# google/libultrahdr

Hardware: AMD Instinct MI355X
Metric: Mpixels/s encode+decode (API-1 P010+YUV420, 4K), device-resident round trip (higher is better)
Workload: dtype f32; 1 GPU; API-1 3840x2160 round trip per step: encode (P010 HLG + YCbCr420 -> two-pass 3-ch gain map at scale 1, FDCT q95, Huffman: two JPEG scans) + decode (Huffman, IDCT, applyGainMap -> RGBA_F16 linear); frames resident in HBM

## Files before the change

### libultrahdr_amd/csrc/api_context.cpp

```cpp
#include "api_internal.h"

#include <sys/mman.h>
#include <mutex>
#include <algorithm>

namespace uhdr_api {
uhdr_error_info_t ensure(DeviceBuf& b, size_t bytes) {
  if (b.cap >= bytes) return ok_status();
  if (b.p) (void)hipFree(b.p);
  b.p = nullptr;
  b.cap = 0;
  size_t want = bytes + (bytes >> 3) + 256;
  HIP_TRY(hipMalloc(&b.p, want));
  b.cap = want;
  return ok_status();
}


size_t bytes_per_sample(int fmt) {
  switch (fmt) {
    case UHDR_IMG_FMT_24bppYCbCrP010:
    case UHDR_IMG_FMT_30bppYCbCr444: return 2;
    case UHDR_IMG_FMT_24bppRGB888: return 3;
    case UHDR_IMG_FMT_32bppRGBA8888:
// ... 389 lines not shown
  c->gain_tabs.push_back(g);
  *out = g.meta;
  return ok_status();
}

uhdr_error_info_t select_hdr_lut(uhdr_hip_ctx* c, uhdr_color_transfer_t ct, const float** lut, int* n) {
  *lut = nullptr;
  *n = 0;
  if (ct == UHDR_CT_HLG) {
    UHDR_TRY(upload_lut(&c->d_hlg_inv_ootf, host::hlg_inv_oetf_ootf_lut(), c->stream));
    *lut = c->d_hlg_inv_ootf; *n = kInvOetfN;
  } else if (ct == UHDR_CT_PQ) {
    UHDR_TRY(upload_lut(&c->d_pq_inv, host::pq_inv_oetf_lut(), c->stream));
    *lut = c->d_pq_inv; *n = kInvOetfN;
  } else if (ct == UHDR_CT_SRGB) {
    *lut = c->d_srgb; *n = kSrgbN;
  }
  return ok_status();
}

uhdr_error_info_t validate_metadata(const uhdr_gainmap_metadata_t* m) {
  if (!m) return err_status(UHDR_CODEC_INVALID_PARAM, "received nullptr for gainmap metadata descriptor");
  uhdr_error_info_t st = ok_status();
  for (int i = 0; i < 3; i++) {
    if (!std::isfinite(m->min_content_boost[i]) || !std::isfinite(m->max_content_boost[i]) ||
        !std::isfinite(m->offset_sdr[i]) || !std::isfinite(m->offset_hdr[i]) ||
        !std::isfinite(m->hdr_capacity_min) || !std::isfinite(m->hdr_capacity_max) || !std::isfinite(m->gamma[i])) {
      st = err_status(UHDR_CODEC_INVALID_PARAM, "Field(s) of gainmap metadata descriptor are either NaN or infinite");
    } else if (m->max_content_boost[i] < m->min_content_boost[i]) {
      st = err_status(UHDR_CODEC_INVALID_PARAM, "received bad value for content boost max %f, expects to be >= content boost min %f",
                      m->max_content_boost[i], m->min_content_boost[i]);
    } else if (m->min_content_boost[i] <= 0.0f) {
      return err_status(UHDR_CODEC_INVALID_PARAM, "received bad value for min boost %f, expects > 0.0f", m->min_content_boost[i]);
    } else if (m->gamma[i] <= 0.0f) {
      st = err_status(UHDR_CODEC_INVALID_PARAM, "received bad value for gamma %f, expects > 0.0f", m->gamma[i]);
    } else if (m->offset_sdr[i] < 0.0f) {
      st = err_status(UHDR_CODEC_INVALID_PARAM, "received bad value for offset sdr %f, expects to be >= 0.0f", m->offset_sdr[i]);
    } else if (m->offset_hdr[i] < 0.0f) {
      st = err_status(UHDR_CODEC_INVALID_PARAM, "received bad value for offset hdr %f, expects to be >= 0.0f", m->offset_hdr[i]);
    } else if (m->hdr_capacity_max <= m->hdr_capacity_min) {
      st = err_status(UHDR_CODEC_INVALID_PARAM, "received bad value for hdr capacity max %f, expects to be > hdr capacity min %f",
                      m->hdr_capacity_max, m->hdr_capacity_min);
    } else if (m->hdr_capacity_min < 1.0f) {
      st = err_status(UHDR_CODEC_INVALID_PARAM, "received bad value for hdr capacity min %f, expects to be >= 1.0f", m->hdr_capacity_min);
    }
  }
  return st;
}

bool is_rgb_fmt_host(int fmt) {
  return fmt == UHDR_IMG_FMT_64bppRGBAHalfFloat || fmt == UHDR_IMG_FMT_32bppRGBA8888 ||
         fmt == UHDR_IMG_FMT_32bppRGBA1010102;
}

uhdr_error_info_t validate_apply(const uhdr_raw_image_t* sdr, const uhdr_raw_image_t* gm,
                                 const uhdr_gainmap_metadata_t* md, uhdr_color_transfer_t out_ct,
                                 const uhdr_raw_image_t* dest) {
  if (dest == nullptr || dest->planes[UHDR_PLANE_PACKED] == nullptr)
    return err_status(UHDR_CODEC_INVALID_PARAM, "apply gainmap method received nullptr for destination image or plane pointer");
  if (dest->stride[UHDR_PLANE_PACKED] < dest->w)
    return err_status(UHDR_CODEC_INVALID_PARAM, "destination stride (%u) cannot be less than image width (%u)",
                      dest->stride[UHDR_PLANE_PACKED], dest->w);
  if (out_ct != UHDR_CT_LINEAR && out_ct != UHDR_CT_HLG && out_ct != UHDR_CT_PQ)
    return err_status(UHDR_CODEC_INVALID_PARAM,
                      "apply gainmap method expects output color transfer to be one of {UHDR_CT_LINEAR, UHDR_CT_HLG, UHDR_CT_PQ}. Received %d", out_ct);
  if ((out_ct == UHDR_CT_LINEAR && dest->fmt != UHDR_IMG_FMT_64bppRGBAHalfFloat) ||
      ((out_ct == UHDR_CT_HLG || out_ct == UHDR_CT_PQ) && dest->fmt != UHDR_IMG_FMT_32bppRGBA1010102))
    return err_status(UHDR_CODEC_INVALID_PARAM, "unsupported destination pixel format %d for output color transfer %d", dest->fmt, out_ct);
  UHDR_TRY(validate_metadata(md));
  if (!sdr || !gm) return err_status(UHDR_CODEC_INVALID_PARAM, "received nullptr for base image or gainmap image");
  if (sdr->fmt != UHDR_IMG_FMT_24bppYCbCr444 && sdr->fmt != UHDR_IMG_FMT_16bppYCbCr422 &&
      sdr->fmt != UHDR_IMG_FMT_12bppYCbCr420 && sdr->fmt != UHDR_IMG_FMT_24bppRGB888 &&
      sdr->fmt != UHDR_IMG_FMT_32bppRGBA8888)
    return err_status(UHDR_CODEC_UNSUPPORTED_FEATURE, "apply gainmap method expects base image color format to be one of "
                      "{UHDR_IMG_FMT_24bppYCbCr444, UHDR_IMG_FMT_16bppYCbCr422, UHDR_IMG_FMT_12bppYCbCr420, "
                      "UHDR_IMG_FMT_24bppRGB888, UHDR_IMG_FMT_32bppRGBA8888}. Received %d", sdr->fmt);
  if (gm->fmt != UHDR_IMG_FMT_8bppYCbCr400 && gm->fmt != UHDR_IMG_FMT_24bppRGB888 && gm->fmt != UHDR_IMG_FMT_32bppRGBA8888)
    return err_status(UHDR_CODEC_UNSUPPORTED_FEATURE, "apply gainmap method expects gainmap image color format to be one of "
                      "{UHDR_IMG_FMT_8bppYCbCr400, UHDR_IMG_FMT_24bppRGB888, UHDR_IMG_FMT_32bppRGBA8888}. Received %d", gm->fmt);
  return ok_status();
}

uhdr_error_info_t get_apply_tables(uhdr_hip_ctx* c, const uhdr_gainmap_metadata_t& md, float weight,
                                   int idw_scale, const float** d_out) {
  std::string key((const char*)&md, sizeof md);
  key.append((const char*)&weight, sizeof weight);
  key.append((const char*)&idw_scale, sizeof idw_scale);
  for (int i = 0; i < kTableSlots; i++)
    if (c->tab_cap[i] && c->tab_key[i] == key) { *d_out = c->d_tab[i]; return ok_status(); }
  const int slot = c->tab_next;
  c->tab_next = (c->tab_next + 1) % kTableSlots;
  std::vector<float> t;
  host::build_apply_tables(md, weight, idw_scale, &t);
  const size_t bytes = t.size() * sizeof(float);
  if (c->tab_cap[slot]) HIP_TRY(hipEventSynchronize(c->tab_ev[slot]));
  if (c->tab_cap[slot] < bytes) {
    HIP_TRY(hipStreamSynchronize(c->stream));
    if (c->h_tab[slot]) (void)hipHostFree(c->h_tab[slot]);
    if (c->d_tab[slot]) (void)hipFree(c->d_tab[slot]);
    c->h_tab[slot] = nullptr; c->d_tab[slot] = nullptr; c->tab_cap[slot] = 0;
    HIP_TRY(hipHostMalloc((void**)&c->h_tab[slot], bytes, hipHostMallocDefault));
    HIP_TRY(hipMalloc((void**)&c->d_tab[slot], bytes));
    if (!c->tab_ev[slot]) HIP_TRY(hipEventCreateWithFlags(&c->tab_ev[slot], hipEventDisableTiming));
    c->tab_cap[slot] = bytes;
  }
  memcpy(c->h_tab[slot], t.data(), bytes);
  HIP_TRY(hipMemcpyAsync(c->d_tab[slot], c->h_tab[slot], bytes, hipMemcpyHostToDevice, c->stream));
  HIP_TRY(hipEventRecord(c->tab_ev[slot], c->stream));
  c->tab_key[slot] = key;
  *d_out = c->d_tab[slot];
  return ok_status();
}
}


const char* uhdr_hip_version(void) { return "libuhdr_hip 0.3 (gfx950; reference libultrahdr 2.0.2 hot path)"; }

int uhdr_hip_device_count(void) {
  int n = 0;
  if (hipGetDeviceCount(&n) != hipSuccess) return 0;
  return n;
}

int uhdr_hip_current_device(void) {
  int d = -1;
  if (hipGetDevice(&d) != hipSuccess) return -1;
  return d;
}

uhdr_hip_ctx_t* uhdr_hip_create(int device, uhdr_error_info_t* err) {
  auto fail = [&](const char* what, hipError_t e) -> uhdr_hip_ctx_t* {
    if (err) *err = err_status(UHDR_CODEC_ERROR, "uhdr_hip_create: %s failed: %s (no CPU fallback exists behind this library)",
                               what, hipGetErrorString(e));
    return nullptr;
  };
  if (err) *err = ok_status();
  int n = 0;
  hipError_t e = hipGetDeviceCount(&n);
  if (e != hipSuccess || n == 0) return fail("hipGetDeviceCount", e == hipSuccess ? hipErrorNoDevice : e);
  if (device < 0) {
    e = hipGetDevice(&device);
    if (e != hipSuccess) return fail("hipGetDevice", e);
  }
  if (device >= n) return fail("device index", hipErrorInvalidDevice);
  e = hipSetDevice(device);
  if (e != hipSuccess) return fail("hipSetDevice", e);
  uhdr_hip_ctx* c = new uhdr_hip_ctx();
  c->device = device;
  {
    const char* e = getenv("UHDR_HIP_HUFF_TWO_PASS");
    c->huff_two_pass = e && atoi(e) != 0;
    e = getenv("UHDR_HIP_HUFF_ROUTE_LOG");
    c->huff_route_log = e && atoi(e) != 0;
  }
  e = hipStreamCreateWithFlags(&c->own_stream, hipStreamNonBlocking);
  if (e != hipSuccess) { delete c; return fail("hipStreamCreate", e); }
  c->stream = c->own_stream;
  uhdr_error_info_t st = upload_lut(&c->d_srgb, host::srgb_inv_oetf_lut(), c->stream);
  if (st.error_code != UHDR_CODEC_OK) {
    if (err) *err = st;
    (void)hipStreamDestroy(c->own_stream);
    delete c;
    return nullptr;
  }
  return c;
}

void uhdr_hip_destroy(uhdr_hip_ctx_t* c) {
  if (!c) return;
  (void)hipSetDevice(c->device);
  (void)hipStreamSynchronize(c->stream);
  for (auto& e : c->prof_entries) { (void)hipEventDestroy(e.a); (void)hipEventDestroy(e.b); }
  float* luts[] = {c->d_srgb, c->d_hlg_inv, c->d_pq_inv, c->d_hlg_oetf, c->d_pq_oetf, c->d_hlg_inv_ootf, (float*)c->d_math,
                   c->d_hlg_buckets, c->d_pq_buckets, c->d_hlg_buckets_pre, c->d_pq_buckets_pre};
  for (float* p : luts) if (p) (void)hipFree(p);
  for (int i = 0; i < kTableSlots; i++) {
    if (c->h_tab[i]) (void)hipHostFree(c->h_tab[i]);
    if (c->d_tab[i]) (void)hipFree(c->d_tab[i]);
    if (c->tab_ev[i]) (void)hipEventDestroy(c->tab_ev[i]);
  }
  for (auto& b : c->scratch) if (b.p) (void)hipFree(b.p);
  for (auto& b : c->jpg) if (b.p) (void)hipFree(b.p);
  for (auto& b : c->enc) if (b.p) (void)hipFree(b.p);
  if (c->huff_slots.p) (void)hipFree(c->huff_slots.p);
  for (auto& r : c->resident) if (r.buf.p) (void)hipFree(r.buf.p);
  if (c->pending.buf.p) (void)hipFree(c->pending.buf.p);
  if (c->pending.tmp.p) (void)hipFree(c->pending.tmp.p);
  if (c->minmax.p) (void)hipFree(c->minmax.p);
  if (c->d_coef_src) (void)hipFree(c->d_coef_src);
  if (c->d_huff) (void)hipFree(c->d_huff);
  if (c->d_srgb8) (void)hipFree(c->d_srgb8);
  for (float* q : c->d_lin10) if (q) (void)hipFree(q);
  for (auto& g : c->gain_tabs) if (g.d) (void)hipFree(g.d);
  uhdr_hip_comm_destroy(c);
  aux_worker_destroy(c);
  if (c->aux) uhdr_hip_destroy(c->aux);
  if (c->exchange.p) (void)hipFree(c->exchange.p);
  if (c->affine.p) (void)hipFree(c->affine.p);
  if (c->d_srgb_of_byte) (void)hipFree(c->d_srgb_of_byte);
  if (c->h_mm) (void)hipHostFree(c->h_mm);
  if (c->aux_ev) (void)hipEventDestroy(c->aux_ev);
  if (c->aux_ev2) (void)hipEventDestroy(c->aux_ev2);
  if (c->md_ev) (void)hipEventDestroy(c->md_ev);
  if (c->md_stream) (void)hipStreamDestroy(c->md_stream);
  if (c->h_flags) (void)hipHostFree(c->h_flags);
  if (c->pin.p) (void)hipHostFree(c->pin.p);
  if (c->pin.ev) (void)hipEventDestroy(c->pin.ev);
  if (c->huff_tabs.dev.p) (void)hipFree(c->huff_tabs.dev.p);
  if (c->own_stream) (void)hipStreamDestroy(c->own_stream);
  delete c;
}

int uhdr_hip_recycle(uhdr_hip_ctx_t* c, size_t keep_bytes) {
  if (!c) return -1;
  (void)hipSetDevice(c->device);
  (void)hipStreamSynchronize(c->stream);
  uhdr_hip_resident_forget(c);
  uhdr_hip_resident_begin(c);
  uhdr_hip_resident_end(c);
  c->sticky = ok_status();
  for (auto& h : c->huff_hint) h = uhdr_hip_ctx::HuffHint();
  c->stats = uhdr_hip_stats_t();
  c->deferred_md.valid = false;
  c->huff_slots_refused = 0;
  std::vector<DeviceBuf*> bufs;
  for (auto& b : c->scratch) bufs.push_back(&b);
  for (auto& b : c->jpg) bufs.push_back(&b);
  for (auto& b : c->enc) bufs.push_back(&b);
  bufs.push_back(&c->huff_slots);
  for (auto& r : c->resident) bufs.push_back(&r.buf);
  bufs.push_back(&c->pending.buf);
  bufs.push_back(&c->pending.tmp);
  size_t total = c->pin.cap;
  for (DeviceBuf* b : bufs) total += b->p ? b->cap : 0;
  std::sort(bufs.begin(), bufs.end(), [](const DeviceBuf* a, const DeviceBuf* b) { return (a->p ? a->cap : 0) > (b->p ? b->cap : 0); });
  for (DeviceBuf* b : bufs) {
    if (total <= keep_bytes) break;
    if (!b->p) continue;
    (void)hipFree(b->p);
    total -= b->cap;
    b->p = nullptr;
    b->cap = 0;
  }
  if (total > keep_bytes && c->pin.p) {
    if (c->pin.ev_pending && c->pin.ev) (void)hipEventSynchronize(c->pin.ev);
    (void)hipHostFree(c->pin.p);
    c->pin.p = nullptr;
    c->pin.cap = c->pin.off = 0;
    c->pin.ev_pending = false;
  }
  if (c->aux) (void)uhdr_hip_recycle(c->aux, keep_bytes);
  return c->device;
}

uhdr_error_info_t uhdr_hip_set_stream(uhdr_hip_ctx_t* c, void* hip_stream) {
  if (!c) return err_status(UHDR_CODEC_INVALID_PARAM, "received nullptr for uhdr_hip context");
  HIP_TRY(hipStreamSynchronize(c->stream));
  c->stream = hip_stream ? (hipStream_t)hip_stream : c->own_stream;
  return ok_status();
}

void* uhdr_hip_get_stream(uhdr_hip_ctx_t* c) { return c ? (void*)c->stream : nullptr; }

uhdr_error_info_t uhdr_hip_synchronize(uhdr_hip_ctx_t* c) {
  if (!c) return err_status(UHDR_CODEC_INVALID_PARAM, "received nullptr for uhdr_hip context");
  HIP_TRY(hipStreamSynchronize(c->stream));
  return ok_status();
}

void uhdr_hip_get_stats(uhdr_hip_ctx_t* c, uhdr_hip_stats_t* out) {
  if (!out) return;
  if (!c) { memset(out, 0, sizeof *out); return; }
  *out = c->stats;
}

namespace {
std::mutex g_seam_mu;
std::vector<uhdr_hip_seam_stage_t> g_seam_rows;
unsigned long long g_seam_seq = 0;
void seam_dump_at_exit() {
  const char* path = getenv("UHDR_HIP_SEAM_STATS_FILE");
  FILE* f = path ? fopen(path, "w") : nullptr;
  if (!f) return;
  std::lock_guard<std::mutex> lk(g_seam_mu);
  fprintf(f, "{");
  for (size_t i = 0; i < g_seam_rows.size(); i++) {
    const auto& r = g_seam_rows[i];
    fprintf(f, "%s\"%s\": {\"device\": %llu, \"reference\": %llu, \"device_ms\": %.3f, \"first_seq\": %llu}", i ? ", " : "", r.name, r.device_calls,
            r.reference_calls, r.device_ms, r.first_seq);
  }
  fprintf(f, "}\n");
  fclose(f);
}
}

void uhdr_hip_seam_note(const char* stage, int on_device, double ms) {
  if (!stage) return;
  static const bool dump = [] { return getenv("UHDR_HIP_SEAM_STATS_FILE") ? (atexit(seam_dump_at_exit), true) : false; }();
  (void)dump;
  std::lock_guard<std::mutex> lk(g_seam_mu);
  uhdr_hip_seam_stage_t* row = nullptr;
  for (auto& r : g_seam_rows)
    if (!strncmp(r.name, stage, sizeof r.name - 1)) { row = &r; break; }
  if (!row) {
    if (g_seam_rows.size() >= 64) return;
    uhdr_hip_seam_stage_t r;
// ... 152 lines not shown
```

### libultrahdr_amd/csrc/api_entropy.cpp

```cpp
#include "api_internal.h"

#include <condition_variable>
#include <functional>
#include <mutex>

uhdr_error_info_t uhdr_api::check_scan(const uhdr_hip_jpeg_scan_t* sc, bool need_coef, int* mcus_per_row, int* mcu_rows, int* blocks_per_mcu) {
  if (!sc) return err_status(UHDR_CODEC_INVALID_PARAM, "received nullptr for the scan description");
  if (sc->num_components != 1 && sc->num_components != 3)
    return err_status(UHDR_CODEC_INVALID_PARAM, "a scan has 1 or 3 components, received %d", sc->num_components);
  if (sc->w == 0 || sc->h == 0 || sc->w > 65535 || sc->h > 65535)
    return err_status(UHDR_CODEC_INVALID_PARAM, "image dimensions %ux%u are outside JPEG's 1..65535", sc->w, sc->h);
  int hmax = 1, vmax = 1, bpm = 0;
  for (int i = 0; i < sc->num_components; i++) {
    const int hs = sc->num_components == 1 ? 1 : sc->h_samp[i], vs = sc->num_components == 1 ? 1 : sc->v_samp[i];
    if (hs < 1 || hs > 2 || vs < 1 || vs > 2) return err_status(UHDR_CODEC_INVALID_PARAM, "component %d: sampling factors %dx%d not in {1, 2}", i, hs, vs);
    if (hs > hmax) hmax = hs;
    if (vs > vmax) vmax = vs;
    bpm += hs * vs;
    if (need_coef && (!sc->coef[i] || ((uintptr_t)sc->coef[i] & 15)))
      return err_status(UHDR_CODEC_INVALID_PARAM, "coefficient buffer %d is null or not 16-byte aligned", i);
    if (sc->blocks_w[i] < 1 || sc->blocks_h[i] < 1) return err_status(UHDR_CODEC_INVALID_PARAM, "component %d: empty block grid", i);
  }
  if (sc->num_components == 1) {
    *mcus_per_row = sc->blocks_w[0];
// ... 171 lines not shown
static bool make_fast_table(const uint8_t bits[17], const uint8_t vals[256], HuffFastTable* t, int* nsub_out = nullptr) {
  memset(t, 0, sizeof *t);
  int code = 0, k = 0, nsub = 0;
  int sub_of[512];
  for (int i = 0; i < 512; i++) sub_of[i] = -1;
  for (int l = 1; l <= 16; l++) {
    for (int i = 0; i < bits[l]; i++, k++, code++) {
      if (code >= (1 << l) || k >= 256) return false;
      if (l <= 9) {
        const int lo = code << (9 - l);
        for (int x = 0; x < (1 << (9 - l)); x++) t->l1[lo + x] = (uint16_t)((l << 8) | vals[k]);
      } else {
        const int prefix = code >> (l - 9);
        if (sub_of[prefix] < 0) {
          if (nsub >= kHuffL2Max) return false;
          sub_of[prefix] = nsub++;
          t->l1[prefix] = (uint16_t)(0x8000u | (unsigned)sub_of[prefix]);
        }
        const int rest = (code << (16 - l)) & 127;
        for (int x = 0; x < (1 << (16 - l)); x++) t->l2[sub_of[prefix]][rest + x] = (uint16_t)((l << 8) | vals[k]);
      }
    }
    code <<= 1;
  }
  if (nsub_out) *nsub_out = nsub;
  return true;
}

static void make_track_table(const HuffFastTable& f, bool is_dc, HuffFastTable* t) {
  auto conv = [&](uint16_t e) -> uint16_t {
    if (e & 0x8000u) return e;
    unsigned adv, kinc;
    if (e == 0) {
      adv = 16;
      kinc = is_dc ? 1 : 64;
    } else {
      const unsigned len = (e >> 8) & 31u, rs = e & 255u;
      if (is_dc) {
        const unsigned sz = rs > 15u ? 0u : rs;
        adv = len + sz;
        kinc = 1;
      } else {
        const unsigned sz = rs & 15u, run = rs >> 4;
        adv = len + sz;
        kinc = sz ? run + 1 : (run == 15u ? 16u : 64u);
      }
    }
    return (uint16_t)(adv | (kinc << 5));
  };
  for (int i = 0; i < 512; i++) t->l1[i] = conv(f.l1[i]);
  for (int s = 0; s < kHuffL2Max; s++)
    for (int i = 0; i < 128; i++) t->l2[s][i] = conv(f.l2[s][i]);
}

static void make_value_table(const HuffFastTable& f, bool is_dc, uint32_t* out ) {
  auto conv = [&](uint16_t e, bool first_level) -> uint32_t {
    if (first_level && (e & 0x8000u)) return 0x80000000u | (e & 31u);
    unsigned adv, kinc, sz = 0, bad = 0;
    if (e == 0) {
      adv = 16;
      kinc = is_dc ? 1 : 64;
      bad = 1;
    } else {
      const unsigned len = (e >> 8) & 31u, rs = e & 255u;
      if (is_dc) {
        if (rs > 15u) bad = 1; else sz = rs;
        adv = len + sz;
        kinc = 1;
      } else {
        sz = rs & 15u;
        const unsigned run = rs >> 4;
        adv = len + sz;
        kinc = sz ? run + 1 : (run == 15u ? 16u : 64u);
      }
    }
    return adv | (kinc << 5) | (sz << 12) | (bad << 16);
  };
  for (int i = 0; i < 512; i++) out[i] = conv(f.l1[i], true);
  for (int s = 0; s < kHuffL2Max; s++)
    for (int i = 0; i < 128; i++) out[512 + s * 128 + i] = conv(f.l2[s][i], false);
}

static void make_pair_table(const HuffFastTable& f, const HuffFastTable& t, const HuffFastTable& f_ac, const HuffFastTable& t_ac, int l2_base, uint32_t* out ) {
  constexpr int B = kHuffPairBits;
  for (int idx = 0; idx < kHuffPairWords; idx++) {
    const int p9 = idx >> (B - 9);
    const uint16_t e = f.l1[p9];
    uint32_t first;
    bool defined;
    if (e & 0x8000u) {
      const int sub = e & 31, rest = (idx & ((1 << (B - 9)) - 1)) << (16 - B);
      const uint16_t e2 = f.l2[sub][rest];
      if (e2 == 0 || (int)((e2 >> 8) & 31u) > B) {
        out[idx] = 0x80000000u | (uint32_t)(l2_base + sub);
        continue;
      }
      first = t.l2[sub][rest];
      defined = true;
    } else {
      first = t.l1[p9];
      defined = e != 0;
    }
    uint32_t word = first & 0xfffu;
    const int adv1 = (int)(first & 31u), kinc1 = (int)((first >> 5) & 127u);
    if (defined && kinc1 < 64 && adv1 < B) {
      const int r = B - adv1;
      const int next9 = ((idx << adv1) & (kHuffPairWords - 1)) >> (B - 9);
      const uint16_t n = f_ac.l1[next9];
      if (n != 0 && !(n & 0x8000u) && (int)((n >> 8) & 31u) <= r) {
        const uint32_t second = t_ac.l1[next9];
        word |= (second & 31u) << 12 | ((second >> 5) & 127u) << 17;
      }
    }
    out[idx] = word;
  }
}

static void make_pair_value_table(const HuffFastTable& f, const uint32_t* v, const HuffFastTable& f_ac, const uint32_t* v_ac, int l2_base, uint32_t* out ) {
  constexpr int B = kHuffPairBits;
  for (int idx = 0; idx < kHuffPairWords; idx++) {
    const int p9 = idx >> (B - 9);
    const uint16_t e = f.l1[p9];
    uint32_t first;
    bool defined;
    if (e & 0x8000u) {
      const int sub = e & 31, rest = (idx & ((1 << (B - 9)) - 1)) << (16 - B);
      const uint16_t e2 = f.l2[sub][rest];
      if (e2 == 0 || (int)((e2 >> 8) & 31u) > B) {
        out[2 * idx] = 0x80000000u | (uint32_t)(l2_base + sub);
        out[2 * idx + 1] = 0;
        continue;
      }
      first = v[512 + sub * 128 + rest];
      defined = true;
    } else {
      first = v[p9];
      defined = e != 0;
    }
    uint32_t second = 0;
    const int adv1 = (int)(first & 31u), kinc1 = (int)((first >> 5) & 127u);
    if (defined && !((first >> 16) & 1u) && kinc1 < 64 && adv1 < B) {
      const int r = B - adv1;
      const int next9 = ((idx << adv1) & (kHuffPairWords - 1)) >> (B - 9);
      const uint16_t n = f_ac.l1[next9];
      if (n != 0 && !(n & 0x8000u) && (int)((n >> 8) & 31u) <= r) second = v_ac[next9];
    }
    out[2 * idx] = first;
    out[2 * idx + 1] = second;
  }
}

uhdr_error_info_t uhdr_hip_huffman_decode_dev(uhdr_hip_ctx_t* c, const uhdr_hip_jpeg_scan_t* sc, const uhdr_hip_huff_tables_t* tables,
                                              const uint8_t* data, size_t data_bytes) {
  if (!c) return err_status(UHDR_CODEC_INVALID_PARAM, "received nullptr for uhdr_hip context");
  if (!data || data_bytes == 0 || data_bytes > 0xFFFFFFF0ull) return err_status(UHDR_CODEC_INVALID_PARAM, "received no (or more than 4 GiB of) entropy-coded data");
  int mpr = 0, mrows = 0, bpm = 0;
  UHDR_TRY(check_scan(sc, true, &mpr, &mrows, &bpm));
  if (sc->restart_interval < 0 || sc->restart_interval > 65535) return err_status(UHDR_CODEC_INVALID_PARAM, "restart_interval %d out of range", sc->restart_interval);
  HIP_TRY(hipSetDevice(c->device));
  if (!c->d_huff) {
    std::vector<uint32_t> blob(host::jpeg_huff_code_tables());
    blob.resize((size_t)host::kHuffTabWords + 16);
    memcpy(blob.data() + host::kHuffTabWords, host::jpeg_zigzag_to_natural(), 64);
    HIP_TRY(hipMalloc((void**)&c->d_huff, blob.size() * sizeof(uint32_t)));
    HIP_TRY(hipMemcpyAsync(c->d_huff, blob.data(), blob.size() * sizeof(uint32_t), hipMemcpyHostToDevice, c->stream));
    HIP_TRY(hipStreamSynchronize(c->stream));
  }
  const DbgClock dbg;
  constexpr size_t kTabDec = 0, kTabFast = (sizeof(HuffDecTable) * 4 + 255) & ~(size_t)255,
                   kTabVal = (kTabFast + sizeof(HuffFastTable) * 8 + 255) & ~(size_t)255, kTabPair = kTabVal + (size_t)4 * kHuffValWords * 4,
                   kTabPairVal = kTabPair + (size_t)kHuffPairBlobWords * 4, kTabBytes = kTabPairVal + (size_t)kHuffPairValBlobWords * 4;
  {
    uint8_t key[4 * (17 + 256)];
    for (int t = 0; t < 4; t++) {
      uint8_t* bits = key + (size_t)t * (17 + 256);
      uint8_t* vals = bits + 17;
      if (tables) {
        memcpy(bits, tables->bits[t], 17);
        memcpy(vals, tables->vals[t], 256);
      } else {
        memset(bits, 0, 17 + 256);
        host::jpeg_std_huff_table(t & 1, t >> 1, bits, vals);
      }
    }
    uhdr_hip_ctx::HuffTabCache& hc = c->huff_tabs;
    if (!hc.valid || memcmp(hc.key, key, sizeof key) != 0) {
      hc.valid = false;
      std::vector<HuffDecTable> tabs(4);
      std::vector<HuffFastTable> ftabs(8);
      std::vector<uint32_t> vtabs((size_t)4 * kHuffValWords), ptabs((size_t)kHuffPairBlobWords), pvtabs((size_t)kHuffPairValBlobWords);
      bool fast_ok = true;
      int l2_count[4] = {0, 0, 0, 0};
      for (int t = 0; t < 4; t++) {
        const uint8_t* bits = key + (size_t)t * (17 + 256);
        if (!make_dec_table(bits, bits + 17, &tabs[(size_t)t])) return err_status(UHDR_CODEC_INVALID_PARAM, "Huffman table %d is not a valid DHT table", t);
        fast_ok = make_fast_table(bits, bits + 17, &ftabs[(size_t)t], &l2_count[t]) && fast_ok;
      }
      int l2_base[4] = {0, 0, 0, 0};
      for (int t = 1; t < 4; t++) l2_base[t] = l2_base[t - 1] + l2_count[t - 1];
      if (l2_base[3] + l2_count[3] > kHuffL2Total) fast_ok = false;
      if (fast_ok)
        for (int t = 0; t < 4; t++) {
          make_track_table(ftabs[(size_t)t], (t & 1) == 0, &ftabs[(size_t)t + 4]);
          make_value_table(ftabs[(size_t)t], (t & 1) == 0, vtabs.data() + (size_t)t * kHuffValWords);
        }
      if (fast_ok)
        for (int t = 0; t < 4; t++)
        {
          make_pair_table(ftabs[(size_t)t], ftabs[(size_t)t + 4], ftabs[(size_t)(t | 1)], ftabs[(size_t)(t | 1) + 4], l2_base[t], ptabs.data() + (size_t)t * kHuffPairWords);
          make_pair_value_table(ftabs[(size_t)t], vtabs.data() + (size_t)t * kHuffValWords, ftabs[(size_t)(t | 1)], vtabs.data() + (size_t)(t | 1) * kHuffValWords,
                                l2_base[t], pvtabs.data() + (size_t)t * 2 * kHuffPairWords);
          uint16_t* l2t = (uint16_t*)(ptabs.data() + (size_t)4 * kHuffPairWords) + (size_t)l2_base[t] * 128;
          uint16_t* l2v = (uint16_t*)(pvtabs.data() + (size_t)8 * kHuffPairWords) + (size_t)l2_base[t] * 128;
          for (int i = 0; i < l2_count[t] * 128; i++) {
            l2t[i] = ftabs[(size_t)t + 4].l2[i / 128][i % 128];
            const uint32_t v = vtabs[(size_t)t * kHuffValWords + 512 + (size_t)i];
            l2v[i] = (uint16_t)(((v >> 16) & 1u) ? 0u : (v & 0xffffu));
          }
        }
      UHDR_TRY(ensure(hc.dev, kTabBytes));
      HIP_TRY(hipStreamSynchronize(c->stream));
      HIP_TRY(hipMemcpy((uint8_t*)hc.dev.p + kTabDec, tabs.data(), sizeof(HuffDecTable) * 4, hipMemcpyHostToDevice));
      HIP_TRY(hipMemcpy((uint8_t*)hc.dev.p + kTabFast, ftabs.data(), sizeof(HuffFastTable) * 8, hipMemcpyHostToDevice));
      HIP_TRY(hipMemcpy((uint8_t*)hc.dev.p + kTabVal, vtabs.data(), vtabs.size() * 4, hipMemcpyHostToDevice));
      HIP_TRY(hipMemcpy((uint8_t*)hc.dev.p + kTabPair, ptabs.data(), ptabs.size() * 4, hipMemcpyHostToDevice));
      HIP_TRY(hipMemcpy((uint8_t*)hc.dev.p + kTabPairVal, pvtabs.data(), pvtabs.size() * 4, hipMemcpyHostToDevice));
      memcpy(hc.key, key, sizeof key);
      hc.fast_ok = fast_ok;
      hc.valid = true;
    }
  }
  const bool fast_ok = c->huff_tabs.fast_ok;
  const uint8_t* tabs_dev = (const uint8_t*)c->huff_tabs.dev.p;
  if (!c->h_flags) HIP_TRY(hipHostMalloc((void**)&c->h_flags, 64 * sizeof(uint32_t), hipHostMallocDefault));
  HuffDecArgs a;
  memset(&a, 0, sizeof a);
  a.ncomp = sc->num_components;
  size_t zero_bytes[3] = {0, 0, 0};
  for (int i = 0; i < a.ncomp; i++) {
    a.coef[i] = const_cast<int16_t*>(sc->coef[i]);
    a.bw[i] = sc->blocks_w[i]; a.bh[i] = sc->blocks_h[i];
    a.hs[i] = a.ncomp == 1 ? 1 : sc->h_samp[i]; a.vs[i] = a.ncomp == 1 ? 1 : sc->v_samp[i];
    zero_bytes[i] = (size_t)a.bw[i] * a.bh[i] * 64 * sizeof(int16_t);
  }
  a.mcus_per_row = mpr;
  a.total_mcus = mpr * mrows;
  a.ri = sc->restart_interval;
  a.nseg = a.ri > 0 ? (a.total_mcus + a.ri - 1) / a.ri : 1;
  a.data = data;
  a.nbytes = (uint32_t)data_bytes;
  a.zigzag = (const uint8_t*)(c->d_huff + host::kHuffTabWords);
  const int nchunks = huff_marker_chunks(data_bytes);
  const size_t need = 16 + ((size_t)nchunks + 2 * (size_t)a.nseg) * sizeof(uint32_t);
  UHDR_TRY(ensure(c->scratch[5], need));
  uint8_t* base = (uint8_t*)c->scratch[5].p;
  a.tabs = (const HuffDecTable*)(tabs_dev + kTabDec);
  a.status = (uint32_t*)base;
  uint32_t* counts = a.status + 4;
  uint32_t* starts = counts + nchunks;
  uint32_t* ends = starts + a.nseg;
  a.starts = starts;
  a.ends = ends;
  dbg.mark("huffman_decode_dev: tables ready");
  const bool rst_sync = a.nseg > 1 && data_bytes / (size_t)a.nseg >= 320 && !getenv("UHDR_HIP_HUFF_RST_INTERVALS");
  const bool try_sync = (a.nseg == 1 || rst_sync) && data_bytes >= 4096 && data_bytes < ((size_t)1 << 29) && fast_ok && !getenv("UHDR_HIP_HUFF_SERIAL") && bpm <= 16;
  const int write_form = [] { const char* e = getenv("UHDR_HIP_HUFF_WRITE"); return e ? atoi(e) : 2; }();
  const bool form2 = try_sync && !rst_sync && write_form != 1;
  bool coef_zeroed = !form2;
  if (!form2)
    for (int i = 0; i < a.ncomp; i++) HIP_TRY(hipMemsetAsync(a.coef[i], 0, zero_bytes[i], c->stream));
  bool sync_done = false;
  if (try_sync) {
    struct Attempt { uint32_t sub_bits; int levels; };
    std::vector<Attempt> attempts;
    bool sparse = false;
    {
      const char* eb = getenv("UHDR_HIP_HUFF_SUB_BITS");
      const char* el = getenv("UHDR_HIP_HUFF_LEVELS");
      const int vb = eb ? atoi(eb) : 0;
      const bool vb_ok = vb >= 256 && vb <= 4096 && (vb & (vb - 1)) == 0;
      if (vb_ok || el) {
        const uint32_t sbits = vb_ok ? (uint32_t)vb : 1024u;
        const int lv = el ? atoi(el) : (sbits <= 512 ? 7 : 4);
        if (lv >= 1 && lv <= 15 && bpm * (lv + 1) <= kHuffHypSlots) attempts.push_back({sbits, lv});
        attempts.push_back({sbits, 0});
      } else {
        const uint64_t bits_per_block = (uint64_t)data_bytes * 8u / (uint64_t)((uint64_t)a.total_mcus * (uint64_t)bpm);
        const int lv_fit = kHuffHypSlots / bpm - 1;
        const int lv = lv_fit >= 15 ? 15 : (lv_fit >= 11 ? 11 : (lv_fit >= 7 ? 7 : (lv_fit >= 4 ? 4 : 0)));
        sparse = bits_per_block < 64;
        uint32_t first = bits_per_block < 64 ? 1024u : (bits_per_block < 200 ? 512u : (bits_per_block < 400 ? 2048u : 4096u));
        const uhdr_hip_ctx::HuffHint& hint = c->huff_hint[bpm & 15];
        if (hint.sub_bits > first && bits_per_block * 4 >= hint.bits_per_block * 3 && bits_per_block * 4 <= hint.bits_per_block * 5) first = hint.sub_bits;
        if (lv > 0)
          for (uint32_t sbits = first; sbits <= 4096u; sbits <<= 1) attempts.push_back({sbits, lv});
        attempts.push_back({1024u, 0});
      }
    }
    uint32_t sub_bits = attempts[0].sub_bits;
    bool use_hyp = false;
    for (const Attempt& t : attempts) { if (t.sub_bits < sub_bits) sub_bits = t.sub_bits; use_hyp = use_hyp || t.levels > 0; }
    const int max_rounds = 40;
    const int nch = huff_sync_chunks(data_bytes);
    const uint32_t nsub = huff_sync_max_subsequences(data_bytes, sub_bits);
    const uint32_t total_blocks = (uint32_t)a.total_mcus * (uint32_t)bpm;
    size_t off = 0;
    auto take = [&](size_t bytes) { const size_t o = off; off += (bytes + 255) & ~(size_t)255; return o; };
    const size_t rst_words = data_bytes / 32 + 2;
    const size_t o_clean = take(data_bytes + 16), o_cnt = take((size_t)nch * 4);
    const size_t o_flags = take(128), o_nblk = take((size_t)nsub * 4 + 4), o_dcd = take((size_t)total_blocks * 4), o_rm = rst_sync ? take(rst_words * 4) : 0;
    const size_t zero_bytes_sync = off - o_flags;
    const size_t o_s0 = take((size_t)nsub * 8), o_hm = use_hyp ? take((size_t)nsub * kHuffHypSlots) : 0;
    const size_t ff_bytes = off - o_s0;
    const size_t o_s1 = take((size_t)nsub * 8), o_c0 = take(nsub), o_c1 = take(nsub), o_dcp = take((size_t)((total_blocks + 255) / 256) * 12 + 16),
                 o_ft = take(sizeof(HuffFastTable) * 8),
                 o_st = take(((size_t)nsub / 2048 + 2) * 4), o_vt = take((size_t)4 * kHuffValWords * 4);
    const size_t o_hs = use_hyp ? take((size_t)nsub * kHuffHypSlots * 8) : 0, o_hc = use_hyp ? take((size_t)nsub * kHuffHypSlots * 2) : 0;
    size_t chain_tiles_off = 0;
    const size_t o_ch = use_hyp ? take(huff_hyp_chain_bytes(data_bytes, sub_bits, &chain_tiles_off)) : 0;
    (void)chain_tiles_off;
    const size_t o_ds = rst_sync ? take((size_t)a.nseg * 12) : 0, o_rp = rst_sync ? take((size_t)nch * 12) : 0;
    const size_t o_sl = use_hyp ? take((size_t)nsub * (size_t)bpm * 8) : 0;
    const int max_pieces = [&] {
      const char* e = getenv("UHDR_HIP_HUFF_PIECES");
      const int v = e ? atoi(e) : 4;
      return (use_hyp && form2 && !rst_sync && v >= 1 && v <= 4) ? v : 1;
    }();
    const size_t o_ms = max_pieces > 1 ? take((size_t)nsub * kHuffHypSlots * (size_t)(max_pieces - 1) * 8) : 0;
    const size_t o_mc = max_pieces > 1 ? take((size_t)nsub * kHuffHypSlots * (size_t)(max_pieces - 1) * 2) : 0;
    const size_t o_pe = max_pieces > 1 ? take((size_t)nsub * (size_t)max_pieces * 8 + 64) : 0;
    const size_t o_pc = max_pieces > 1 ? take(((size_t)nsub * (size_t)max_pieces + 4) * 4) : 0;
    const size_t o_st2 = max_pieces > 1 ? take(((size_t)nsub * (size_t)max_pieces / 2048 + 4) * 4) : 0;
    const size_t scan_bytes = form2 ? (size_t)total_blocks * 64 * sizeof(int16_t) : 0;
    const size_t o_cs = form2 ? take(scan_bytes + 256) : 0;
    UHDR_TRY(ensure(c->scratch[6], off));
    uint8_t* sb = (uint8_t*)c->scratch[6].p;
    HuffSyncArgs y;
    memset(&y, 0, sizeof y);
    y.clean = sb + o_clean;
    y.nbytes = (uint32_t)data_bytes;
    y.flags = (uint32_t*)(sb + o_flags);
    y.nstuffed = y.flags + 8;
    y.sub_bits = sub_bits;
    y.state[0] = (uint64_t*)(sb + o_s0); y.state[1] = (uint64_t*)(sb + o_s1);
    y.changed[0] = sb + o_c0; y.changed[1] = sb + o_c1;
    y.nblk = (uint32_t*)(sb + o_nblk);
    y.scan_tmp = (uint32_t*)(sb + o_st);
    y.dcd = (int*)(sb + o_dcd);
    y.total_blocks = total_blocks;
    y.blocks_per_mcu = bpm; y.ncomp = a.ncomp; y.mcus_per_row = a.mcus_per_row;
    uint32_t* rst_map = nullptr;
    if (rst_sync) {
      rst_map = (uint32_t*)(sb + o_rm);
      y.rst_map = rst_map;
      y.rst_blocks = (uint32_t)a.ri * (uint32_t)bpm;
      y.dc_seg = (int*)(sb + o_ds);
      y.rst_partial = (uint32_t*)(sb + o_rp);
      y.rst_chunks = (uint32_t)nch;
    }
    int j = 0;
    for (int i = 0; i < a.ncomp; i++) {
      y.bw[i] = a.bw[i]; y.bh[i] = a.bh[i]; y.hs[i] = a.hs[i]; y.vs[i] = a.vs[i]; y.coef[i] = a.coef[i];
      y.first_blk[i] = j;
      for (int k = 0; k < a.hs[i] * a.vs[i] && j < 16; k++) y.comp_of[j++] = (uint8_t)i;
    }
    y.ftabs = (const HuffFastTable*)(tabs_dev + kTabFast);
    y.ttabs = y.ftabs + 4;
    y.vtabs = (const uint32_t*)(tabs_dev + kTabVal);
    y.ptabs = (const uint32_t*)(tabs_dev + kTabPair);
    y.pvtabs = (const uint32_t*)(tabs_dev + kTabPairVal);
    y.zigzag = a.zigzag;
    (void)o_ft; (void)o_vt;
    if (use_hyp) {
      y.strag_list = (uint32_t*)(sb + o_sl);
      y.strag_cap = nsub * (uint32_t)bpm;
    }
    if (form2) y.coef_scan = (int16_t*)(sb + o_cs);
    const int main_levels_env = [&] { const char* e = getenv("UHDR_HIP_HUFF_MAIN_LEVELS"); return e ? atoi(e) : (sparse ? 1 : 2); }();
    if (j == bpm && bpm <= 16) {
      const bool fills_in_unstuff = attempts[0].levels > 0 && zero_bytes_sync % 16 == 0 && ff_bytes % 16 == 0 && zero_bytes_sync / 16 < 0xFFFFFFFFull &&
                                    ff_bytes / 16 < 0xFFFFFFFFull && !getenv("UHDR_HIP_HUFF_FILL_LAUNCHES");
      HuffInitFill init_fill;
      memset(&init_fill, 0, sizeof init_fill);
      if (fills_in_unstuff) {
        init_fill.zero_ptr = (uint4*)y.flags;
        init_fill.zero_vec = (uint32_t)(zero_bytes_sync / 16);
        init_fill.ff_ptr = (uint4*)y.state[0];
        init_fill.ff_vec = (uint32_t)(ff_bytes / 16);
      } else {
        HIP_TRY(hipMemsetAsync(y.flags, 0, zero_bytes_sync, c->stream));
      }
      auto pass0_zeroes = [&](const Attempt& t) { return form2 && t.levels > 0 && scan_bytes % 16 == 0 && scan_bytes / 16 < 0xFFFFFFFFull; };
      if (form2 && !pass0_zeroes(attempts[0])) HIP_TRY(hipMemsetAsync(y.coef_scan, 0, scan_bytes, c->stream));
      dbg.mark("huffman_decode_dev: fills enqueued");
      int final_buf = 0;
      uint32_t* fl = c->h_flags;
      for (int q = 0; q < 24; q++) fl[q] = 0;
      bool hyp_done = false, unstuffed = false, rounds_ran = false;
      auto start_over = [&](const Attempt& next) -> uhdr_error_info_t {
        HIP_TRY(hipMemsetAsync(y.flags, 0, 32, c->stream));
        HIP_TRY(hipMemsetAsync(y.flags + kHuffFlagStragglers, 0, 4, c->stream));
        HIP_TRY(hipMemsetAsync(y.nblk, 0, (size_t)nsub * 4 + 4, c->stream));
        if (form2) {
          if (!pass0_zeroes(next)) HIP_TRY(hipMemsetAsync(y.coef_scan, 0, scan_bytes, c->stream));
        } else {
          HIP_TRY(hipMemsetAsync(y.dcd, 0, (size_t)total_blocks * 4, c->stream));
          for (int i = 0; i < a.ncomp; i++) HIP_TRY(hipMemsetAsync(a.coef[i], 0, zero_bytes[i], c->stream));
        }
        return ok_status();
      };
      for (size_t ti = 0; ti < attempts.size() && !hyp_done && !rounds_ran; ti++) {
        const Attempt& t = attempts[ti];
        if (ti > 0) UHDR_TRY(start_over(t));
        y.sub_bits = t.sub_bits;
        y.zero_ptr = pass0_zeroes(t) ? (uint4*)y.coef_scan : nullptr;
        y.zero_vec = pass0_zeroes(t) ? (uint32_t)(scan_bytes / 16) : 0u;
        const uint32_t nsub_t = huff_sync_max_subsequences(data_bytes, t.sub_bits);
        if (t.levels > 0) {
          y.hyp_h = bpm;
          y.hyp_levels = t.levels;
          y.hyp_main_levels = rst_sync ? 0 : main_levels_env;
          y.strag_levels = [&] { const char* e = getenv("UHDR_HIP_HUFF_STRAG_LEVELS"); return e ? atoi(e) : t.levels; }();
          y.hyp_state = (uint64_t*)(sb + o_hs);
          y.hyp_map = sb + o_hm;
          y.hyp_cnt = (uint16_t*)(sb + o_hc);
          y.hyp_hist = getenv("UHDR_HIP_HUFF_DEBUG") ? 1 : 0;
          {
            int q = t.sub_bits >= 1024u ? (int)(t.sub_bits / 256u) : 1;
            if (getenv("UHDR_HIP_HUFF_PIECES_ALL")) q = (int)(t.sub_bits / 256u);
            if (q > max_pieces) q = max_pieces;
            if (q < 1) q = 1;
            while (q > 1 && (t.sub_bits % (uint32_t)q || (t.sub_bits / (uint32_t)q) % 32u)) q--;
            if (q == 3) q = 2;
            if (getenv("UHDR_HIP_HUFF_QMERGE") && atoi(getenv("UHDR_HIP_HUFF_QMERGE")) == 0) q = 1;
            y.pieces = q;
            y.mid_state = q > 1 ? (uint64_t*)(sb + o_ms) : nullptr;
            y.mid_cnt = q > 1 ? (uint16_t*)(sb + o_mc) : nullptr;
            y.pend = q > 1 ? (uint64_t*)(sb + o_pe) : nullptr;
            y.pcnt = q > 1 ? (uint32_t*)(sb + o_pc) : nullptr;
            y.scan_tmp = q > 1 ? (uint32_t*)(sb + o_st2) : (uint32_t*)(sb + o_st);
          }
          if (!(fills_in_unstuff && ti == 0)) HIP_TRY(hipMemsetAsync(y.state[0], 0xff, ff_bytes, c->stream));
          size_t tiles_off = 0;
          (void)huff_hyp_chain_bytes(data_bytes, t.sub_bits, &tiles_off);
          {
            ProfScope ps(c, "huffman_decode");
            if (!unstuffed)
              HIP_TRY(launch_huffman_unstuff(data, (uint32_t)data_bytes, (uint32_t*)(sb + o_cnt), y.flags + 8, sb + o_clean, c->stream, rst_map, y.rst_partial,
                                             fills_in_unstuff && ti == 0 ? &init_fill : nullptr));
            unstuffed = true;
            HIP_TRY(launch_huffman_decode_hyp(y, (int*)(sb + o_dcp), sb + o_ch, sb + o_ch + tiles_off, c->stream));
          }
          dbg.mark("huffman_decode_dev: hypothesis attempt enqueued");
          HIP_TRY(hipMemcpyAsync(fl, y.flags, 24 * sizeof(uint32_t), hipMemcpyDeviceToHost, c->stream));
          HIP_TRY(wait_stream(c));
          dbg.mark("huffman_decode_dev: hypothesis attempt finished");
          hyp_done = fl[2] == 0;
          if (hyp_done && ti > 0) {
            uhdr_hip_ctx::HuffHint& hint = c->huff_hint[bpm & 15];
            hint.sub_bits = t.sub_bits;
            hint.bits_per_block = (uint32_t)((uint64_t)data_bytes * 8u / ((uint64_t)a.total_mcus * (uint64_t)bpm));
          }
          if (getenv("UHDR_HIP_HUFF_DEBUG")) {
            uint32_t hist[32] = {};
            (void)hipMemcpy(hist, y.flags, sizeof hist, hipMemcpyDeviceToHost);
            fprintf(stderr, "uhdr_hip: hypothesis decode of %zu bytes, %u subsequences of %u bits x %d: merges per level %u %u %u %u %u %u+, %u paths unmerged after %d levels (%d in lockstep, %u paths handed to the straggler waves), true path %s\n",
                    data_bytes, nsub_t, t.sub_bits, bpm, hist[10], hist[11], hist[12], hist[13], hist[14], hist[15], fl[3], t.levels, y.hyp_main_levels, fl[kHuffFlagStragglers], hyp_done ? "resolved" : "LOST (next attempt)");
            fprintf(stderr, "uhdr_hip: the stragglers' merges at level 2 .. 10, 11+: %u %u %u %u %u %u %u %u %u %u\n", hist[22], hist[23], hist[24], hist[25], hist[26], hist[27], hist[28], hist[29],
                    hist[30], hist[31]);
          }
        } else {
          y.pieces = 1;
          y.scan_tmp = (uint32_t*)(sb + o_st);
          {
            ProfScope ps(c, "huffman_decode");
            if (!unstuffed) HIP_TRY(launch_huffman_unstuff(data, (uint32_t)data_bytes, (uint32_t*)(sb + o_cnt), y.flags + 8, sb + o_clean, c->stream, rst_map, y.rst_partial));
            unstuffed = true;
            HIP_TRY(launch_huffman_decode_sync(y, max_rounds, (int*)(sb + o_dcp), &final_buf, c->stream));
          }
          HIP_TRY(hipMemcpyAsync(fl, y.flags, 24 * sizeof(uint32_t), hipMemcpyDeviceToHost, c->stream));
          HIP_TRY(wait_stream(c));
          rounds_ran = true;
        }
      }
      const bool settled = hyp_done || fl[4 + max_rounds % 3] == 0;
      if (rst_sync && getenv("UHDR_HIP_HUFF_DEBUG"))
        fprintf(stderr, "uhdr_hip: restart file through the parallel decoder: %s, status bits %#x, %u markers dropped (%d expected), sequence sums %s\n",
                settled ? "settled" : "NOT settled", fl[1], fl[9], a.nseg - 1, fl[0] == fl[16] && fl[7] == fl[17] ? "equal" : "DIFFERENT");
      if (settled && rst_sync && ((fl[1] & 14u) != 0 || fl[9] != (uint32_t)(a.nseg - 1) || fl[0] != fl[16] || fl[7] != fl[17])) {
        for (int i = 0; i < a.ncomp; i++) HIP_TRY(hipMemsetAsync(a.coef[i], 0, zero_bytes[i], c->stream));
        coef_zeroed = true;
      } else if (settled) {
        if (fl[1] & 8u) return err_status(UHDR_CODEC_INVALID_PARAM, "corrupt entropy-coded data (the scan ends before its last block)");
        if (fl[1] & 2u) return err_status(UHDR_CODEC_INVALID_PARAM, "corrupt entropy-coded data (undefined Huffman code or a run past the end of a block)");
        sync_done = true;
      } else {
        if (a.nseg == 1 && !c->huff_serial_ok && data_bytes > (256u << 10)) {
          c->stats.entropy_decode_declined++;
          return err_status(UHDR_CODEC_UNSUPPORTED_FEATURE, "the parallel entropy decode did not settle in %d rounds; %zu bytes on one lane would take longer than the CPU", max_rounds, data_bytes);
        }
        for (int i = 0; i < a.ncomp; i++) HIP_TRY(hipMemsetAsync(a.coef[i], 0, zero_bytes[i], c->stream));
        coef_zeroed = true;
      }
    }
  }
  if (sync_done) {
    c->stats.entropy_decode_parallel++;
    return ok_status();
  }
  if (a.nseg == 1 && !c->huff_serial_ok && data_bytes > (256u << 10)) {
    c->stats.entropy_decode_declined++;
    return err_status(UHDR_CODEC_UNSUPPORTED_FEATURE, "a %zu-byte scan without restart markers that the parallel decoder does not take (Huffman tables outside its two-level form)", data_bytes);
  }
  if (!coef_zeroed)
    for (int i = 0; i < a.ncomp; i++) HIP_TRY(hipMemsetAsync(a.coef[i], 0, zero_bytes[i], c->stream));
  HIP_TRY(hipMemsetAsync(a.status, 0, 16, c->stream));
  {
    ProfScope ps(c, "huffman_decode");
    HIP_TRY(launch_huffman_decode(a, counts, starts, ends, c->stream));
  }
  if (a.nseg == 1) c->stats.entropy_decode_single_lane++;
  else c->stats.entropy_decode_intervals++;
  uint32_t st[2] = {0, 0};
  HIP_TRY(hipMemcpyAsync(st, a.status, sizeof st, hipMemcpyDeviceToHost, c->stream));
  HIP_TRY(wait_stream(c));
  if (st[1] != (uint32_t)(a.nseg - 1))
    return err_status(UHDR_CODEC_INVALID_PARAM, "found %u restart markers, a restart interval of %d MCUs over %d MCUs needs %d", st[1], a.ri,
                      a.total_mcus, a.nseg - 1);
  if (st[0] & 4u) return err_status(UHDR_CODEC_INVALID_PARAM, "restart markers out of sequence");
  if (st[0] & 2u) return err_status(UHDR_CODEC_INVALID_PARAM, "corrupt entropy-coded data (undefined Huffman code or a run past the end of a block)");
  return ok_status();
}

uhdr_error_info_t uhdr_api::aux_context(uhdr_hip_ctx* c, uhdr_hip_ctx** out) {
  if (!c->aux) {
    uhdr_error_info_t e = ok_status();
    c->aux = uhdr_hip_create(c->device, &e);
    if (!c->aux) return e.error_code != UHDR_CODEC_OK ? e : err_status(UHDR_CODEC_ERROR, "could not create the auxiliary context");
  }
  c->aux->prof = c->prof;
  c->aux->huff_serial_ok = c->huff_serial_ok;
  c->aux->huff_route_log = c->huff_route_log;
  c->aux->huff_two_pass = c->huff_two_pass;
  *out = c->aux;
  return ok_status();
}
void uhdr_api::aux_merge(uhdr_hip_ctx* c) {
  if (!c->aux) return;
  uhdr_hip_ctx* x = c->aux;
  c->stats.entropy_decode_parallel += x->stats.entropy_decode_parallel;
  c->stats.entropy_decode_intervals += x->stats.entropy_decode_intervals;
  c->stats.entropy_decode_single_lane += x->stats.entropy_decode_single_lane;
  c->stats.entropy_decode_declined += x->stats.entropy_decode_declined;
  c->stats.entropy_encode_stream += x->stats.entropy_encode_stream;
  c->stats.entropy_encode_intervals += x->stats.entropy_encode_intervals;
  x->stats = uhdr_hip_stats_t();
  for (auto& e : x->prof_entries) c->prof_entries.push_back(e);
  x->prof_entries.clear();
}

struct AuxWorker {
  static constexpr int kSpinUs = 300;
  std::thread th;
  std::mutex mu;
  std::condition_variable cv;
  std::function<void()> job;
  std::atomic<int> state{0};
  std::atomic<bool> busy{false};
  static bool spin_until(const std::function<bool()>& pred, int us) {
    const auto t0 = std::chrono::steady_clock::now();
    while (!pred()) {
      if (std::chrono::steady_clock::now() - t0 > std::chrono::microseconds(us)) return pred();
#if defined(__x86_64__)
      __builtin_ia32_pause();
#endif
    }
    return true;
  }
  AuxWorker() {
    th = std::thread([this] {
      for (;;) {
        if (!spin_until([this] { return state.load(std::memory_order_acquire) != 0; }, kSpinUs)) {
          std::unique_lock<std::mutex> lk(mu);
          cv.wait(lk, [this] { return state.load(std::memory_order_acquire) != 0; });
        }
        if (state.load(std::memory_order_acquire) == 2) return;
        std::function<void()> j;
        {
          std::lock_guard<std::mutex> lk(mu);
          j = std::move(job);
          state.store(0, std::memory_order_release);
        }
        j();
        {
          std::lock_guard<std::mutex> lk(mu);
          busy.store(false, std::memory_order_release);
        }
        cv.notify_all();
      }
    });
  }
  void run(std::function<void()> j) {
    {
      std::lock_guard<std::mutex> lk(mu);
      job = std::move(j);
      busy.store(true, std::memory_order_release);
      state.store(1, std::memory_order_release);
    }
    cv.notify_all();
  }
  void wait() {
    if (spin_until([this] { return !busy.load(std::memory_order_acquire); }, kSpinUs)) return;
    std::unique_lock<std::mutex> lk(mu);
    cv.wait(lk, [this] { return !busy.load(std::memory_order_acquire); });
  }
  ~AuxWorker() {
    {
      std::lock_guard<std::mutex> lk(mu);
      state.store(2, std::memory_order_release);
    }
    cv.notify_all();
    if (th.joinable()) th.join();
  }
};
void aux_worker_destroy(uhdr_hip_ctx* c) {
  if (c && c->aux_worker) {
    delete c->aux_worker;
    c->aux_worker = nullptr;
  }
}
bool uhdr_api::aux_post(uhdr_hip_ctx* c, std::function<void()> job) {
  static const bool no_thread = getenv("UHDR_HIP_NO_AUX_THREAD") != nullptr;
  if (no_thread) return false;
  if (!c->aux_worker) {
    try {
      c->aux_worker = new AuxWorker();
    } catch (...) {
      c->aux_worker = nullptr;
    }
  }
  if (!c->aux_worker) return false;
  c->aux_worker->run(std::move(job));
  return true;
}
void uhdr_api::aux_wait(uhdr_hip_ctx* c) {
  if (c->aux_worker) c->aux_worker->wait();
}
namespace {
template <typename FA, typename FB>
void run_pair(uhdr_hip_ctx* c, FA&& job_a, FB&& job_b) {
  static const bool no_thread = getenv("UHDR_HIP_NO_AUX_THREAD") != nullptr;
  if (!c->aux_worker && !no_thread) {
    try {
      c->aux_worker = new AuxWorker();
    } catch (...) {
      c->aux_worker = nullptr;
    }
  }
  if (c->aux_worker) {
    c->aux_worker->run(job_b);
    job_a();
    c->aux_worker->wait();
  } else {
    job_a();
    job_b();
  }
}
}

uhdr_error_info_t uhdr_hip_huffman_encode2_dev(uhdr_hip_ctx_t* c, const uhdr_hip_jpeg_scan_t* scan_a, uint8_t* out_a, size_t cap_a, size_t* bytes_a,
                                               const uhdr_hip_jpeg_scan_t* scan_b, uint8_t* out_b, size_t cap_b, size_t* bytes_b) {
  if (!c) return err_status(UHDR_CODEC_INVALID_PARAM, "received nullptr for uhdr_hip context");
  HIP_TRY(hipSetDevice(c->device));
  uhdr_hip_ctx* x = nullptr;
  UHDR_TRY(aux_context(c, &x));
  if (!c->aux_ev) HIP_TRY(hipEventCreateWithFlags(&c->aux_ev, hipEventDisableTiming));
  HIP_TRY(hipEventRecord(c->aux_ev, c->stream));
  HIP_TRY(hipStreamWaitEvent(x->stream, c->aux_ev, 0));
  uhdr_error_info_t ra = ok_status(), rb = ok_status();
  const int dev = c->device;
  run_pair(c, [&] { ra = uhdr_hip_huffman_encode_dev(c, scan_a, out_a, cap_a, bytes_a); },
           [&, dev] { (void)hipSetDevice(dev); rb = uhdr_hip_huffman_encode_dev(x, scan_b, out_b, cap_b, bytes_b); });
  aux_merge(c);
  return ra.error_code != UHDR_CODEC_OK ? ra : rb;
}

uhdr_error_info_t uhdr_hip_huffman_decode2_dev(uhdr_hip_ctx_t* c, const uhdr_hip_jpeg_scan_t* scan_a, const uhdr_hip_huff_tables_t* tables_a, const uint8_t* data_a,
                                               size_t bytes_a, const uhdr_hip_jpeg_scan_t* scan_b, const uhdr_hip_huff_tables_t* tables_b,
                                               const uint8_t* data_b, size_t bytes_b) {
  if (!c) return err_status(UHDR_CODEC_INVALID_PARAM, "received nullptr for uhdr_hip context");
  HIP_TRY(hipSetDevice(c->device));
  uhdr_hip_ctx* x = nullptr;
  UHDR_TRY(aux_context(c, &x));
  if (!c->aux_ev) HIP_TRY(hipEventCreateWithFlags(&c->aux_ev, hipEventDisableTiming));
  HIP_TRY(hipEventRecord(c->aux_ev, c->stream));
  HIP_TRY(hipStreamWaitEvent(x->stream, c->aux_ev, 0));
  uhdr_error_info_t ra = ok_status(), rb = ok_status();
  const int dev = c->device;
  run_pair(c, [&] { ra = uhdr_hip_huffman_decode_dev(c, scan_a, tables_a, data_a, bytes_a); },
           [&, dev] { (void)hipSetDevice(dev); rb = uhdr_hip_huffman_decode_dev(x, scan_b, tables_b, data_b, bytes_b); });
  aux_merge(c);
  return ra.error_code != UHDR_CODEC_OK ? ra : rb;
}
```

### libultrahdr_amd/csrc/api_internal.h

```cpp
#ifndef UHDR_HIP_API_INTERNAL_H
#define UHDR_HIP_API_INTERNAL_H

#pragma GCC visibility push(default)
#include "uhdr_hip.h"
#pragma GCC visibility pop

#include <cfloat>
#include <chrono>
#include <cmath>
#include <cstdarg>
#include <cstdio>
#include <cstring>
#include <atomic>
#include <functional>
#include <map>
#include <memory>
#include <string>
#include <thread>
#include <vector>
#include "exact_math.h"
#include "host_tables.h"
#include "uhdr_types.h"
#include "rccl_bind.h"

using namespace uhdr;

inline uhdr_error_info_t ok_status() {
  uhdr_error_info_t s;
  s.error_code = UHDR_CODEC_OK;
  s.has_detail = 0;
  s.detail[0] = 0;
  return s;
}
inline uhdr_error_info_t err_status(uhdr_codec_err_t code, const char* fmt, ...) {
  uhdr_error_info_t s;
  s.error_code = code;
  s.has_detail = 1;
  va_list ap;
  va_start(ap, fmt);
  vsnprintf(s.detail, sizeof s.detail, fmt, ap);
  va_end(ap);
  return s;
}
#define HIP_TRY(expr)                                                                      \
  do {                                                                                     \
    hipError_t e_ = (expr);                                                                \
    if (e_ != hipSuccess)                                                                  \
      return err_status(e_ == hipErrorOutOfMemory ? UHDR_CODEC_MEM_ERROR : UHDR_CODEC_ERROR, \
                        "HIP error '%s' at %s:%d", hipGetErrorString(e_), __FILE__, __LINE__); \
  } while (0)
#define UHDR_TRY(expr)                                 \
  do {                                                 \
    uhdr_error_info_t s_ = (expr);                     \
    if (s_.error_code != UHDR_CODEC_OK) return s_;     \
  } while (0)

struct DbgClock {
  bool on;
  std::chrono::steady_clock::time_point t0;
  DbgClock() : on(getenv("UHDR_HIP_CLOCK_DEBUG") != nullptr), t0(std::chrono::steady_clock::now()) {}
  void mark(const char* what) const {
    if (on) fprintf(stderr, "uhdr_hip:   [%7.1f us] %s\n", std::chrono::duration<double, std::micro>(std::chrono::steady_clock::now() - t0).count(), what);
  }
};

struct ProfEntry {
  hipEvent_t a, b;
  std::string family;
};

constexpr int kTableSlots = 4;

struct DeviceBuf {
  void* p = nullptr;
  size_t cap = 0;
};

struct uhdr_hip_ctx {
  int device = 0;
  hipStream_t own_stream = nullptr;
  hipStream_t stream = nullptr;
  float* d_srgb = nullptr;
  float* d_hlg_inv = nullptr;
  float* d_pq_inv = nullptr;
  float* d_hlg_oetf = nullptr;
  float* d_pq_oetf = nullptr;
  float* d_hlg_buckets = nullptr;
  float* d_pq_buckets = nullptr;
  float* d_hlg_buckets_pre = nullptr;
  float* d_pq_buckets_pre = nullptr;
  float* d_hlg_inv_ootf = nullptr;
  double* d_math = nullptr;
  float* h_tab[kTableSlots] = {};
  float* d_tab[kTableSlots] = {};
  size_t tab_cap[kTableSlots] = {};
  hipEvent_t tab_ev[kTableSlots] = {};
  std::string tab_key[kTableSlots];
  int tab_next = 0;
  DeviceBuf scratch[8];
  uhdr_hip_stats_t stats = {};
  bool huff_serial_ok = true;
  DeviceBuf huff_slots;
  bool huff_two_pass = false;
  bool huff_route_log = false;
  size_t huff_slots_refused = 0;
  DeviceBuf enc[3];
  uhdr_hip_ctx* aux = nullptr;
  struct AuxWorker* aux_worker = nullptr;
  DeviceBuf jpg[6];
  struct Resident {
    DeviceBuf buf;
    bool valid = false;
    uhdr_img_fmt_t fmt = UHDR_IMG_FMT_UNSPECIFIED;
    unsigned int w = 0, h = 0;
    const void* host[3] = {};
    unsigned int host_stride[3] = {};
    size_t off[3] = {};
    unsigned int dev_stride[3] = {};
    unsigned int prows[3] = {}, pcols[3] = {};
    bool host_unwritten = false;
    bool adopted = false;
    void* adopt_dst = nullptr;
    unsigned int adopt_stride = 0, adopt_w = 0, adopt_h = 0;
    bool adopt_expand = false;
  } resident[2];
  struct HuffHint { uint32_t sub_bits = 0, bits_per_block = 0; } huff_hint[16];
  struct HuffTabCache {
    bool valid = false, fast_ok = false;
    uint8_t key[4 * (17 + 256)] = {};
    DeviceBuf dev;
  } huff_tabs;
  struct PinArena {
    void* p = nullptr;
    size_t cap = 0, off = 0;
    hipEvent_t ev = nullptr;
    bool ev_pending = false;
  } pin;
  uint32_t* h_flags = nullptr;
  bool resident_on = false;
  bool resident_lazy = false;
  uhdr_error_info_t sticky = {};
  unsigned int resident_next = 0;
  struct PendingCopy {
    DeviceBuf buf;
    bool on = false;
    size_t off = 0, pitch = 0, dst_pitch = 0;
    unsigned int w = 0, h = 0, bps = 0;
    bool expand = false;
    void* dst = nullptr;
    DeviceBuf tmp;
  } pending;
  struct MallEntry { const void* p; uint64_t stamp; };
  std::vector<MallEntry> mall;
  uint64_t mall_clock = 0;
  DeviceBuf minmax;
  uint32_t* d_huff = nullptr;
  CoefSrc* d_coef_src = nullptr;
  unsigned int coef_src_next = 0;
  CoefSrc* coef_src_last_slot = nullptr;
  std::vector<uint8_t> coef_src_last;
  float* d_srgb8 = nullptr;
  StepTab srgb8_meta = {};
  float* d_lin10[5] = {};
  struct GainTab { float mn, mx; float* d; StepTab meta; };
  std::vector<GainTab> gain_tabs;
  void* comm = nullptr;
  int comm_rank = 0, comm_size = 0;
  bool comm_custom = false;
  uhdr_hip_comm_ops_t comm_ops = {};
  DeviceBuf exchange;
  DeviceBuf affine;
  float* d_srgb_of_byte = nullptr;
  float* h_mm = nullptr;
  bool defer_md = false;
  hipStream_t md_stream = nullptr;
  hipEvent_t md_ev = nullptr;
  std::function<void()> on_side_launched;
  bool side_job_posted = false;
  struct DeferredMd { bool valid = false, run = false; uhdr_hip_encode_cfg_t cfg; uhdr_color_transfer_t hdr_ct; int use_base_cg = 1; } deferred_md;
  hipEvent_t aux_ev = nullptr;
  hipEvent_t aux_ev2 = nullptr;
  bool prof = false;
  std::vector<ProfEntry> prof_entries;
};

struct ProfScope {
  uhdr_hip_ctx* c;
  ProfEntry e;
  bool on;
  ProfScope(uhdr_hip_ctx* ctx, const char* family) : c(ctx), on(ctx->prof) {
    if (!on) return;
    e.family = family;
    if (hipEventCreate(&e.a) != hipSuccess || hipEventCreate(&e.b) != hipSuccess) { on = false; return; }
    (void)hipEventRecord(e.a, c->stream);
  }
  ~ProfScope() {
    if (!on) return;
    (void)hipEventRecord(e.b, c->stream);
    c->prof_entries.push_back(e);
  }
};

namespace uhdr_api {
uhdr_error_info_t ensure(DeviceBuf& b, size_t bytes);
size_t bytes_per_sample(int fmt);
bool plane_geom(const uhdr_raw_image_t* im, int pl, size_t* rows, size_t* width);
size_t plane_bytes(const uhdr_raw_image_t* im, int pl);
uhdr_error_info_t validate_image(const uhdr_raw_image_t* im, const char* what);
ImageView view_of(const uhdr_raw_image_t* im);
ImageViewMut view_mut_of(const uhdr_raw_image_t* im);
uhdr_error_info_t adopted_copy_out(uhdr_hip_ctx* c, const void* src, size_t src_pitch, unsigned int bps, bool expand, unsigned int w, unsigned int h,
                                   void* dst, size_t dst_pitch);
uhdr_error_info_t resident_write_back(uhdr_hip_ctx* c, uhdr_hip_ctx::Resident& r);
uhdr_error_info_t resident_write_back_all(uhdr_hip_ctx* c);
void resident_retire(uhdr_hip_ctx* c, uhdr_hip_ctx::Resident& r, bool host_is_rewritten);
void resident_drop(uhdr_hip_ctx* c, const void* host_plane);
uhdr_error_info_t fast_h2d(uhdr_hip_ctx* c, void* dst, const void* src, size_t bytes);
uhdr_error_info_t stage_in(uhdr_hip_ctx* c, int slot, const uhdr_raw_image_t* host, uhdr_raw_image_t* dev, bool upload);
bool resident_keeps(int fmt);
uhdr_error_info_t resident_keep(uhdr_hip_ctx* c, const uhdr_raw_image_t* dev, const uhdr_raw_image_t* host, bool host_unwritten = false);
uhdr_error_info_t stage_out(uhdr_hip_ctx* c, const uhdr_raw_image_t* dev, uhdr_raw_image_t* host);
uhdr_error_info_t upload_lut(float** dst, const std::vector<float>& src, hipStream_t s);
uhdr_error_info_t upload_math(uhdr_hip_ctx* c);
uhdr_error_info_t upload_step_table(const host::OetfBuckets& b, float** slot, StepTab* meta, hipStream_t s);
uhdr_error_info_t gain_step_table(uhdr_hip_ctx* c, const GenParams& p, StepTab* out);
uhdr_error_info_t select_hdr_lut(uhdr_hip_ctx* c, uhdr_color_transfer_t ct, const float** lut, int* n);
uhdr_error_info_t validate_metadata(const uhdr_gainmap_metadata_t* m);
bool is_rgb_fmt_host(int fmt);
uhdr_error_info_t validate_apply(const uhdr_raw_image_t* sdr, const uhdr_raw_image_t* gm, const uhdr_gainmap_metadata_t* md, uhdr_color_transfer_t out_ct,
                                 const uhdr_raw_image_t* dest);
uhdr_error_info_t get_apply_tables(uhdr_hip_ctx* c, const uhdr_gainmap_metadata_t& md, float weight, int idw_scale, const float** d_out);
uhdr_error_info_t fill_gen_params(uhdr_hip_ctx* c, const uhdr_raw_image_t* sdr, const uhdr_raw_image_t* hdr, const uhdr_hip_encode_cfg_t* cfg, GenParams* p,
                                  int* use_base_cg, float* hdr_white_nits_out, bool sdr_in_registers = false);
void fill_finalize(MinmaxTableParams* t, const uhdr_hip_encode_cfg_t* cfg);
void fill_gainmap_desc(const uhdr_raw_image_t* hdr, const GenParams& p, uhdr_raw_image_t* gm);
uhdr_error_info_t generate_gainmap_finalize_md(const uhdr_hip_encode_cfg_t* cfg, uhdr_color_transfer_t hdr_ct, int use_base_cg, const float mm[6], uhdr_gainmap_metadata_t* md);
void note_table_stats(uhdr_hip_ctx* c, const uhdr_hip_encode_cfg_t* cfg);
uhdr_error_info_t two_pass_tail(uhdr_hip_ctx* c, const GenParams& p, int n_partials, const uhdr_hip_encode_cfg_t* cfg, uhdr_raw_image_t* gm);
uhdr_error_info_t fill_tone_map_params(uhdr_hip_ctx* c, const uhdr_raw_image_t* hdr, ToneMapParams* pp);
uhdr_error_info_t comm_all_reduce_min(uhdr_hip_ctx* c, float* buf, size_t n);
uhdr_error_info_t check_scan(const uhdr_hip_jpeg_scan_t* sc, bool need_coef, int* mcus_per_row, int* mcu_rows, int* blocks_per_mcu);
uhdr_error_info_t aux_context(uhdr_hip_ctx* c, uhdr_hip_ctx** out);
void aux_merge(uhdr_hip_ctx* c);
bool aux_post(uhdr_hip_ctx* c, std::function<void()> job);
void aux_wait(uhdr_hip_ctx* c);
}
using namespace uhdr_api;

void aux_worker_destroy(uhdr_hip_ctx* c);

#endif
```

### libultrahdr_amd/csrc/api_jpeg.cpp

```cpp
#include "api_internal.h"

void uhdr_hip_jpeg_quant_table(int quality, int is_chroma, uint16_t qt[64]) { host::jpeg_quant_table(quality, is_chroma, qt); }

int uhdr_hip_oetf_code_thresholds(uhdr_color_transfer_t ct, float thresholds[1024]) {
  if ((ct != UHDR_CT_HLG && ct != UHDR_CT_PQ) || !thresholds) return -1;
  const std::vector<float>& t = host::oetf_code_thresholds(ct);
  for (int i = 0; i < 1024; i++) thresholds[i] = t[(size_t)i];
  return 0;
}

uhdr_error_info_t uhdr_hip_selftest(uhdr_hip_ctx_t* c, int which, unsigned int arg0, unsigned int arg1, unsigned int seed, const float mm[6],
                                    unsigned long long out[8]) {
  if (!c) return err_status(UHDR_CODEC_INVALID_PARAM, "received nullptr for uhdr_hip context");
  if (!out || which < 0 || which > 4 || (which == 4 && (!mm || arg0 > 2 || arg1 < 1 || arg1 > 3 || arg0 >= arg1)) || (which == 2 && (arg0 < 1 || arg1 > 254 || arg0 > arg1)))
    return err_status(UHDR_CODEC_INVALID_PARAM, "bad self-test arguments");
  HIP_TRY(hipSetDevice(c->device));
  UHDR_TRY(upload_math(c));
  UHDR_TRY(ensure(c->affine, kAffineDevBytes));
  UHDR_TRY(ensure(c->exchange, 256));
  unsigned long long* d_out = (unsigned long long*)c->exchange.p;
  HIP_TRY(hipMemsetAsync(d_out, 0, 64, c->stream));
  if (which == 4) {
    MinmaxTableParams t;
    memset(&t, 0, sizeof t);
// ... 1016 lines not shown
}

static uhdr_error_info_t idct_upsample_rgb_impl(uhdr_hip_ctx_t* c, const int16_t* const coef[3], const int bw[3], const int bh[3],
                                                const uint16_t* const qt[3], int variant, int vsamp, uhdr_raw_image_t* rgb) {
  if (bw[1] != bw[2] || bh[1] != bh[2]) return err_status(UHDR_CODEC_UNSUPPORTED_FEATURE, "Cb and Cr block grids differ");
  if (vsamp == 1 && ((unsigned)bw[1] * 8 < (rgb->w + 1) / 2 || (unsigned)bh[1] * 8 < rgb->h))
    return err_status(UHDR_CODEC_INVALID_PARAM, "a %dx%d chroma block grid does not cover a %ux%u 4:2:2 image", bw[1], bh[1], rgb->w, rgb->h);
  for (int k = 0; k < 3; k++)
    for (int i = 0; i < 64; i++)
      if (qt[k][i] == 0) return err_status(UHDR_CODEC_INVALID_PARAM, "quantization table %d entry %d is zero", k, i);
  uint8_t* scratch = nullptr;
  if (variant == 0) {
    UHDR_TRY(ensure(c->jpg[5], upsample_scratch_bytes(bw, bh)));
    scratch = (uint8_t*)c->jpg[5].p;
  }
  rgb->range = UHDR_CR_FULL_RANGE;
  ProfScope ps(c, vsamp == 2 ? "idct_upsample_rgb" : "idct_upsample_rgb422");
  HIP_TRY(launch_idct_upsample_rgb(coef, bw, bh, qt, variant, vsamp, view_mut_of(rgb), scratch, c->stream));
  return ok_status();
}

static uhdr_error_info_t idct_upsample_rgb_dev(const char* name, uhdr_hip_ctx_t* c, const int16_t* coef_y, const int16_t* coef_cb,
                                               const int16_t* coef_cr, unsigned int w, unsigned int h, int cbw, int cbh, const uint16_t qt_y[64],
                                               const uint16_t qt_cb[64], const uint16_t qt_cr[64], int variant, int vsamp, uhdr_raw_image_t* rgb) {
  if (!c) return err_status(UHDR_CODEC_INVALID_PARAM, "received nullptr for uhdr_hip context");
  if (!coef_y || !coef_cb || !coef_cr || !qt_y || !qt_cb || !qt_cr || !rgb || !rgb->planes[0])
    return err_status(UHDR_CODEC_INVALID_PARAM, "received bad argument for %s", name);
  if (rgb->fmt != UHDR_IMG_FMT_24bppRGB888 && rgb->fmt != UHDR_IMG_FMT_32bppRGBA8888)
    return err_status(UHDR_CODEC_UNSUPPORTED_FEATURE, "%s expects UHDR_IMG_FMT_24bppRGB888 or UHDR_IMG_FMT_32bppRGBA8888. Received %d", name, rgb->fmt);
  if (variant != 0 && variant != 1) return err_status(UHDR_CODEC_INVALID_PARAM, "unknown libjpeg variant %d", variant);
  if (w == 0 || h == 0 || w > 65535 || h > 65535) return err_status(UHDR_CODEC_INVALID_PARAM, "image dimensions %ux%u are outside JPEG's 1..65535", w, h);
  if (rgb->w != w || rgb->h != h) return err_status(UHDR_CODEC_INVALID_PARAM, "destination is %ux%u, the image %ux%u", rgb->w, rgb->h, w, h);
  if (rgb->stride[0] < w) return err_status(UHDR_CODEC_INVALID_PARAM, "stride (%u) cannot be less than width (%u)", rgb->stride[0], w);
  if (((uintptr_t)coef_y | (uintptr_t)coef_cb | (uintptr_t)coef_cr) & 15)
    return err_status(UHDR_CODEC_INVALID_PARAM, "coefficient buffers must be 16-byte aligned");
  HIP_TRY(hipSetDevice(c->device));
  const int16_t* coef[3] = {coef_y, coef_cb, coef_cr};
  const int bw[3] = {(int)((w + 7) / 8), cbw, cbw};
  const int bh[3] = {(int)((h + 7) / 8), cbh, cbh};
  const uint16_t* qt[3] = {qt_y, qt_cb, qt_cr};
  return idct_upsample_rgb_impl(c, coef, bw, bh, qt, variant, vsamp, rgb);
}

uhdr_error_info_t uhdr_hip_idct_upsample_rgb_dev(uhdr_hip_ctx_t* c, const int16_t* coef_y, const int16_t* coef_cb, const int16_t* coef_cr,
                                                 unsigned int w, unsigned int h, const uint16_t qt_y[64], const uint16_t qt_cb[64],
                                                 const uint16_t qt_cr[64], int variant, uhdr_raw_image_t* rgb) {
  return idct_upsample_rgb_dev("idct_upsample_rgb", c, coef_y, coef_cb, coef_cr, w, h, (int)((w + 15) / 16), (int)((h + 15) / 16), qt_y, qt_cb, qt_cr,
                               variant, 2, rgb);
}

uhdr_error_info_t uhdr_hip_idct_upsample_rgb422_dev(uhdr_hip_ctx_t* c, const int16_t* coef_y, const int16_t* coef_cb, const int16_t* coef_cr,
                                                    unsigned int w, unsigned int h, const uint16_t qt_y[64], const uint16_t qt_cb[64],
                                                    const uint16_t qt_cr[64], int variant, uhdr_raw_image_t* rgb) {
  return idct_upsample_rgb_dev("idct_upsample_rgb422", c, coef_y, coef_cb, coef_cr, w, h, (int)(((w + 1) / 2 + 7) / 8), (int)((h + 7) / 8), qt_y, qt_cb,
                               qt_cr, variant, 1, rgb);
}

static uhdr_error_info_t jpeg_decode_rgb_impl(uhdr_hip_ctx_t* c, const uhdr_hip_jpeg_header_t* hdr, const uint8_t* scan_data, size_t scan_bytes,
                                              int out_channels, int variant, uint8_t* rgb, unsigned int stride_px, bool allow_422) {
  const char* name = allow_422 ? "jpeg_decode_rgb_any" : "jpeg_decode_rgb";
  if (!c) return err_status(UHDR_CODEC_INVALID_PARAM, "received nullptr for uhdr_hip context");
  if (!hdr || !scan_data || !rgb) return err_status(UHDR_CODEC_INVALID_PARAM, "received nullptr argument for %s", name);
  if (out_channels != 3 && out_channels != 4) return err_status(UHDR_CODEC_INVALID_PARAM, "out_channels is 3 (RGB888) or 4 (RGBA8888), received %d", out_channels);
  if (variant != 0 && variant != 1) return err_status(UHDR_CODEC_INVALID_PARAM, "unknown libjpeg variant %d", variant);
  uhdr_hip_jpeg_scan_t sc = hdr->scan;
  int mpr = 0, mrows = 0, bpm = 0;
  UHDR_TRY(check_scan(&sc, false, &mpr, &mrows, &bpm));
  if (stride_px < sc.w) return err_status(UHDR_CODEC_INVALID_PARAM, "stride (%u) cannot be less than width (%u)", stride_px, sc.w);
  const bool s444 = sc.num_components == 3 && sc.h_samp[0] == 1 && sc.v_samp[0] == 1 && sc.h_samp[1] == 1 && sc.v_samp[1] == 1 &&
                    sc.h_samp[2] == 1 && sc.v_samp[2] == 1;
  if (s444) {
    uint8_t* planes[3] = {rgb, nullptr, nullptr};
    const unsigned int hs[3] = {stride_px, 0, 0}, vs[3] = {sc.h, 0, 0};
    return jpeg_decode_scan_impl(c, hdr, scan_data, scan_bytes, out_channels, variant, planes, hs, vs);
  }
  const int vsamp = subsampled_vsamp(sc);
  if (vsamp == 0 || (vsamp == 1 && !allow_422))
    return err_status(UHDR_CODEC_UNSUPPORTED_FEATURE, "RGB output on the device takes 4:2:0 or 4:4:4 files; received %d components at %dx%d / %dx%d / %dx%d",
                      sc.num_components, sc.h_samp[0], sc.v_samp[0], sc.h_samp[1], sc.v_samp[1], sc.h_samp[2], sc.v_samp[2]);
  if (sc.blocks_w[1] != sc.blocks_w[2] || sc.blocks_h[1] != sc.blocks_h[2]) return err_status(UHDR_CODEC_UNSUPPORTED_FEATURE, "Cb and Cr block grids differ");
  const DbgClock dbg;
  UHDR_TRY(jpeg_scan_to_coefficients(c, hdr, scan_data, scan_bytes, dbg, sc));
  resident_drop(c, rgb);
  uhdr_raw_image_t img;
  memset(&img, 0, sizeof img);
  img.fmt = out_channels == 3 ? UHDR_IMG_FMT_24bppRGB888 : UHDR_IMG_FMT_32bppRGBA8888;
  img.w = sc.w;
  img.h = sc.h;
  const size_t pitch_px = ((size_t)sc.w + 63) & ~(size_t)63;
  UHDR_TRY(ensure(c->jpg[4], pitch_px * (size_t)out_channels * sc.h));
  img.planes[0] = c->jpg[4].p;
  img.stride[0] = (unsigned int)pitch_px;
  const uint16_t* qt[3] = {hdr->qtable[0], hdr->qtable[1], hdr->qtable[2]};
  UHDR_TRY(idct_upsample_rgb_impl(c, sc.coef, sc.blocks_w, sc.blocks_h, qt, variant, vsamp, &img));
  HIP_TRY(hipMemcpy2DAsync(rgb, (size_t)stride_px * out_channels, c->jpg[4].p, pitch_px * out_channels, (size_t)sc.w * out_channels, sc.h,
                           hipMemcpyDeviceToHost, c->stream));
  HIP_TRY(hipStreamSynchronize(c->stream));
  dbg.mark(vsamp == 1 ? "jpeg_decode_rgb_any: done" : "jpeg_decode_rgb: done");
  return ok_status();
}

static uhdr_error_info_t jpeg_decode_rgb_timed(uhdr_hip_ctx_t* c, const uhdr_hip_jpeg_header_t* hdr, const uint8_t* scan_data, size_t scan_bytes,
                                               int out_channels, int variant, uint8_t* rgb, unsigned int stride_px, bool allow_422) {
  const auto t0 = std::chrono::steady_clock::now();
  const uhdr_error_info_t r = jpeg_decode_rgb_impl(c, hdr, scan_data, scan_bytes, out_channels, variant, rgb, stride_px, allow_422);
  if (c) c->stats.last_jpeg_decode_rgb_ns = (unsigned long long)std::chrono::duration_cast<std::chrono::nanoseconds>(std::chrono::steady_clock::now() - t0).count();
  return r;
}

uhdr_error_info_t uhdr_hip_jpeg_decode_rgb(uhdr_hip_ctx_t* c, const uhdr_hip_jpeg_header_t* hdr, const uint8_t* scan_data, size_t scan_bytes,
                                           int out_channels, int variant, uint8_t* rgb, unsigned int stride_px) {
  return jpeg_decode_rgb_timed(c, hdr, scan_data, scan_bytes, out_channels, variant, rgb, stride_px, false);
}

uhdr_error_info_t uhdr_hip_jpeg_decode_rgb_any(uhdr_hip_ctx_t* c, const uhdr_hip_jpeg_header_t* hdr, const uint8_t* scan_data, size_t scan_bytes,
                                               int out_channels, int variant, uint8_t* rgb, unsigned int stride_px) {
  return jpeg_decode_rgb_timed(c, hdr, scan_data, scan_bytes, out_channels, variant, rgb, stride_px, true);
}

uhdr_error_info_t uhdr_hip_decode_api1_scans_dev(uhdr_hip_ctx_t* c, const uhdr_hip_jpeg_header_t* base, const uint8_t* base_data, size_t base_bytes,
                                                 uhdr_color_gamut_t base_cg, const uhdr_hip_jpeg_header_t* map, const uint8_t* map_data, size_t map_bytes,
                                                 uhdr_color_gamut_t map_cg, int libjpeg_variant, const uhdr_gainmap_metadata_t* md,
                                                 uhdr_color_transfer_t output_ct, uhdr_img_fmt_t output_format, float max_display_boost,
                                                 uhdr_raw_image_t* dest) {
  if (!c) return err_status(UHDR_CODEC_INVALID_PARAM, "received nullptr for uhdr_hip context");
  if (!base || !base_data || !map || !map_data || !md || !dest) return err_status(UHDR_CODEC_INVALID_PARAM, "received nullptr argument for decode_api1_scans");
  if (libjpeg_variant != 0 && libjpeg_variant != 1) return err_status(UHDR_CODEC_INVALID_PARAM, "unknown libjpeg variant %d", libjpeg_variant);
  uhdr_hip_jpeg_scan_t sb = base->scan, sm = map->scan;
  int mpr = 0, mrows = 0, bpm = 0;
  UHDR_TRY(check_scan(&sb, false, &mpr, &mrows, &bpm));
  if (sb.num_components != 3 || sb.h_samp[0] != 2 || sb.v_samp[0] != 2 || sb.h_samp[1] != 1 || sb.v_samp[1] != 1 || sb.h_samp[2] != 1 || sb.v_samp[2] != 1)
    return err_status(UHDR_CODEC_UNSUPPORTED_FEATURE, "decode_api1_scans takes a 4:2:0 base image (the form JpegR writes); decode the scans with uhdr_hip_jpeg_decode_scan");
  UHDR_TRY(check_scan(&sm, false, &mpr, &mrows, &bpm));
  const int nm = sm.num_components;
  if (nm == 3 && (bpm != 3 || memcmp(map->qtable[1], map->qtable[2], sizeof map->qtable[1])))
    return err_status(UHDR_CODEC_UNSUPPORTED_FEATURE, "a three-channel gain map is a 4:4:4 scan with one chroma quantization table here");
  if (base_bytes == 0 || map_bytes == 0 || base_bytes > 0xFFFFFFF0ull || map_bytes > 0xFFFFFFF0ull) return err_status(UHDR_CODEC_INVALID_PARAM, "received no (or too much) entropy-coded data");
  HIP_TRY(hipSetDevice(c->device));
  for (int i = 0; i < 3; i++) {
    UHDR_TRY(ensure(c->jpg[1 + i], (size_t)sb.blocks_w[i] * sb.blocks_h[i] * 128));
    sb.coef[i] = (const int16_t*)c->jpg[1 + i].p;
  }
  size_t off = 0, o_map[3] = {0, 0, 0};
  for (int i = 0; i < nm; i++) { o_map[i] = off; off += ((size_t)sm.blocks_w[i] * sm.blocks_h[i] * 128 + 255) & ~(size_t)255; }
  UHDR_TRY(ensure(c->enc[0], off));
  for (int i = 0; i < nm; i++) sm.coef[i] = (const int16_t*)((const uint8_t*)c->enc[0].p + o_map[i]);
  c->huff_serial_ok = false;
  auto tables_of = [](const uhdr_hip_jpeg_header_t* h) -> const uhdr_hip_huff_tables_t* {
    for (int t = 0; t < 4; t++)
      for (int l = 0; l < 17; l++)
        if (h->tables.bits[t][l]) return &h->tables;
    return nullptr;
  };
  const uhdr_error_info_t hs = uhdr_hip_huffman_decode2_dev(c, &sb, tables_of(base), base_data, base_bytes, &sm, tables_of(map), map_data, map_bytes);
  c->huff_serial_ok = true;
  if (hs.error_code != UHDR_CODEC_OK) return hs;
  uhdr_raw_image_t gm;
  memset(&gm, 0, sizeof gm);
  gm.cg = map_cg;
  gm.ct = UHDR_CT_UNSPECIFIED;
  gm.range = UHDR_CR_FULL_RANGE;
  gm.w = sm.w;
  gm.h = sm.h;
  const size_t pitch_px = ((size_t)sm.w + 63) & ~(size_t)63;
  if (nm == 3) {
    gm.fmt = UHDR_IMG_FMT_32bppRGBA8888;
    UHDR_TRY(ensure(c->jpg[4], pitch_px * 4 * sm.h));
    gm.planes[0] = c->jpg[4].p;
    gm.stride[0] = (unsigned int)pitch_px;
    UHDR_TRY(uhdr_hip_idct_dequant_rgb_dev(c, sm.coef[0], sm.coef[1], sm.coef[2], sm.blocks_w[0], sm.blocks_h[0], map->qtable[0], map->qtable[1], libjpeg_variant, &gm));
  } else {
    gm.fmt = UHDR_IMG_FMT_8bppYCbCr400;
    const size_t pitch = ((size_t)sm.blocks_w[0] * 8 + 63) & ~(size_t)63;
    UHDR_TRY(ensure(c->jpg[4], pitch * (size_t)sm.blocks_h[0] * 8));
    gm.planes[0] = c->jpg[4].p;
    gm.stride[0] = (unsigned int)pitch;
    UHDR_TRY(uhdr_hip_idct_dequant_dev(c, sm.coef[0], sm.blocks_w[0], sm.blocks_h[0], map->qtable[0], (uint8_t*)c->jpg[4].p, pitch));
  }
  uhdr_hip_jpeg_coefficients_t bc;
  memset(&bc, 0, sizeof bc);
  for (int i = 0; i < 3; i++) {
    bc.coef[i] = sb.coef[i];
    bc.blocks_w[i] = sb.blocks_w[i];
    bc.blocks_h[i] = sb.blocks_h[i];
    memcpy(bc.qtable[i], base->qtable[i], sizeof bc.qtable[i]);
  }
  uhdr_error_info_t ap = uhdr_hip_apply_gainmap_coef_dev(c, &bc, sb.w, sb.h, base_cg, &gm, md, output_ct, output_format, max_display_boost, dest);
  if (ap.error_code != UHDR_CODEC_UNSUPPORTED_FEATURE) return ap;
  size_t ppitch[3], poff[3], total = 0;
  for (int i = 0; i < 3; i++) {
    ppitch[i] = ((size_t)sb.blocks_w[i] * 8 + 63) & ~(size_t)63;
    poff[i] = total;
    total += ppitch[i] * (size_t)sb.blocks_h[i] * 8;
  }
  UHDR_TRY(ensure(c->jpg[0], total));
  uhdr_raw_image_t bi;
  memset(&bi, 0, sizeof bi);
  bi.fmt = UHDR_IMG_FMT_12bppYCbCr420;
  bi.cg = base_cg;
  bi.ct = UHDR_CT_SRGB;
  bi.range = UHDR_CR_FULL_RANGE;
  bi.w = sb.w;
  bi.h = sb.h;
  for (int i = 0; i < 3; i++) {
    uint8_t* d = (uint8_t*)c->jpg[0].p + poff[i];
    UHDR_TRY(uhdr_hip_idct_dequant_dev(c, sb.coef[i], sb.blocks_w[i], sb.blocks_h[i], base->qtable[i], d, ppitch[i]));
    bi.planes[i] = d;
    bi.stride[i] = (unsigned int)ppitch[i];
  }
  return uhdr_hip_apply_gainmap_dev(c, &bi, &gm, md, output_ct, output_format, max_display_boost, dest, 0, 0);
}

size_t uhdr_hip_jpeg_assemble(const uhdr_hip_jpeg_scan_t* sc, const uint16_t qt_luma[64], const uint16_t qt_chroma[64], const uint8_t* scan_data,
                              size_t scan_bytes, uint8_t* out, size_t cap) {
  int mpr = 0, mrows = 0, bpm = 0;
  if (check_scan(sc, false, &mpr, &mrows, &bpm).error_code != UHDR_CODEC_OK || !qt_luma || !scan_data || !out) return 0;
  if (sc->num_components > 1 && !qt_chroma) return 0;
  const int nc = sc->num_components, ntab = nc > 1 ? 2 : 1;
  const uint8_t* zz = host::jpeg_zigzag_to_natural();
  std::vector<uint8_t> v;
  v.reserve(scan_bytes + 1024);
  auto put = [&](unsigned b) { v.push_back((uint8_t)b); };
  auto put16 = [&](unsigned x) { put(x >> 8); put(x & 0xff); };
  put(0xff); put(0xd8);
  put(0xff); put(0xe0); put16(16); for (char ch : {'J', 'F', 'I', 'F'}) put((unsigned char)ch); put(0); put(1); put(1); put(0); put16(1); put16(1); put(0); put(0);
  for (int t = 0; t < ntab; t++) {
    const uint16_t* q = t ? qt_chroma : qt_luma;
    put(0xff); put(0xdb); put16(67); put(t);
    for (int i = 0; i < 64; i++) {
      if (q[zz[i]] == 0 || q[zz[i]] > 255) return 0;
      put(q[zz[i]]);
    }
  }
  put(0xff); put(0xc0); put16(8 + 3 * nc); put(8); put16(sc->h); put16(sc->w); put(nc);
  for (int i = 0; i < nc; i++) { put(i + 1); put(((nc == 1 ? 1 : sc->h_samp[i]) << 4) | (nc == 1 ? 1 : sc->v_samp[i])); put(i ? 1 : 0); }
  for (int t = 0; t < ntab; t++) {
    for (int ac = 0; ac < 2; ac++) {
      uint8_t bits[17], vals[256];
      const int nv = host::jpeg_std_huff_table(ac, t, bits, vals);
      put(0xff); put(0xc4); put16(2 + 1 + 16 + nv); put((ac << 4) | t);
      for (int i = 1; i <= 16; i++) put(bits[i]);
      for (int i = 0; i < nv; i++) put(vals[i]);
    }
  }
  if (sc->restart_interval > 0) { put(0xff); put(0xdd); put16(4); put16((unsigned)sc->restart_interval); }
  put(0xff); put(0xda); put16(6 + 2 * nc); put(nc);
  for (int i = 0; i < nc; i++) { put(i + 1); put(i ? 0x11 : 0x00); }
  put(0); put(63); put(0);
  v.insert(v.end(), scan_data, scan_data + scan_bytes);
  put(0xff); put(0xd9);
  if (v.size() > cap) return 0;
  memcpy(out, v.data(), v.size());
  return v.size();
}
```

### libultrahdr_amd/csrc/huffman_decode_sync.hip

```cpp
#include <cstdio>
#include <cstdlib>
#include <cstring>

#include "lds_copy.h"
#include "wg_scan.h"
#include "uhdr_types.h"

namespace uhdr {
namespace {

constexpr int kChunk = 4096;
constexpr int kSyncBlock = 64;

__device__ __forceinline__ uint32_t rst_weight1(uint32_t at) { return (at * 2654435761u + 0x9e3779b9u) | 1u; }
__device__ __forceinline__ uint32_t rst_weight2(uint32_t at) { return ((at ^ (at >> 15)) * 0x85ebca6bu + 0xc2b2ae35u) | 1u; }
__device__ __forceinline__ bool is_stuffed(const uint8_t* __restrict__ d, uint32_t i) { return i > 0 && d[i] == 0 && d[i - 1] == 0xffu; }
__device__ __forceinline__ bool is_rst_first(const uint8_t* __restrict__ d, uint32_t i, uint32_t n) {
  return d[i] == 0xffu && i + 1 < n && (d[i + 1] & 0xf8u) == 0xd0u;
}
template <bool RST>
__device__ __forceinline__ bool is_dropped(const uint8_t* __restrict__ d, uint32_t i, uint32_t n) {
  if (is_stuffed(d, i)) return true;
  if (!RST) return false;
  return is_rst_first(d, i, n) || (i > 0 && (d[i] & 0xf8u) == 0xd0u && d[i - 1] == 0xffu);
}

template <bool RST>
__device__ __forceinline__ uint32_t dropmask16(const uint8_t* __restrict__ data, uint32_t base, uint32_t n) {
  uint32_t m = 0;
  if (base + 17u <= n && base > 0 && ((uintptr_t)(data + base) & 15u) == 0) {
    const uint4 v = *(const uint4*)(data + base);
    const uint32_t w[4] = {v.x, v.y, v.z, v.w};
    uint32_t prev = data[base - 1];
    const uint32_t next = data[base + 16u];
#pragma unroll
    for (uint32_t k = 0; k < 16; k++) {
      const uint32_t cur = (w[k >> 2] >> (8u * (k & 3u))) & 0xffu;
      const uint32_t nx = k < 15 ? (w[(k + 1u) >> 2] >> (8u * ((k + 1u) & 3u))) & 0xffu : next;
      bool drop = cur == 0u && prev == 0xffu;
      if (RST) drop = drop || (cur == 0xffu && (nx & 0xf8u) == 0xd0u) || ((cur & 0xf8u) == 0xd0u && prev == 0xffu);
      m |= drop ? (1u << k) : 0u;
      prev = cur;
    }
  } else {
    for (uint32_t k = 0; k < 16 && base + k < n; k++) m |= is_dropped<RST>(data, base + k, n) ? (1u << k) : 0u;
  }
  return m;
}
template <bool RST>
__global__ __launch_bounds__(256) void unstuff_count_kernel(const uint8_t* __restrict__ data, uint32_t n, uint32_t* __restrict__ counts, const HuffInitFill fill) {
  __shared__ uint32_t s_cnt;
  if (threadIdx.x == 0) s_cnt = 0;
  {
    const uint32_t t = blockIdx.x * 256u + threadIdx.x, nt = gridDim.x * 256u;
    const uint4 z = make_uint4(0, 0, 0, 0), f = make_uint4(0xffffffffu, 0xffffffffu, 0xffffffffu, 0xffffffffu);
    for (uint32_t v = t; v < fill.zero_vec; v += nt) fill.zero_ptr[v] = z;
    for (uint32_t v = t; v < fill.ff_vec; v += nt) fill.ff_ptr[v] = f;
  }
  __syncthreads();
  const uint32_t base = blockIdx.x * kChunk + threadIdx.x * 16;
  const uint32_t c = base < n ? (uint32_t)__builtin_popcount(dropmask16<RST>(data, base, n)) : 0u;
  if (c) atomicAdd(&s_cnt, c);
  __syncthreads();
  if (threadIdx.x == 0) counts[blockIdx.x] = s_cnt;
}
__global__ __launch_bounds__(1024) void sync_scan_kernel(uint32_t* __restrict__ counts, int n, uint32_t* __restrict__ total) {
  __shared__ uint32_t s_w[16];
  const int tid = (int)threadIdx.x;
  const int per = (n + 1023) / 1024, lo = min(tid * per, n), hi = min(lo + per, n);
  uint32_t sum = 0;
  for (int i0 = lo; i0 < hi; i0 += 8) {
    uint32_t v[8];
#pragma unroll
    for (int j = 0; j < 8; j++) v[j] = counts[min(i0 + j, hi - 1)];
#pragma unroll
    for (int j = 0; j < 8; j++) sum += (i0 + j < hi) ? v[j] : 0u;
  }
  uint32_t sc[1] = {sum}, all[1];
  wg_incl_scan<1024, 1>(sc, s_w, all);
  uint32_t run = sc[0] - sum;
  for (int i0 = lo; i0 < hi; i0 += 8) {
    uint32_t v[8];
#pragma unroll
    for (int j = 0; j < 8; j++) v[j] = counts[min(i0 + j, hi - 1)];
#pragma unroll
    for (int j = 0; j < 8; j++) {
      if (i0 + j < hi) counts[i0 + j] = run;
      run += v[j];
    }
  }
  if (tid == 1023 && total) *total = all[0];
}
constexpr int kScanThreads = 256, kScanPer = 8, kScanTile = kScanThreads * kScanPer;
__global__ __launch_bounds__(kScanThreads) void scan_tiles_kernel(uint32_t* __restrict__ v, int n, uint32_t* __restrict__ tile_sum) {
  __shared__ uint32_t s_val[kScanTile];
  __shared__ uint32_t s_w[kScanThreads / 64];
  const int tid = (int)threadIdx.x, base = (int)blockIdx.x * kScanTile;
  uint32_t ld[kScanPer];
#pragma unroll
  for (int j = 0; j < kScanPer; j++) ld[j] = v[min(base + j * kScanThreads + tid, n - 1)];
#pragma unroll
  for (int j = 0; j < kScanPer; j++) s_val[j * kScanThreads + tid] = base + j * kScanThreads + tid < n ? ld[j] : 0u;
  __syncthreads();
  uint32_t x[kScanPer], sum = 0;
#pragma unroll
  for (int j = 0; j < kScanPer; j++) { x[j] = s_val[tid * kScanPer + j]; sum += x[j]; }
  uint32_t sc[1] = {sum}, all[1];
  wg_incl_scan<kScanThreads, 1>(sc, s_w, all);
  uint32_t run = sc[0] - sum;
#pragma unroll
  for (int j = 0; j < kScanPer; j++) { s_val[tid * kScanPer + j] = run; run += x[j]; }
  __syncthreads();
#pragma unroll
  for (int j = 0; j < kScanPer; j++) {
    const int i = base + j * kScanThreads + tid;
    if (i < n) v[i] = s_val[j * kScanThreads + tid];
  }
  if (tid == kScanThreads - 1) tile_sum[blockIdx.x] = all[0];
}
__device__ __forceinline__ uint32_t tile_offset(const HuffSyncArgs& a) {
  const uint32_t tile = (uint32_t)__builtin_amdgcn_readfirstlane((int)((blockIdx.x * blockDim.x) / (uint32_t)kScanTile));
  uint32_t off = 0;
  for (uint32_t t = 0; t < tile; t++) off += a.scan_tmp[t];
  return off;
}
constexpr int kUnstuffSelfPrefix = 4096;
template <bool RST>
__global__ __launch_bounds__(256) void unstuff_compact_kernel(const uint8_t* __restrict__ data, uint32_t n, const uint32_t* __restrict__ chunk_base,
                                                              uint8_t* __restrict__ clean, uint32_t* __restrict__ rst_map, uint32_t* __restrict__ rst_partial,
                                                              uint32_t* __restrict__ total) {
  __shared__ uint32_t s_w[4];
  __shared__ uint32_t s_rst[3];
  const uint32_t tid = threadIdx.x, base = blockIdx.x * kChunk + tid * 16;
  if (RST && tid < 3) s_rst[tid] = 0;
  const uint32_t mask = base < n ? dropmask16<RST>(data, base, n) : 0u;
  const uint32_t c = (uint32_t)__builtin_popcount(mask);
  uint32_t before = 0;
  if (total) {
    uint32_t part[1] = {0}, all[1];
    for (uint32_t i = tid; i < blockIdx.x; i += 256u) part[0] += chunk_base[i];
    wg_incl_scan<256, 1>(part, s_w, all);
    before = all[0];
  } else {
    before = chunk_base[blockIdx.x];
  }
  uint32_t sc[1] = {c}, mine[1];
  wg_incl_scan<256, 1>(sc, s_w, mine);
  if (total && blockIdx.x == gridDim.x - 1 && tid == 0) *total = before + mine[0];
  uint32_t dropped = before + sc[0] - c;
  if (mask == 0 && base + 16u <= n && ((uintptr_t)(data + base) & 15u) == 0) {
    const uint4 v = *(const uint4*)(data + base);
    uint8_t* d = clean + (base - dropped);
    __builtin_memcpy(d, &v.x, 4);
    __builtin_memcpy(d + 4, &v.y, 4);
    __builtin_memcpy(d + 8, &v.z, 4);
    __builtin_memcpy(d + 12, &v.w, 4);
  } else {
// ... 1055 lines not shown
__device__ __forceinline__ void chain_stage_rows(uint8_t (*s_rows)[kMapPitch], int tid, const uint8_t* __restrict__ rows, int first, int n) {
  const int row = tid / 3, part = tid - row * 3;
  uint4 v;
  if (first + row < n) {
    v = *(const uint4*)(rows + (size_t)(first + row) * kHuffHypSlots + part * 16);
  } else {
    const uint32_t b0 = (uint32_t)(16 * part) * 0x01010101u + 0x03020100u;
    v = make_uint4(b0, b0 + 0x04040404u, b0 + 0x08080808u, b0 + 0x0c0c0c0cu);
  }
  uint32_t* d = (uint32_t*)(s_rows[row] + part * 16);
  d[0] = v.x; d[1] = v.y; d[2] = v.z; d[3] = v.w;
}
__device__ __forceinline__ uint32_t chain_step(const uint8_t* row, uint32_t cur) { return cur == 0xffu ? 0xffu : (uint32_t)row[cur]; }

__device__ __forceinline__ void chain_entry_walk(const HuffSyncArgs& a, const uint8_t* __restrict__ tile_map, uint8_t* __restrict__ tile_entry,
                                                 uint8_t (*s_tiles)[kMapPitch], uint8_t (*s_gmap)[kMapPitch], uint32_t* s_gentry ) {
  const int tid = (int)threadIdx.x;
  const uint32_t nclean = a.nbytes - *a.nstuffed, nbits = nclean * 8u;
  const int nlinks = (int)((nbits + a.sub_bits - 1) / a.sub_bits) - 1;
  const int ntiles = (nlinks + kChainTile - 1) / kChainTile;
  const int grp = tid / kHuffHypSlots, s = tid - grp * kHuffHypSlots;
  uint32_t carry = 0;
  for (int c0 = 0; c0 < ntiles; c0 += kChainTile) {
    chain_stage_rows(s_tiles, tid, tile_map, c0, ntiles);
    __syncthreads();
    {
      uint32_t cur = (uint32_t)s;
#pragma unroll
      for (int k = 0; k < kChainGroup; k++) cur = chain_step(s_tiles[grp * kChainGroup + k], cur);
      s_gmap[grp][s] = (uint8_t)cur;
    }
    __syncthreads();
    if (tid == 0) {
      uint32_t c = carry;
      for (int g = 0; g < kChainGroups; g++) {
        s_gentry[g] = c;
        c = chain_step(s_gmap[g], c);
      }
      s_gentry[kChainGroups] = c;
    }
    __syncthreads();
    if (tid < kChainGroups) {
      uint32_t cur = s_gentry[tid];
      for (int k = 0; k < kChainGroup; k++) {
        const int tl = c0 + tid * kChainGroup + k;
        if (tl < ntiles) tile_entry[tl] = (uint8_t)cur;
        cur = chain_step(s_tiles[tid * kChainGroup + k], cur);
      }
    }
    carry = s_gentry[kChainGroups];
    __syncthreads();
  }
}
__global__ __launch_bounds__(kChainWg) void hyp_chain_tiles_kernel(const HuffSyncArgs a, uint8_t* __restrict__ prefix ,
                                                                   uint8_t* __restrict__ tile_map ) {
  __shared__ __attribute__((aligned(16))) uint8_t s_links[kChainTile][kMapPitch];
  __shared__ __attribute__((aligned(16))) uint8_t s_gmap[kChainGroups][kMapPitch];
  __shared__ __attribute__((aligned(16))) uint8_t s_gpre[kChainGroups][kMapPitch];
  const int tid = (int)threadIdx.x;
  const uint32_t nclean = a.nbytes - *a.nstuffed, nbits = nclean * 8u;
  const int nsub = (int)((nbits + a.sub_bits - 1) / a.sub_bits);
  const int nlinks = nsub - 1;
  const int base = (int)blockIdx.x * kChainTile;
  if (base < nlinks) {
    chain_stage_rows(s_links, tid, a.hyp_map, base, nlinks);
    __syncthreads();
    const int grp = tid / kHuffHypSlots, s = tid - grp * kHuffHypSlots;
    {
      uint32_t cur = (uint32_t)s;
#pragma unroll
      for (int k = 0; k < kChainGroup; k++) cur = chain_step(s_links[grp * kChainGroup + k], cur);
      s_gmap[grp][s] = (uint8_t)cur;
    }
    __syncthreads();
    if (tid < kHuffHypSlots) {
      uint32_t c = (uint32_t)tid;
#pragma unroll
      for (int g = 0; g < kChainGroups; g++) {
        s_gpre[g][tid] = (uint8_t)c;
        c = chain_step(s_gmap[g], c);
      }
      tile_map[(size_t)blockIdx.x * kHuffHypSlots + tid] = (uint8_t)c;
    }
    __syncthreads();
    uint32_t cur = s_gpre[grp][s];
#pragma unroll
    for (int k = 0; k < kChainGroup; k++) {
      const int link = grp * kChainGroup + k, i = base + link;
      if (i < nlinks) prefix[(size_t)i * kHuffHypSlots + s] = (uint8_t)cur;
      cur = chain_step(s_links[link], cur);
    }
  }
}
__global__ __launch_bounds__(kChainWg) void hyp_chain_entry_kernel(const HuffSyncArgs a, const uint8_t* __restrict__ tile_map, uint8_t* __restrict__ tile_entry) {
  __shared__ __attribute__((aligned(16))) uint8_t s_tiles[kChainTile][kMapPitch];
  __shared__ __attribute__((aligned(16))) uint8_t s_gmap[kChainGroups][kMapPitch];
  __shared__ uint32_t s_gentry[kChainGroups + 1];
  chain_entry_walk(a, tile_map, tile_entry, s_tiles, s_gmap, s_gentry);
}
__global__ __launch_bounds__(kChainThreads) void hyp_chain_walk_kernel(const HuffSyncArgs a, const uint8_t* __restrict__ prefix,
                                                                       const uint8_t* __restrict__ tile_entry) {
  const int tid = (int)threadIdx.x;
  const uint32_t nclean = a.nbytes - *a.nstuffed, nbits = nclean * 8u;
  const int nsub = (int)((nbits + a.sub_bits - 1) / a.sub_bits);
  const int nlinks = nsub - 1;
  const int i = (int)blockIdx.x * kChainTile + tid;
  bool lost = false;
  if (i < nlinks) {
    uint32_t g = tile_entry[blockIdx.x];
    if (g != 0xffu) g = prefix[(size_t)i * kHuffHypSlots + g];
    if (g == 0xffu) {
      lost = true;
    } else {
      const size_t at = (size_t)i * kHuffHypSlots + g;
      const uint64_t end_i = a.hyp_state[at];
      const uint32_t cnt_next = a.hyp_cnt[at];
      a.state[0][i] = end_i;
      a.nblk[i + 1] = cnt_next;
      if (a.pieces > 1) {
        const uint32_t Q = (uint32_t)a.pieces;
        a.pend[(size_t)i * Q + (Q - 1u)] = end_i;
        const size_t mo = at * (size_t)(Q - 1u);
        uint32_t sum = 0;
        for (uint32_t q = 0; q + 1u < Q; q++) {
          const uint32_t cq = a.mid_cnt[mo + q];
          a.pend[(size_t)(i + 1) * Q + q] = a.mid_state[mo + q];
          a.pcnt[(size_t)(i + 1) * Q + q] = cq;
          sum += cq;
        }
        a.pcnt[(size_t)(i + 1) * Q + (Q - 1u)] = cnt_next - sum;
      }
      if (i == nlinks - 1 && a.hyp_map[at] == 0xffu) lost = true;
    }
  }
  const uint64_t m = __builtin_amdgcn_ballot_w64(lost);
  if (m != 0 && (uint32_t)(tid & 63) == (uint32_t)__builtin_ctzll(m)) atomicOr(a.flags + 2, 1u);
}

__device__ __forceinline__ void dc_block_scan(int v[3], int* s_sum , int) {
  int x[3] = {v[0], v[1], v[2]}, all[3];
  wg_incl_scan<1024, 3>(x, s_sum, all);
  v[0] = x[0]; v[1] = x[1]; v[2] = x[2];
}
__global__ __launch_bounds__(1024) void dc_partial_kernel(const HuffSyncArgs a, int* __restrict__ partial) {
  __shared__ int s_sum[3 * 16];
  const int tid = (int)threadIdx.x;
  const uint32_t t = blockIdx.x * 1024u + (uint32_t)tid;
  int v[3] = {0, 0, 0};
  if (t < a.total_blocks) v[a.comp_of[t % (uint32_t)a.blocks_per_mcu]] = a.dcd[t];
  dc_block_scan(v, s_sum, tid);
  if (tid == 1023) { partial[blockIdx.x * 3] = v[0]; partial[blockIdx.x * 3 + 1] = v[1]; partial[blockIdx.x * 3 + 2] = v[2]; }
}
constexpr int kPlaceChunk = 256;
__device__ __forceinline__ void dc_chunk_scan(int v[3], int* s_sum , int) {
  int x[3] = {v[0], v[1], v[2]}, all[3];
  wg_incl_scan<kPlaceChunk, 3>(x, s_sum, all);
  v[0] = x[0]; v[1] = x[1]; v[2] = x[2];
}
__global__ __launch_bounds__(kPlaceChunk) void dc_partial2_kernel(const HuffSyncArgs a, int* __restrict__ partial) {
  __shared__ int s_sum[3 * (kPlaceChunk / 64)];
  const int tid = (int)threadIdx.x;
  const uint32_t t = blockIdx.x * (uint32_t)kPlaceChunk + (uint32_t)tid;
  int v[3] = {0, 0, 0};
  if (t < a.total_blocks) v[a.comp_of[t % (uint32_t)a.blocks_per_mcu]] = a.coef_scan[(size_t)t * 64];
  dc_chunk_scan(v, s_sum, tid);
  if (tid == kPlaceChunk - 1) { partial[blockIdx.x * 3] = v[0]; partial[blockIdx.x * 3 + 1] = v[1]; partial[blockIdx.x * 3 + 2] = v[2]; }
}
constexpr int kPlaceSelfPrefix = 4096;
__global__ __launch_bounds__(kPlaceChunk) void coef_place_kernel(const HuffSyncArgs a, const int* __restrict__ partial, int self_prefix) {
  __shared__ int s_sum[3 * (kPlaceChunk / 64)];
  __shared__ int16_t s_dc[kPlaceChunk];
  __shared__ uint32_t s_dst[kPlaceChunk];
  __shared__ uint8_t s_inv[64];
  const int tid = (int)threadIdx.x;
  const uint32_t t0 = blockIdx.x * (uint32_t)kPlaceChunk, t = t0 + (uint32_t)tid;
  const uint32_t bpm = (uint32_t)a.blocks_per_mcu;
  if (tid < 64) s_inv[a.zigzag[tid]] = (uint8_t)tid;
  int v[3] = {0, 0, 0};
  int c = 0;
  uint32_t where = 0xffffffffu;
  if (t < a.total_blocks) {
    const uint32_t m = t / bpm, j = t - m * bpm;
    c = a.comp_of[j];
    v[c] = a.coef_scan[(size_t)t * 64];
    const int my = (int)(m / (uint32_t)a.mcus_per_row), mx = (int)(m - (uint32_t)my * (uint32_t)a.mcus_per_row);
    const int jj = (int)j - a.first_blk[c];
    const int by = my * a.vs[c] + jj / a.hs[c], bx = mx * a.hs[c] + jj % a.hs[c];
    if (by < a.bh[c] && bx < a.bw[c]) where = ((uint32_t)c << 30) | ((uint32_t)by * (uint32_t)a.bw[c] + (uint32_t)bx);
  }
  s_dst[tid] = where;
  int carry[3];
  if (self_prefix) {
    int part[3] = {0, 0, 0};
    for (uint32_t i = (uint32_t)tid; i < blockIdx.x; i += (uint32_t)kPlaceChunk) {
      part[0] += partial[i * 3];
      part[1] += partial[i * 3 + 1];
      part[2] += partial[i * 3 + 2];
    }
    wg_incl_scan<kPlaceChunk, 3>(part, s_sum, carry);
  } else {
    carry[0] = partial[blockIdx.x * 3];
    carry[1] = partial[blockIdx.x * 3 + 1];
    carry[2] = partial[blockIdx.x * 3 + 2];
  }
  dc_chunk_scan(v, s_sum, tid);
  s_dc[tid] = (int16_t)((c == 0 ? carry[0] : (c == 1 ? carry[1] : carry[2])) + v[c]);
  __syncthreads();
  const uint32_t lane = (uint32_t)tid & 63u, wv = (uint32_t)tid >> 6;
  const uint32_t half = lane >> 5, n0 = (lane & 31u) * 2u;
  const uint32_t z0 = s_inv[n0], z1 = s_inv[n0 + 1u];
  int16_t* const c0 = a.coef[0];
  int16_t* const c1 = a.coef[1];
  int16_t* const c2 = a.coef[2];
#pragma unroll 4
  for (uint32_t s = 0; s < 32u; s++) {
    const uint32_t loc = wv * 64u + s * 2u + half;
    const uint32_t ent = s_dst[loc];
    if (ent == 0xffffffffu) continue;
    const int16_t* src = a.coef_scan + (size_t)(t0 + loc) * 64;
    uint32_t lo = (uint16_t)src[z0];
    const uint32_t hi = (uint16_t)src[z1];
    if (n0 == 0) lo = (uint16_t)s_dc[loc];
    const uint32_t cc = ent >> 30;
    int16_t* base = cc == 0 ? c0 : (cc == 1 ? c1 : c2);
    uint32_t* dst = (uint32_t*)(base + (size_t)(ent & 0x3fffffffu) * 64);
    dst[lane & 31u] = lo | (hi << 16);
  }
}
__global__ __launch_bounds__(1024) void dc_scan_partials_kernel(int* __restrict__ partial, int nchunks) {
  __shared__ int s_sum[3 * 16];
  const int tid = (int)threadIdx.x;
  const int per = (nchunks + 1023) / 1024, lo = min(tid * per, nchunks), hi = min(lo + per, nchunks);
  int v[3] = {0, 0, 0};
  for (int i = lo; i < hi; i++)
    for (int c = 0; c < 3; c++) v[c] += partial[i * 3 + c];
  int own[3] = {v[0], v[1], v[2]};
  dc_block_scan(v, s_sum, tid);
  int run[3] = {v[0] - own[0], v[1] - own[1], v[2] - own[2]};
  for (int i = lo; i < hi; i++)
    for (int c = 0; c < 3; c++) {
      const int x = partial[i * 3 + c];
      partial[i * 3 + c] = run[c];
      run[c] += x;
    }
}
__global__ __launch_bounds__(1024) void dc_apply_kernel(const HuffSyncArgs a, const int* __restrict__ partial) {
  __shared__ int s_sum[3 * 16];
  const int tid = (int)threadIdx.x;
  const uint32_t t = blockIdx.x * 1024u + (uint32_t)tid;
  const uint32_t bpm = (uint32_t)a.blocks_per_mcu;
  int v[3] = {0, 0, 0};
  int c = 0;
  uint32_t m = 0, j = 0;
  if (t < a.total_blocks) {
    m = t / bpm;
    j = t - m * bpm;
    c = a.comp_of[j];
    v[c] = a.dcd[t];
  }
  dc_block_scan(v, s_sum, tid);
  if (t >= a.total_blocks) return;
  const int dc = partial[blockIdx.x * 3 + c] + v[c];
  if (a.rst_map) {
    a.dcd[t] = dc;
    if ((t + 1u) % a.rst_blocks == 0 && t + 1u < a.total_blocks) {
      int* g = a.dc_seg + (size_t)((t + 1u) / a.rst_blocks) * 3;
      for (int cc = 0; cc < 3; cc++) g[cc] = partial[blockIdx.x * 3 + cc] + v[cc];
    }
    return;
  }
  const int my = (int)(m / (uint32_t)a.mcus_per_row), mx = (int)(m - (uint32_t)my * (uint32_t)a.mcus_per_row);
  const int jj = (int)j - a.first_blk[c];
  const int by = my * a.vs[c] + jj / a.hs[c], bx = mx * a.hs[c] + jj % a.hs[c];
  if (by < a.bh[c] && bx < a.bw[c]) a.coef[c][((size_t)by * a.bw[c] + bx) * 64] = (int16_t)dc;
}
__global__ __launch_bounds__(256) void dc_restart_kernel(const HuffSyncArgs a) {
  if (blockIdx.x == 0) {
    __shared__ uint32_t s_acc[3];
    if (threadIdx.x < 3) s_acc[threadIdx.x] = 0;
    __syncthreads();
    uint32_t v[3] = {0, 0, 0};
    for (uint32_t i = threadIdx.x; i < a.rst_chunks; i += 256u)
      for (int k = 0; k < 3; k++) v[k] += a.rst_partial[i * 3 + k];
    for (int k = 0; k < 3; k++)
      if (v[k]) atomicAdd(&s_acc[k], v[k]);
    __syncthreads();
    if (threadIdx.x == 0) { a.flags[9] = s_acc[0]; a.flags[16] = s_acc[1]; a.flags[17] = s_acc[2]; }
  }
  const uint32_t t = blockIdx.x * 256u + threadIdx.x;
  if (t >= a.total_blocks) return;
  const uint32_t bpm = (uint32_t)a.blocks_per_mcu;
  const uint32_t m = t / bpm, j = t - m * bpm, seg = t / a.rst_blocks;
  const int c = a.comp_of[j];
  const int dc = a.dcd[t] - (seg ? a.dc_seg[(size_t)seg * 3 + c] : 0);
  const int my = (int)(m / (uint32_t)a.mcus_per_row), mx = (int)(m - (uint32_t)my * (uint32_t)a.mcus_per_row);
  const int jj = (int)j - a.first_blk[c];
  const int by = my * a.vs[c] + jj / a.hs[c], bx = mx * a.hs[c] + jj % a.hs[c];
  if (by < a.bh[c] && bx < a.bw[c]) a.coef[c][((size_t)by * a.bw[c] + bx) * 64] = (int16_t)dc;
}

}

static void launch_write(const HuffSyncArgs& a, uint32_t nsub, int final_buf, hipStream_t s) {
  const size_t per_wave = (size_t)64 * ((a.sub_bits >> 3) + 4) + 64;
  const int waves = per_wave * 4 <= (20u << 10) ? 4 : (per_wave * 2 <= (20u << 10) ? 2 : 1);
  const size_t lds = per_wave * waves;
  const int threads = 64 * waves;
  const int grid = (int)((nsub + threads - 1) / threads);
  if (lds > (20u << 10)) (void)hipFuncSetAttribute((const void*)sync_write_kernel, hipFuncAttributeMaxDynamicSharedMemorySize, (int)lds);
  hipLaunchKernelGGL(sync_write_kernel, dim3(grid), dim3(threads), lds, s, a, final_buf);
}

int huff_sync_chunks(uint64_t nbytes) { return (int)((nbytes + kChunk - 1) / kChunk); }

namespace {
__global__ __launch_bounds__(256) void stray_marker_kernel(const uint8_t* __restrict__ data, uint32_t n, uint32_t* __restrict__ flag) {
  const uint32_t base = (blockIdx.x * 256u + threadIdx.x) * 16u;
  if (base >= n) return;
  bool found = false;
  if (base + 17u <= n && ((uintptr_t)(data + base) & 15u) == 0) {
    const uint4 v = *(const uint4*)(data + base);
    const uint32_t w[5] = {v.x, v.y, v.z, v.w, (uint32_t)data[base + 16u]};
#pragma unroll
    for (uint32_t i = 0; i < 16; i++) {
      const uint32_t c0 = (w[i >> 2] >> (8u * (i & 3u))) & 0xffu, c1 = (w[(i + 1u) >> 2] >> (8u * ((i + 1u) & 3u))) & 0xffu;
      found = found || (c0 == 0xffu && c1 != 0u && c1 != 0xffu && (c1 & 0xf8u) != 0xd0u);
    }
  } else {
    for (uint32_t i = base; i < base + 16u && i + 1u < n; i++) {
      const uint32_t c0 = data[i], c1 = data[i + 1u];
      found = found || (c0 == 0xffu && c1 != 0u && c1 != 0xffu && (c1 & 0xf8u) != 0xd0u);
    }
  }
  if (found) *(volatile uint32_t*)flag = 1u;
}
}
hipError_t launch_stray_marker_check(const uint8_t* data, uint32_t nbytes, uint32_t* flag, hipStream_t s) {
  const int grid = (int)((nbytes + 4095u) / 4096u);
  hipLaunchKernelGGL(stray_marker_kernel, dim3(grid), dim3(256), 0, s, data, nbytes, flag);
  return hipGetLastError();
}

hipError_t launch_huffman_unstuff(const uint8_t* data, uint32_t nbytes, uint32_t* chunk_counts, uint32_t* nstuffed_dev, uint8_t* clean, hipStream_t s,
                                  uint32_t* rst_map, uint32_t* rst_partial, const HuffInitFill* fill) {
  const int nchunks = huff_sync_chunks(nbytes);
  HuffInitFill f;
  memset(&f, 0, sizeof f);
  if (fill) f = *fill;
  if (rst_map) hipLaunchKernelGGL(unstuff_count_kernel<true>, dim3(nchunks), dim3(256), 0, s, data, nbytes, chunk_counts, f);
  else hipLaunchKernelGGL(unstuff_count_kernel<false>, dim3(nchunks), dim3(256), 0, s, data, nbytes, chunk_counts, f);
  uint32_t* total = nstuffed_dev;
  if (nchunks > kUnstuffSelfPrefix) {
    hipLaunchKernelGGL(sync_scan_kernel, dim3(1), dim3(1024), 0, s, chunk_counts, nchunks, nstuffed_dev);
    total = nullptr;
  }
  if (rst_map) hipLaunchKernelGGL(unstuff_compact_kernel<true>, dim3(nchunks), dim3(256), 0, s, data, nbytes, (const uint32_t*)chunk_counts, clean, rst_map, rst_partial, total);
  else hipLaunchKernelGGL(unstuff_compact_kernel<false>, dim3(nchunks), dim3(256), 0, s, data, nbytes, (const uint32_t*)chunk_counts, clean, rst_map, rst_partial, total);
  return hipGetLastError();
}
static void launch_write2(const HuffSyncArgs& a, uint32_t nsub, int final_buf, hipStream_t s) {
  const size_t per_wave = (size_t)64 * ((a.sub_bits >> 3) + 4) + 64;
  const int waves = per_wave * 4 <= (20u << 10) ? 4 : (per_wave * 2 <= (20u << 10) ? 2 : 1);
  const size_t lds = sizeof(Write2Lds) + per_wave * waves;
  const int threads = 64 * waves;
  const int grid = (int)((nsub + threads - 1) / threads);
  static size_t opted = 0;
  if (lds > opted) {
    (void)hipFuncSetAttribute((const void*)sync_write2_kernel, hipFuncAttributeMaxDynamicSharedMemorySize, (int)lds);
    opted = lds;
  }
  hipLaunchKernelGGL(sync_write2_kernel, dim3(grid), dim3(threads), lds, s, a, final_buf);
}
static void launch_place(const HuffSyncArgs& a, int* dc_partial, hipStream_t s) {
  const int nch = (int)((a.total_blocks + kPlaceChunk - 1) / kPlaceChunk);
  hipLaunchKernelGGL(dc_partial2_kernel, dim3(nch), dim3(kPlaceChunk), 0, s, a, dc_partial);
  const int self_prefix = nch <= kPlaceSelfPrefix ? 1 : 0;
  if (!self_prefix) hipLaunchKernelGGL(dc_scan_partials_kernel, dim3(1), dim3(1024), 0, s, dc_partial, nch);
  hipLaunchKernelGGL(coef_place_kernel, dim3(nch), dim3(kPlaceChunk), 0, s, a, (const int*)dc_partial, self_prefix);
}
int huff_place_chunk() { return kPlaceChunk; }
static void launch_dc(const HuffSyncArgs& a, int* dc_partial, hipStream_t s) {
  const int nch = (int)((a.total_blocks + 1023) / 1024);
  hipLaunchKernelGGL(dc_partial_kernel, dim3(nch), dim3(1024), 0, s, a, dc_partial);
  hipLaunchKernelGGL(dc_scan_partials_kernel, dim3(1), dim3(1024), 0, s, dc_partial, nch);
  hipLaunchKernelGGL(dc_apply_kernel, dim3(nch), dim3(1024), 0, s, a, (const int*)dc_partial);
  if (a.rst_map) hipLaunchKernelGGL(dc_restart_kernel, dim3((a.total_blocks + 255) / 256), dim3(256), 0, s, a);
}

uint32_t huff_sync_max_subsequences(uint64_t nbytes, uint32_t sub_bits) { return (uint32_t)((nbytes * 8 + sub_bits - 1) / sub_bits); }

hipError_t launch_huffman_decode_sync(const HuffSyncArgs& a, int max_rounds, int* dc_partial, int* final_buf, hipStream_t s) {
  const uint32_t nsub = huff_sync_max_subsequences(a.nbytes, a.sub_bits);
  const int grid = (int)((nsub + kSyncBlock - 1) / kSyncBlock);
  const size_t lds = (size_t)kSyncBlock * ((a.sub_bits >> 3) + 4) + 64;
  for (int r = 0; r <= max_rounds; r++) hipLaunchKernelGGL(sync_round_kernel, dim3(grid), dim3(kSyncBlock), lds, s, a, r);
  *final_buf = 0;
  {
    const int nt = (int)((nsub + kScanTile - 1) / kScanTile);
    hipLaunchKernelGGL(scan_tiles_kernel, dim3(nt), dim3(kScanThreads), 0, s, a.nblk, (int)nsub, a.scan_tmp);
  }
  if (a.coef_scan && !a.rst_map) {
    launch_write2(a, nsub, *final_buf, s);
    launch_place(a, dc_partial, s);
  } else {
    launch_write(a, nsub, *final_buf, s);
    launch_dc(a, dc_partial, s);
  }
  return hipGetLastError();
}

size_t huff_hyp_chain_bytes(uint64_t nbytes, uint32_t sub_bits, size_t* tiles_offset) {
  const size_t nsub = huff_sync_max_subsequences(nbytes, sub_bits), ntiles = (nsub + kChainTile - 1) / kChainTile;
  const size_t pre = ntiles * kChainThreads * kHuffHypSlots;
  if (tiles_offset) *tiles_offset = pre;
  return pre + ntiles * kHuffHypSlots + ((ntiles + 255) & ~(size_t)255);
}

hipError_t launch_huffman_decode_hyp(const HuffSyncArgs& a, int* dc_partial, uint8_t* chain_prefix, uint8_t* chain_tiles, hipStream_t s) {
  const uint32_t nsub = huff_sync_max_subsequences(a.nbytes, a.sub_bits);
  const int grid = (int)((nsub + 63) / 64);
  const int threads = 64 * a.hyp_h;
  const size_t lds0 = (size_t)64 * ((a.sub_bits >> 3) + 4) + 64;
  const size_t lds1_stage = ((((size_t)(64 + a.hyp_levels) * ((a.sub_bits >> 3) + 4) + 16 + 7) >> 2) + 1 & ~(size_t)1) * 4;
  const size_t lds1 = lds1_stage + (size_t)threads * 10 + 16;
  {
    static size_t opted = 0;
    if (lds1 + sizeof(PairLds) + 64 > (64u << 10) && lds1 > opted) {
      const hipError_t e1 = hipFuncSetAttribute((const void*)hyp_pass1q_kernel, hipFuncAttributeMaxDynamicSharedMemorySize, (int)lds1);
      if (e1 != hipSuccess) return e1;
      opted = lds1;
    }
  }
  const bool dbg = getenv("UHDR_HIP_HUFF_DEBUG") != nullptr;
  hipEvent_t ev[9];
  int nev = 0;
  auto mark = [&]() {
    if (dbg && nev < 9) {
      (void)hipEventCreate(&ev[nev]);
      (void)hipEventRecord(ev[nev], s);
      nev++;
    }
  };
  mark();
  static const bool qmerge = !(getenv("UHDR_HIP_HUFF_QMERGE") && atoi(getenv("UHDR_HIP_HUFF_QMERGE")) == 0);
  static const bool no_fused = getenv("UHDR_HIP_HUFF_NO_FUSED_PASSES") != nullptr;
  const size_t lds01 = (((((size_t)64 * ((a.sub_bits >> 3) + 4) + 16 + 7) >> 2) + 1) & ~(size_t)1) * 4 + (size_t)64 * a.hyp_h * 8 + (size_t)threads * 2 + 16;
  if (qmerge && !no_fused && a.hyp_main_levels == 1 && a.hyp_levels > 1 && !a.rst_map && lds01 + sizeof(PairLds) + 64 <= (64u << 10)) {
    hipLaunchKernelGGL(hyp_pass01_kernel, dim3((nsub + kFusedStride - 1) / kFusedStride), dim3(threads), lds01, s, a);
    mark();
  } else {
    hipLaunchKernelGGL(hyp_pass0_kernel, dim3(grid), dim3(threads), lds0, s, a);
    mark();
    if (qmerge) hipLaunchKernelGGL(hyp_pass1q_kernel, dim3(grid), dim3(threads), lds1, s, a);
    else hipLaunchKernelGGL(hyp_pass1_kernel, dim3(grid), dim3(threads), lds1, s, a);
  }
  {
    const hipError_t e1 = hipGetLastError();
    if (e1 != hipSuccess) return e1;
  }
  if (qmerge && a.hyp_main_levels > 0 && a.hyp_main_levels < a.hyp_levels) {
    static const int smul = [] { const char* e = getenv("UHDR_HIP_HUFF_STRAG_MUL"); const int v = e ? atoi(e) : 1; return v >= 1 && v <= 16 ? v : 1; }();
    int sgrid = (int)((nsub * (uint32_t)a.hyp_h / 16u + kStragWaves - 1) / kStragWaves) * smul;
    if (sgrid < 64) sgrid = 64;
    if (sgrid > 4096) sgrid = 4096;
    hipLaunchKernelGGL(hyp_straggler_kernel, dim3(sgrid), dim3(64 * kStragWaves), 0, s, a);
  }
  mark();
  const int ntiles = (int)((nsub + kChainTile - 1) / kChainTile);
  uint8_t* chain_entry = chain_tiles + (size_t)ntiles * kHuffHypSlots;
  hipLaunchKernelGGL(hyp_chain_tiles_kernel, dim3(ntiles), dim3(kChainWg), 0, s, a, chain_prefix, chain_tiles);
  hipLaunchKernelGGL(hyp_chain_entry_kernel, dim3(1), dim3(kChainWg), 0, s, a, (const uint8_t*)chain_tiles, chain_entry);
  hipLaunchKernelGGL(hyp_chain_walk_kernel, dim3(ntiles), dim3(kChainThreads), 0, s, a, (const uint8_t*)chain_prefix, (const uint8_t*)chain_entry);
  mark();
  HuffSyncArgs w = a;
  uint32_t nw = nsub;
  if (a.pieces > 1 && a.coef_scan && !a.rst_map) {
    w.sub_bits = a.sub_bits / (uint32_t)a.pieces;
    w.state[0] = a.pend;
    w.nblk = a.pcnt;
    nw = nsub * (uint32_t)a.pieces;
  }
  {
    const int nt = (int)((nw + kScanTile - 1) / kScanTile);
    hipLaunchKernelGGL(scan_tiles_kernel, dim3(nt), dim3(kScanThreads), 0, s, w.nblk, (int)nw, w.scan_tmp);
  }
  mark();
  if (a.coef_scan && !a.rst_map) {
    launch_write2(w, nw, 0, s);
    mark();
    launch_place(a, dc_partial, s);
  } else {
    launch_write(a, nsub, 0, s);
    mark();
    launch_dc(a, dc_partial, s);
  }
  mark();
  if (dbg) {
    (void)hipStreamSynchronize(s);
    static const char* names[] = {"pass0", "pass1 (+ stragglers)", "chain x3", "nblk scan", "write", "dc x3 / place", "-"};
    fprintf(stderr, "uhdr_hip: hypothesis decode kernels:");
    for (int i = 0; i + 1 < nev; i++) {
      float ms = 0;
      (void)hipEventElapsedTime(&ms, ev[i], ev[i + 1]);
      fprintf(stderr, " %s %.0f us,", names[i], ms * 1e3f);
    }
    fprintf(stderr, "\n");
    for (int i = 0; i < nev; i++) (void)hipEventDestroy(ev[i]);
  }
  return hipGetLastError();
}

}
```

### libultrahdr_amd/csrc/idct_core.h

```cpp
#pragma once
#include "uhdr_types.h"

namespace uhdr {
namespace idct {

#define FIX_0_298631336 2446
#define FIX_0_390180644 3196
#define FIX_0_541196100 4433
#define FIX_0_765366865 6270
#define FIX_0_899976223 7373
#define FIX_1_175875602 9633
#define FIX_1_501321110 12299
#define FIX_1_847759065 15137
#define FIX_1_961570560 16069
#define FIX_2_053119869 16819
#define FIX_2_562915447 20995
#define FIX_3_072711026 25172

template <bool M24>
__device__ __forceinline__ int mulc(int a, int c) {
  if constexpr (M24) return __mul24(a, c);
  else return (int)((uint32_t)a * (uint32_t)c);
}
template <int PASS, bool M24>
__device__ __forceinline__ void idct_1d(const int in[8], int out[8]) {
  constexpr int sh = PASS == 0 ? 13 - 2 : 13 + 2 + 3;
  constexpr uint32_t fudge = (1u << (sh - 1)) + (PASS == 1 ? (512u << 18) : 0u);
  int z2 = in[2], z3 = in[6];
  int z1 = mulc<M24>(z2 + z3, FIX_0_541196100);
  int tmp2 = z1 + mulc<M24>(z3, -FIX_1_847759065);
  int tmp3 = z1 + mulc<M24>(z2, FIX_0_765366865);
  z2 = in[0]; z3 = in[4];
  int tmp0 = (int)(((uint32_t)(z2 + z3) << 13) + fudge);
  int tmp1 = (int)(((uint32_t)(z2 - z3) << 13) + fudge);
  const int tmp10 = tmp0 + tmp3, tmp13 = tmp0 - tmp3, tmp11 = tmp1 + tmp2, tmp12 = tmp1 - tmp2;
  tmp0 = in[7]; tmp1 = in[5]; tmp2 = in[3]; tmp3 = in[1];
  z1 = tmp0 + tmp3; z2 = tmp1 + tmp2; z3 = tmp0 + tmp2;
  int z4 = tmp1 + tmp3;
  const int z5 = mulc<M24>(z3 + z4, FIX_1_175875602);
  tmp0 = mulc<M24>(tmp0, FIX_0_298631336);
  tmp1 = mulc<M24>(tmp1, FIX_2_053119869);
  tmp2 = mulc<M24>(tmp2, FIX_3_072711026);
  tmp3 = mulc<M24>(tmp3, FIX_1_501321110);
  z1 = mulc<M24>(z1, -FIX_0_899976223);
  z2 = mulc<M24>(z2, -FIX_2_562915447);
  z3 = mulc<M24>(z3, -FIX_1_961570560);
  z4 = mulc<M24>(z4, -FIX_0_390180644);
  z3 += z5; z4 += z5;
  tmp0 += z1 + z3; tmp1 += z2 + z4; tmp2 += z2 + z3; tmp3 += z1 + z4;
  const int sum[8] = {tmp10 + tmp3, tmp11 + tmp2, tmp12 + tmp1, tmp13 + tmp0, tmp13 - tmp0, tmp12 - tmp1, tmp11 - tmp2, tmp10 - tmp3};
#pragma unroll
  for (int k = 0; k < 8; k++) {
    if constexpr (PASS == 0) {
      out[k] = sum[k] >> sh;
    } else {
      const int t = (int)(((uint32_t)sum[k] >> 18) & 1023u) - 384;
      out[k] = min(max(t, 0), 255);
    }
  }
}

__device__ __forceinline__ void load_dequant_row(const int16_t* __restrict__ coef, int bw, int by, int bx, int rr,
                                                 const int q[8], int v[8], int& big, bool row_ok = true) {
  if (bx < bw && row_ok) {
    const uint4 raw = *(const uint4*)(coef + ((size_t)by * bw + bx) * 64 + rr * 8);
    const uint32_t w4[4] = {raw.x, raw.y, raw.z, raw.w};
#pragma unroll
    for (int c = 0; c < 4; c++) {
      v[2 * c] = __mul24((int)(int16_t)(w4[c] & 0xffff), q[2 * c]);
      v[2 * c + 1] = __mul24((int)(int16_t)(w4[c] >> 16), q[2 * c + 1]);
    }
    const int mx = max(max(max(v[0], v[1]), max(v[2], v[3])), max(max(v[4], v[5]), max(v[6], v[7])));
    const int mn = min(min(min(v[0], v[1]), min(v[2], v[3])), min(min(v[4], v[5]), min(v[6], v[7])));
    big |= (int)(mx > 8191) | (int)(mn < -8191);
  } else {
#pragma unroll
    for (int c = 0; c < 8; c++) v[c] = 0;
  }
}

__device__ __forceinline__ void idct_wave(int* ws, const int v[8], int big, int rr, int rb, uint32_t s[8]) {
  const int cb = rr, cc = rb;
  const bool fast = __builtin_amdgcn_ballot_w64(big != 0) == 0;
#pragma unroll
  for (int c = 0; c < 8; c++) ws[rb * 72 + rr * 9 + c] = v[c];
  __builtin_amdgcn_wave_barrier();
  __builtin_amdgcn_s_waitcnt(0xc07f);
  int in[8], out[8];
#pragma unroll
  for (int r = 0; r < 8; r++) in[r] = ws[cb * 72 + r * 9 + cc];
  if (fast) idct_1d<0, true>(in, out); else idct_1d<0, false>(in, out);
  __builtin_amdgcn_wave_barrier();
#pragma unroll
  for (int r = 0; r < 8; r++) ws[cb * 72 + r * 9 + cc] = out[r];
  __builtin_amdgcn_wave_barrier();
  __builtin_amdgcn_s_waitcnt(0xc07f);
#pragma unroll
  for (int c = 0; c < 8; c++) in[c] = ws[rb * 72 + rr * 9 + c];
  if (fast) idct_1d<1, true>(in, out); else idct_1d<1, false>(in, out);
#pragma unroll
  for (int c = 0; c < 8; c++) s[c] = (uint32_t)out[c];
  __builtin_amdgcn_wave_barrier();
}

}
}
```

### libultrahdr_amd/csrc/uhdr_types.h

```cpp
#pragma once
#include <hip/hip_runtime.h>
#include <stdint.h>

#include "device_math.h"
#include "uhdr_hip.h"

namespace uhdr {

struct ImageView {
  const void* p[3];
  uint32_t stride[3];
  uint32_t w, h;
  int fmt;
  int range;
};
struct ImageViewMut {
  void* p[3];
  uint32_t stride[3];
  uint32_t w, h;
  int fmt;
  int range;
};

constexpr int kSrgbN = 1024;
// ... 168 lines not shown
struct YuvXformParams {
  ImageViewMut img;
  Mat3 c;
};
struct RgbToYcbcrParams {
  ImageView src;
  ImageViewMut dst;
  Rgb2Yuv k;
};

hipError_t launch_apply_gainmap(const ApplyParams& p, hipStream_t s);
hipError_t launch_apply_gainmap_coef(const ApplyParams& p, hipStream_t s);
int apply_quad_mode(const ApplyParams& p);
hipError_t launch_generate_gainmap(const GenParams& p, bool two_pass, hipStream_t s);
hipError_t launch_affine_map(const AffineParams& p, hipStream_t s);
hipError_t launch_minmax_table(const MinmaxTableParams& p, hipStream_t s);
hipError_t launch_map_blocks(const float* ratio, const AffineDev* dev, const double* math_tab, int nch, int bw, int bh, const uint16_t* qt_luma,
                             const uint16_t* qt_chroma, int16_t* const coef[3], uint8_t* map_out, uint32_t out_stride, hipStream_t s);
hipError_t launch_base_blocks(const ImageView& yuv420, const Mat3* c, const uint16_t* qt_luma, const uint16_t* qt_chroma, int16_t* const coef[3],
                              hipStream_t s);
hipError_t launch_selftest(int which, unsigned long long* out, uint32_t arg0, uint32_t arg1, uint32_t seed, const double* math_tab, const AffineDev* dev,
                           hipStream_t s);
int gen_partials_count(const GenParams& p);
hipError_t launch_encode_api0_fused(const FusedParams& p, bool two_pass, int* grid_out, hipStream_t s);
hipError_t launch_tone_map(const ToneMapParams& p, hipStream_t s);
hipError_t launch_transform_yuv(const YuvXformParams& p, hipStream_t s);
hipError_t launch_rgb_to_ycbcr(const RgbToYcbcrParams& p, hipStream_t s);
struct FdctEdge {
  int on, w, h, col_mode, fill, mcu_rows;
};
hipError_t launch_fdct_quant(const uint8_t* plane, size_t stride, int bw, int bh,
                             const uint16_t* qt_host, int16_t* coef, hipStream_t s, const FdctEdge* edge = nullptr);

hipError_t launch_fdct_quant_rgb(const uint8_t* rgb, size_t pitch, int bpp, int bw, int bh, const uint16_t* qt_luma_host,
                                 const uint16_t* qt_chroma_host, int16_t* coef_y, int16_t* coef_cb, int16_t* coef_cr, hipStream_t s, int vw = 0,
                                 int vh = 0);
hipError_t launch_repack(int mode, const void* src, size_t src_pitch, void* dst, size_t dst_pitch, uint32_t w, uint32_t h,
                         hipStream_t s);
struct EffectPlane {
  const void* src;
  void* dst;
  uint32_t elem;
  uint32_t src_w, src_h, src_stride;
  uint32_t dst_w, dst_h, dst_stride;
  uint32_t mode;
  uint32_t a0, a1;
};
hipError_t launch_effect_plane(const EffectPlane& p, hipStream_t s);

struct HuffArgs {
  const int16_t* coef[3];
  int bw[3], bh[3];
  int hs[3], vs[3];
  int ncomp;
  int mcus_per_row, total_mcus;
  int ri;
  int blocks_per_mcu;
  int nseg;
  const uint32_t* tables;
  const uint8_t* zigzag;
  uint8_t* slots;
  uint32_t slot_stride;
  uint32_t* seg_bytes;
};
uint32_t huff_slot_stride();
struct HuffStream {
  uint32_t* seg_bits;
  uint64_t* seg_start;
  uint32_t* raw;
  uint64_t raw_words;
  uint32_t* meta;
  uint32_t* slots;
};
int huff_stream_segment_mcus(int blocks_per_mcu);
size_t huff_stream_slot_bytes(int nseg);
int huff_stuff_chunks(uint64_t raw_bytes);
hipError_t launch_huffman_encode_stream(const HuffArgs& a, const HuffStream& t, uint32_t* chunk_counts, uint64_t* out_bytes, uint8_t* out, uint64_t cap,
                                        hipStream_t s);
hipError_t launch_huffman_encode(const HuffArgs& a, uint64_t* offsets, uint32_t* status, uint8_t* out, uint64_t cap, hipStream_t s);

struct HuffDecTable {
  uint16_t lut[512];
  int maxcode[18];
  int valoff[17];
  uint8_t vals[256];
};
struct HuffDecArgs {
  const uint8_t* data;
  uint32_t nbytes;
  const uint32_t* starts;
  const uint32_t* ends;
  int nseg, ri, total_mcus, mcus_per_row, ncomp;
  int bw[3], bh[3], hs[3], vs[3];
  int16_t* coef[3];
  const HuffDecTable* tabs;
  const uint8_t* zigzag;
  uint32_t* status;
};
constexpr int kHuffL2Max = 16;
struct HuffFastTable {
  uint16_t l1[512];
  uint16_t l2[kHuffL2Max][128];
};
constexpr int kHuffValWords = 512 + kHuffL2Max * 128;
constexpr int kHuffPairBits = 10, kHuffPairWords = 1 << kHuffPairBits;
constexpr int kHuffL2Total = 32;
constexpr int kHuffPairBlobWords = 4 * kHuffPairWords + kHuffL2Total * 128 / 2;
constexpr int kHuffPairValBlobWords = 8 * kHuffPairWords + kHuffL2Total * 128 / 2;
struct HuffSyncArgs {
  const uint8_t* clean;
  uint32_t nbytes;
  const uint32_t* nstuffed;
  uint32_t sub_bits;
  uint64_t* state[2];
  uint8_t* changed[2];
  uint32_t* nblk;
  uint32_t* scan_tmp;
  uint32_t* flags;
  int* dcd;
  uint32_t total_blocks;
  int blocks_per_mcu, ncomp, mcus_per_row;
  int bw[3], bh[3], hs[3], vs[3], first_blk[3];
  uint8_t comp_of[16];
  int16_t* coef[3];
  const HuffFastTable* ftabs;
  const HuffFastTable* ttabs;
  const uint32_t* vtabs;
  const uint32_t* ptabs;
  const uint32_t* pvtabs;
  const uint8_t* zigzag;
  int hyp_h, hyp_levels;
  uint64_t* hyp_state;
  uint8_t* hyp_map;
  uint16_t* hyp_cnt;
  int hyp_hist;
  int hyp_main_levels;
  int strag_levels;
  uint32_t* strag_list;
  uint32_t strag_cap;
  int16_t* coef_scan;
  uint4* zero_ptr;
  uint32_t zero_vec;
  int pieces;
  uint64_t* mid_state;
  uint16_t* mid_cnt;
  uint64_t* pend;
  uint32_t* pcnt;
  const uint32_t* rst_map;
  uint32_t rst_blocks;
  int* dc_seg;
  uint32_t* rst_partial;
  uint32_t rst_chunks;
};
constexpr int kHuffHypSlots = 48;
constexpr int kHuffFlagStragglers = 20;
constexpr int kHuffFlagStray = 21;
size_t huff_hyp_chain_bytes(uint64_t nbytes, uint32_t sub_bits, size_t* tiles_offset);
hipError_t launch_huffman_decode_hyp(const HuffSyncArgs& a, int* dc_partial, uint8_t* chain_prefix, uint8_t* chain_tiles, hipStream_t s);
int huff_sync_chunks(uint64_t nbytes);
uint32_t huff_sync_max_subsequences(uint64_t nbytes, uint32_t sub_bits);
struct HuffInitFill {
  uint4* zero_ptr;
  uint32_t zero_vec;
  uint4* ff_ptr;
  uint32_t ff_vec;
};
hipError_t launch_huffman_unstuff(const uint8_t* data, uint32_t nbytes, uint32_t* chunk_counts, uint32_t* nstuffed_dev, uint8_t* clean, hipStream_t s,
                                  uint32_t* rst_map, uint32_t* rst_partial, const HuffInitFill* fill = nullptr);
hipError_t launch_huffman_decode_sync(const HuffSyncArgs& a, int max_rounds, int* dc_partial, int* final_buf, hipStream_t s);
void launch_profile_mark(hipStream_t s);
int huff_marker_chunks(uint64_t nbytes);
int huff_place_chunk();
hipError_t launch_stray_marker_check(const uint8_t* data, uint32_t nbytes, uint32_t* flag, hipStream_t s);
hipError_t launch_huffman_decode(const HuffDecArgs& a, uint32_t* counts, uint32_t* starts, uint32_t* ends, hipStream_t s);

hipError_t launch_idct_dequant(const int16_t* coef, int bw, int bh, const uint16_t* qt_host, uint8_t* plane,
                               size_t stride, hipStream_t s);
hipError_t launch_idct_dequant_rgb(const int16_t* coef_y, const int16_t* coef_cb, const int16_t* coef_cr, int bw, int bh,
                                   const uint16_t* qt_luma_host, const uint16_t* qt_chroma_host, int variant,
                                   const ImageViewMut& rgb, hipStream_t s);
size_t upsample_scratch_bytes(const int bw[3], const int bh[3]);
hipError_t launch_idct_upsample_rgb(const int16_t* const coef[3], const int bw[3], const int bh[3], const uint16_t* const qt_host[3],
                                    int variant, int vsamp, const ImageViewMut& rgb, uint8_t* chroma_scratch, hipStream_t s);
hipError_t launch_jpeg_rgb_to_ycc(const ImageView& rgb, const ImageViewMut& ycc, hipStream_t s);
hipError_t launch_jpeg_ycc_to_rgb(const ImageView& ycc, const ImageViewMut& rgb, int variant, hipStream_t s);

}
```

Baseline: 12020 Mpixels/s.

## Fuse IDCT and color conversion into Huffman coefficient placement via sample sinks

Adds a sample-sink path so the final coefficient-placement kernel after Huffman decoding writes IDCT'd samples directly. Base planes get planar Y/Cb/Cr, and the 3-channel gain map gets packed RGB/RGBA. This skips writing the natural-order coefficient buffers and the separate IDCT/dequant launches, cutting a full coefficient round trip through HBM. In exchange, the base image no longer takes the fused coefficient-domain applyGainMap path and instead goes through the sample-based fallback. Chunk size drops to 240 for RGB placement, and an env var can disable either sink.

```diff
diff --git a/libultrahdr_amd/csrc/api_context.cpp b/libultrahdr_amd/csrc/api_context.cpp
--- a/libultrahdr_amd/csrc/api_context.cpp
+++ b/libultrahdr_amd/csrc/api_context.cpp
@@ -565,6 +565,10 @@
     c->huff_two_pass = e && atoi(e) != 0;
     e = getenv("UHDR_HIP_HUFF_ROUTE_LOG");
     c->huff_route_log = e && atoi(e) != 0;
+    e = getenv("UHDR_HIP_DECODE_COEF_TAIL");
+    const int tail = e ? atoi(e) : 0;
+    c->coef_tail_base = tail != 0 && tail != 3;
+    c->coef_tail_map = tail != 0 && tail != 2;
   }
   e = hipStreamCreateWithFlags(&c->own_stream, hipStreamNonBlocking);
   if (e != hipSuccess) { delete c; return fail("hipStreamCreate", e); }
diff --git a/libultrahdr_amd/csrc/api_entropy.cpp b/libultrahdr_amd/csrc/api_entropy.cpp
--- a/libultrahdr_amd/csrc/api_entropy.cpp
+++ b/libultrahdr_amd/csrc/api_entropy.cpp
@@ -347,6 +347,12 @@
 
 uhdr_error_info_t uhdr_hip_huffman_decode_dev(uhdr_hip_ctx_t* c, const uhdr_hip_jpeg_scan_t* sc, const uhdr_hip_huff_tables_t* tables,
                                               const uint8_t* data, size_t data_bytes) {
+  return huffman_decode_sink_dev(c, sc, tables, data, data_bytes, nullptr, nullptr);
+}
+
+uhdr_error_info_t uhdr_api::huffman_decode_sink_dev(uhdr_hip_ctx* c, const uhdr_hip_jpeg_scan_t* sc, const uhdr_hip_huff_tables_t* tables, const uint8_t* data,
+                                                    size_t data_bytes, const HuffSampleSink* sink, bool* wrote_samples) {
+  if (wrote_samples) *wrote_samples = false;
   if (!c) return err_status(UHDR_CODEC_INVALID_PARAM, "received nullptr for uhdr_hip context");
   if (!data || data_bytes == 0 || data_bytes > 0xFFFFFFF0ull) return err_status(UHDR_CODEC_INVALID_PARAM, "received no (or more than 4 GiB of) entropy-coded data");
   int mpr = 0, mrows = 0, bpm = 0;
@@ -507,7 +513,7 @@
     const size_t zero_bytes_sync = off - o_flags;
     const size_t o_s0 = take((size_t)nsub * 8), o_hm = use_hyp ? take((size_t)nsub * kHuffHypSlots) : 0;
     const size_t ff_bytes = off - o_s0;
-    const size_t o_s1 = take((size_t)nsub * 8), o_c0 = take(nsub), o_c1 = take(nsub), o_dcp = take((size_t)((total_blocks + 255) / 256) * 12 + 16),
+    const size_t o_s1 = take((size_t)nsub * 8), o_c0 = take(nsub), o_c1 = take(nsub), o_dcp = take((size_t)((total_blocks + (uint32_t)huff_place_chunk() - 1) / (uint32_t)huff_place_chunk()) * 12 + 16),
                  o_ft = take(sizeof(HuffFastTable) * 8),
                  o_st = take(((size_t)nsub / 2048 + 2) * 4), o_vt = take((size_t)4 * kHuffValWords * 4);
     const size_t o_hs = use_hyp ? take((size_t)nsub * kHuffHypSlots * 8) : 0, o_hc = use_hyp ? take((size_t)nsub * kHuffHypSlots * 2) : 0;
@@ -571,6 +577,7 @@
       y.strag_cap = nsub * (uint32_t)bpm;
     }
     if (form2) y.coef_scan = (int16_t*)(sb + o_cs);
+    const HuffSampleSink* const use_sink = form2 && sink && sink->kind != 0 ? sink : nullptr;
     const int main_levels_env = [&] { const char* e = getenv("UHDR_HIP_HUFF_MAIN_LEVELS"); return e ? atoi(e) : (sparse ? 1 : 2); }();
     if (j == bpm && bpm <= 16) {
       const bool fills_in_unstuff = attempts[0].levels > 0 && zero_bytes_sync % 16 == 0 && ff_bytes % 16 == 0 && zero_bytes_sync / 16 < 0xFFFFFFFFull &&
@@ -644,7 +651,7 @@
               HIP_TRY(launch_huffman_unstuff(data, (uint32_t)data_bytes, (uint32_t*)(sb + o_cnt), y.flags + 8, sb + o_clean, c->stream, rst_map, y.rst_partial,
                                              fills_in_unstuff && ti == 0 ? &init_fill : nullptr));
             unstuffed = true;
-            HIP_TRY(launch_huffman_decode_hyp(y, (int*)(sb + o_dcp), sb + o_ch, sb + o_ch + tiles_off, c->stream));
+            HIP_TRY(launch_huffman_decode_hyp(y, (int*)(sb + o_dcp), sb + o_ch, sb + o_ch + tiles_off, c->stream, use_sink));
           }
           dbg.mark("huffman_decode_dev: hypothesis attempt enqueued");
           HIP_TRY(hipMemcpyAsync(fl, y.flags, 24 * sizeof(uint32_t), hipMemcpyDeviceToHost, c->stream));
@@ -671,7 +678,7 @@
             ProfScope ps(c, "huffman_decode");
             if (!unstuffed) HIP_TRY(launch_huffman_unstuff(data, (uint32_t)data_bytes, (uint32_t*)(sb + o_cnt), y.flags + 8, sb + o_clean, c->stream, rst_map, y.rst_partial));
             unstuffed = true;
-            HIP_TRY(launch_huffman_decode_sync(y, max_rounds, (int*)(sb + o_dcp), &final_buf, c->stream));
+            HIP_TRY(launch_huffman_decode_sync(y, max_rounds, (int*)(sb + o_dcp), &final_buf, c->stream, use_sink));
           }
           HIP_TRY(hipMemcpyAsync(fl, y.flags, 24 * sizeof(uint32_t), hipMemcpyDeviceToHost, c->stream));
           HIP_TRY(wait_stream(c));
@@ -689,6 +696,7 @@
         if (fl[1] & 8u) return err_status(UHDR_CODEC_INVALID_PARAM, "corrupt entropy-coded data (the scan ends before its last block)");
         if (fl[1] & 2u) return err_status(UHDR_CODEC_INVALID_PARAM, "corrupt entropy-coded data (undefined Huffman code or a run past the end of a block)");
         sync_done = true;
+        if (wrote_samples) *wrote_samples = use_sink != nullptr;
       } else {
         if (a.nseg == 1 && !c->huff_serial_ok && data_bytes > (256u << 10)) {
           c->stats.entropy_decode_declined++;
@@ -883,6 +891,15 @@
 uhdr_error_info_t uhdr_hip_huffman_decode2_dev(uhdr_hip_ctx_t* c, const uhdr_hip_jpeg_scan_t* scan_a, const uhdr_hip_huff_tables_t* tables_a, const uint8_t* data_a,
                                                size_t bytes_a, const uhdr_hip_jpeg_scan_t* scan_b, const uhdr_hip_huff_tables_t* tables_b,
                                                const uint8_t* data_b, size_t bytes_b) {
+  return huffman_decode2_sink_dev(c, scan_a, tables_a, data_a, bytes_a, nullptr, nullptr, scan_b, tables_b, data_b, bytes_b, nullptr, nullptr);
+}
+
+uhdr_error_info_t uhdr_api::huffman_decode2_sink_dev(uhdr_hip_ctx* c, const uhdr_hip_jpeg_scan_t* scan_a, const uhdr_hip_huff_tables_t* tables_a, const uint8_t* data_a,
+                                                     size_t bytes_a, const HuffSampleSink* sink_a, bool* samples_a, const uhdr_hip_jpeg_scan_t* scan_b,
+                                                     const uhdr_hip_huff_tables_t* tables_b, const uint8_t* data_b, size_t bytes_b, const HuffSampleSink* sink_b,
+                                                     bool* samples_b) {
+  if (samples_a) *samples_a = false;
+  if (samples_b) *samples_b = false;
   if (!c) return err_status(UHDR_CODEC_INVALID_PARAM, "received nullptr for uhdr_hip context");
   HIP_TRY(hipSetDevice(c->device));
   uhdr_hip_ctx* x = nullptr;
@@ -892,8 +909,8 @@
   HIP_TRY(hipStreamWaitEvent(x->stream, c->aux_ev, 0));
   uhdr_error_info_t ra = ok_status(), rb = ok_status();
   const int dev = c->device;
-  run_pair(c, [&] { ra = uhdr_hip_huffman_decode_dev(c, scan_a, tables_a, data_a, bytes_a); },
-           [&, dev] { (void)hipSetDevice(dev); rb = uhdr_hip_huffman_decode_dev(x, scan_b, tables_b, data_b, bytes_b); });
+  run_pair(c, [&] { ra = huffman_decode_sink_dev(c, scan_a, tables_a, data_a, bytes_a, sink_a, samples_a); },
+           [&, dev] { (void)hipSetDevice(dev); rb = huffman_decode_sink_dev(x, scan_b, tables_b, data_b, bytes_b, sink_b, samples_b); });
   aux_merge(c);
   return ra.error_code != UHDR_CODEC_OK ? ra : rb;
 }
diff --git a/libultrahdr_amd/csrc/api_internal.h b/libultrahdr_amd/csrc/api_internal.h
--- a/libultrahdr_amd/csrc/api_internal.h
+++ b/libultrahdr_amd/csrc/api_internal.h
@@ -102,6 +102,7 @@
   bool huff_serial_ok = true;
   DeviceBuf huff_slots;
   bool huff_two_pass = false;
+  bool coef_tail_base = false, coef_tail_map = false;
   bool huff_route_log = false;
   size_t huff_slots_refused = 0;
   DeviceBuf enc[3];
@@ -244,6 +245,12 @@
 void aux_merge(uhdr_hip_ctx* c);
 bool aux_post(uhdr_hip_ctx* c, std::function<void()> job);
 void aux_wait(uhdr_hip_ctx* c);
+uhdr_error_info_t huffman_decode_sink_dev(uhdr_hip_ctx* c, const uhdr_hip_jpeg_scan_t* sc, const uhdr_hip_huff_tables_t* tables, const uint8_t* data,
+                                          size_t data_bytes, const HuffSampleSink* sink, bool* wrote_samples);
+uhdr_error_info_t huffman_decode2_sink_dev(uhdr_hip_ctx* c, const uhdr_hip_jpeg_scan_t* scan_a, const uhdr_hip_huff_tables_t* tables_a, const uint8_t* data_a,
+                                           size_t bytes_a, const HuffSampleSink* sink_a, bool* samples_a, const uhdr_hip_jpeg_scan_t* scan_b,
+                                           const uhdr_hip_huff_tables_t* tables_b, const uint8_t* data_b, size_t bytes_b, const HuffSampleSink* sink_b,
+                                           bool* samples_b);
 }
 using namespace uhdr_api;
 
diff --git a/libultrahdr_amd/csrc/api_jpeg.cpp b/libultrahdr_amd/csrc/api_jpeg.cpp
--- a/libultrahdr_amd/csrc/api_jpeg.cpp
+++ b/libultrahdr_amd/csrc/api_jpeg.cpp
@@ -1192,9 +1192,14 @@
         if (h->tables.bits[t][l]) return &h->tables;
     return nullptr;
   };
-  const uhdr_error_info_t hs = uhdr_hip_huffman_decode2_dev(c, &sb, tables_of(base), base_data, base_bytes, &sm, tables_of(map), map_data, map_bytes);
-  c->huff_serial_ok = true;
-  if (hs.error_code != UHDR_CODEC_OK) return hs;
+  size_t ppitch[3], poff[3], total = 0;
+  for (int i = 0; i < 3; i++) {
+    ppitch[i] = ((size_t)sb.blocks_w[i] * 8 + 63) & ~(size_t)63;
+    poff[i] = total;
+    total += ppitch[i] * (size_t)sb.blocks_h[i] * 8;
+  }
+  const bool base_sink = !c->coef_tail_base && ppitch[0] <= 0xFFFFFFFFull;
+  if (base_sink) UHDR_TRY(ensure(c->jpg[0], total));
   uhdr_raw_image_t gm;
   memset(&gm, 0, sizeof gm);
   gm.cg = map_cg;
@@ -1203,37 +1208,61 @@
   gm.w = sm.w;
   gm.h = sm.h;
   const size_t pitch_px = ((size_t)sm.w + 63) & ~(size_t)63;
+  const size_t pitch_y = ((size_t)sm.blocks_w[0] * 8 + 63) & ~(size_t)63;
   if (nm == 3) {
     gm.fmt = UHDR_IMG_FMT_32bppRGBA8888;
     UHDR_TRY(ensure(c->jpg[4], pitch_px * 4 * sm.h));
-    gm.planes[0] = c->jpg[4].p;
     gm.stride[0] = (unsigned int)pitch_px;
-    UHDR_TRY(uhdr_hip_idct_dequant_rgb_dev(c, sm.coef[0], sm.coef[1], sm.coef[2], sm.blocks_w[0], sm.blocks_h[0], map->qtable[0], map->qtable[1], libjpeg_variant, &gm));
   } else {
     gm.fmt = UHDR_IMG_FMT_8bppYCbCr400;
-    const size_t pitch = ((size_t)sm.blocks_w[0] * 8 + 63) & ~(size_t)63;
-    UHDR_TRY(ensure(c->jpg[4], pitch * (size_t)sm.blocks_h[0] * 8));
-    gm.planes[0] = c->jpg[4].p;
-    gm.stride[0] = (unsigned int)pitch;
-    UHDR_TRY(uhdr_hip_idct_dequant_dev(c, sm.coef[0], sm.blocks_w[0], sm.blocks_h[0], map->qtable[0], (uint8_t*)c->jpg[4].p, pitch));
-  }
-  uhdr_hip_jpeg_coefficients_t bc;
-  memset(&bc, 0, sizeof bc);
-  for (int i = 0; i < 3; i++) {
-    bc.coef[i] = sb.coef[i];
-    bc.blocks_w[i] = sb.blocks_w[i];
-    bc.blocks_h[i] = sb.blocks_h[i];
-    memcpy(bc.qtable[i], base->qtable[i], sizeof bc.qtable[i]);
-  }
-  uhdr_error_info_t ap = uhdr_hip_apply_gainmap_coef_dev(c, &bc, sb.w, sb.h, base_cg, &gm, md, output_ct, output_format, max_display_boost, dest);
-  if (ap.error_code != UHDR_CODEC_UNSUPPORTED_FEATURE) return ap;
-  size_t ppitch[3], poff[3], total = 0;
-  for (int i = 0; i < 3; i++) {
-    ppitch[i] = ((size_t)sb.blocks_w[i] * 8 + 63) & ~(size_t)63;
-    poff[i] = total;
-    total += ppitch[i] * (size_t)sb.blocks_h[i] * 8;
-  }
-  UHDR_TRY(ensure(c->jpg[0], total));
+    UHDR_TRY(ensure(c->jpg[4], pitch_y * (size_t)sm.blocks_h[0] * 8));
+    gm.stride[0] = (unsigned int)pitch_y;
+  }
+  gm.planes[0] = c->jpg[4].p;
+  HuffSampleSink kb, km;
+  memset(&kb, 0, sizeof kb);
+  memset(&km, 0, sizeof km);
+  if (base_sink) {
+    kb.kind = 1;
+    for (int i = 0; i < 3; i++) {
+      kb.plane[i] = (uint8_t*)c->jpg[0].p + poff[i];
+      kb.pitch[i] = (uint32_t)ppitch[i];
+      for (int k = 0; k < 64; k++) kb.q[i][k] = base->qtable[i][k];
+    }
+  }
+  if (!c->coef_tail_map && pitch_px * 4 <= 0xFFFFFFFFull) {
+    km.kind = nm == 3 ? 2 : 1;
+    km.bpp = 4;
+    km.plane[0] = (uint8_t*)c->jpg[4].p;
+    km.pitch[0] = (uint32_t)(nm == 3 ? pitch_px * 4 : pitch_y);
+    km.w = sm.w;
+    km.h = sm.h;
+    huff_sink_set_variant(&km, libjpeg_variant);
+    for (int i = 0; i < nm; i++)
+      for (int k = 0; k < 64; k++) km.q[i][k] = map->qtable[i][k];
+  }
+  bool base_samples = false, map_samples = false;
+  const uhdr_error_info_t hs = huffman_decode2_sink_dev(c, &sb, tables_of(base), base_data, base_bytes, kb.kind ? &kb : nullptr, &base_samples, &sm, tables_of(map),
+                                                        map_data, map_bytes, km.kind ? &km : nullptr, &map_samples);
+  c->huff_serial_ok = true;
+  if (hs.error_code != UHDR_CODEC_OK) return hs;
+  if (!map_samples) {
+    if (nm == 3) UHDR_TRY(uhdr_hip_idct_dequant_rgb_dev(c, sm.coef[0], sm.coef[1], sm.coef[2], sm.blocks_w[0], sm.blocks_h[0], map->qtable[0], map->qtable[1], libjpeg_variant, &gm));
+    else UHDR_TRY(uhdr_hip_idct_dequant_dev(c, sm.coef[0], sm.blocks_w[0], sm.blocks_h[0], map->qtable[0], (uint8_t*)c->jpg[4].p, pitch_y));
+  }
+  if (!base_samples) {
+    uhdr_hip_jpeg_coefficients_t bc;
+    memset(&bc, 0, sizeof bc);
+    for (int i = 0; i < 3; i++) {
+      bc.coef[i] = sb.coef[i];
+      bc.blocks_w[i] = sb.blocks_w[i];
+      bc.blocks_h[i] = sb.blocks_h[i];
+      memcpy(bc.qtable[i], base->qtable[i], sizeof bc.qtable[i]);
+    }
+    uhdr_error_info_t ap = uhdr_hip_apply_gainmap_coef_dev(c, &bc, sb.w, sb.h, base_cg, &gm, md, output_ct, output_format, max_display_boost, dest);
+    if (ap.error_code != UHDR_CODEC_UNSUPPORTED_FEATURE) return ap;
+    UHDR_TRY(ensure(c->jpg[0], total));
+  }
   uhdr_raw_image_t bi;
   memset(&bi, 0, sizeof bi);
   bi.fmt = UHDR_IMG_FMT_12bppYCbCr420;
@@ -1244,7 +1273,7 @@
   bi.h = sb.h;
   for (int i = 0; i < 3; i++) {
     uint8_t* d = (uint8_t*)c->jpg[0].p + poff[i];
-    UHDR_TRY(uhdr_hip_idct_dequant_dev(c, sb.coef[i], sb.blocks_w[i], sb.blocks_h[i], base->qtable[i], d, ppitch[i]));
+    if (!base_samples) UHDR_TRY(uhdr_hip_idct_dequant_dev(c, sb.coef[i], sb.blocks_w[i], sb.blocks_h[i], base->qtable[i], d, ppitch[i]));
     bi.planes[i] = d;
     bi.stride[i] = (unsigned int)ppitch[i];
   }
diff --git a/libultrahdr_amd/csrc/huffman_decode_sync.hip b/libultrahdr_amd/csrc/huffman_decode_sync.hip
--- a/libultrahdr_amd/csrc/huffman_decode_sync.hip
+++ b/libultrahdr_amd/csrc/huffman_decode_sync.hip
@@ -2,7 +2,9 @@
 #include <cstdlib>
 #include <cstring>
 
+#include "idct_core.h"
 #include "lds_copy.h"
+#include "upsample_core.h"
 #include "wg_scan.h"
 #include "uhdr_types.h"
 
@@ -1364,41 +1366,40 @@
   if (tid == 1023) { partial[blockIdx.x * 3] = v[0]; partial[blockIdx.x * 3 + 1] = v[1]; partial[blockIdx.x * 3 + 2] = v[2]; }
 }
 constexpr int kPlaceChunk = 256;
+constexpr int kPlaceChunkRgb = 240;
 __device__ __forceinline__ void dc_chunk_scan(int v[3], int* s_sum , int) {
   int x[3] = {v[0], v[1], v[2]}, all[3];
   wg_incl_scan<kPlaceChunk, 3>(x, s_sum, all);
   v[0] = x[0]; v[1] = x[1]; v[2] = x[2];
 }
-__global__ __launch_bounds__(kPlaceChunk) void dc_partial2_kernel(const HuffSyncArgs a, int* __restrict__ partial) {
+__global__ __launch_bounds__(kPlaceChunk) void dc_partial2_kernel(const HuffSyncArgs a, int* __restrict__ partial, uint32_t chunk) {
   __shared__ int s_sum[3 * (kPlaceChunk / 64)];
   const int tid = (int)threadIdx.x;
-  const uint32_t t = blockIdx.x * (uint32_t)kPlaceChunk + (uint32_t)tid;
+  const uint32_t t = blockIdx.x * chunk + (uint32_t)tid;
   int v[3] = {0, 0, 0};
-  if (t < a.total_blocks) v[a.comp_of[t % (uint32_t)a.blocks_per_mcu]] = a.coef_scan[(size_t)t * 64];
+  if ((uint32_t)tid < chunk && t < a.total_blocks) v[a.comp_of[t % (uint32_t)a.blocks_per_mcu]] = a.coef_scan[(size_t)t * 64];
   dc_chunk_scan(v, s_sum, tid);
   if (tid == kPlaceChunk - 1) { partial[blockIdx.x * 3] = v[0]; partial[blockIdx.x * 3 + 1] = v[1]; partial[blockIdx.x * 3 + 2] = v[2]; }
 }
 constexpr int kPlaceSelfPrefix = 4096;
-__global__ __launch_bounds__(kPlaceChunk) void coef_place_kernel(const HuffSyncArgs a, const int* __restrict__ partial, int self_prefix) {
-  __shared__ int s_sum[3 * (kPlaceChunk / 64)];
-  __shared__ int16_t s_dc[kPlaceChunk];
-  __shared__ uint32_t s_dst[kPlaceChunk];
-  __shared__ uint8_t s_inv[64];
+template <bool XY>
+__device__ __forceinline__ void place_prologue(const HuffSyncArgs& a, const int* __restrict__ partial, int self_prefix, uint32_t chunk, int* s_sum,
+                                               int16_t* s_dc, uint32_t* s_dst) {
   const int tid = (int)threadIdx.x;
-  const uint32_t t0 = blockIdx.x * (uint32_t)kPlaceChunk, t = t0 + (uint32_t)tid;
+  const uint32_t t = blockIdx.x * chunk + (uint32_t)tid;
   const uint32_t bpm = (uint32_t)a.blocks_per_mcu;
-  if (tid < 64) s_inv[a.zigzag[tid]] = (uint8_t)tid;
   int v[3] = {0, 0, 0};
   int c = 0;
   uint32_t where = 0xffffffffu;
-  if (t < a.total_blocks) {
+  if ((uint32_t)tid < chunk && t < a.total_blocks) {
     const uint32_t m = t / bpm, j = t - m * bpm;
     c = a.comp_of[j];
     v[c] = a.coef_scan[(size_t)t * 64];
     const int my = (int)(m / (uint32_t)a.mcus_per_row), mx = (int)(m - (uint32_t)my * (uint32_t)a.mcus_per_row);
     const int jj = (int)j - a.first_blk[c];
     const int by = my * a.vs[c] + jj / a.hs[c], bx = mx * a.hs[c] + jj % a.hs[c];
-    if (by < a.bh[c] && bx < a.bw[c]) where = ((uint32_t)c << 30) | ((uint32_t)by * (uint32_t)a.bw[c] + (uint32_t)bx);
+    if (by < a.bh[c] && bx < a.bw[c])
+      where = ((uint32_t)c << 30) | (XY ? ((uint32_t)by << 15) | (uint32_t)bx : (uint32_t)by * (uint32_t)a.bw[c] + (uint32_t)bx);
   }
   s_dst[tid] = where;
   int carry[3];
@@ -1418,6 +1419,16 @@
   dc_chunk_scan(v, s_sum, tid);
   s_dc[tid] = (int16_t)((c == 0 ? carry[0] : (c == 1 ? carry[1] : carry[2])) + v[c]);
   __syncthreads();
+}
+__global__ __launch_bounds__(kPlaceChunk) void coef_place_kernel(const HuffSyncArgs a, const int* __restrict__ partial, int self_prefix) {
+  __shared__ int s_sum[3 * (kPlaceChunk / 64)];
+  __shared__ int16_t s_dc[kPlaceChunk];
+  __shared__ uint32_t s_dst[kPlaceChunk];
+  __shared__ uint8_t s_inv[64];
+  const int tid = (int)threadIdx.x;
+  const uint32_t t0 = blockIdx.x * (uint32_t)kPlaceChunk;
+  if (tid < 64) s_inv[a.zigzag[tid]] = (uint8_t)tid;
+  place_prologue<false>(a, partial, self_prefix, (uint32_t)kPlaceChunk, s_sum, s_dc, s_dst);
   const uint32_t lane = (uint32_t)tid & 63u, wv = (uint32_t)tid >> 6;
   const uint32_t half = lane >> 5, n0 = (lane & 31u) * 2u;
   const uint32_t z0 = s_inv[n0], z1 = s_inv[n0 + 1u];
@@ -1439,6 +1450,111 @@
     dst[lane & 31u] = lo | (hi << 16);
   }
 }
+constexpr int kZzPitch = 72;
+__device__ __forceinline__ void gather_dequant_row(const uint4 raw, int16_t* zz , const uint32_t zp[8], int rr, int dc, const uint16_t* q_row ,
+                                                   int v[8], int& big) {
+  *(uint4*)(zz + rr * 8) = raw;
+  __builtin_amdgcn_wave_barrier();
+  __builtin_amdgcn_s_waitcnt(0xc07f);
+  uint32_t c16[8];
+#pragma unroll
+  for (int c = 0; c < 8; c++) c16[c] = (uint16_t)zz[zp[c]];
+  __builtin_amdgcn_wave_barrier();
+  if (rr == 0) c16[0] = (uint16_t)dc;
+  const uint32_t w4[4] = {c16[0] | (c16[1] << 16), c16[2] | (c16[3] << 16), c16[4] | (c16[5] << 16), c16[6] | (c16[7] << 16)};
+  const uint4 qr = *(const uint4*)q_row;
+  const int q[8] = {(int)(qr.x & 0xffff), (int)(qr.x >> 16), (int)(qr.y & 0xffff), (int)(qr.y >> 16),
+                    (int)(qr.z & 0xffff), (int)(qr.z >> 16), (int)(qr.w & 0xffff), (int)(qr.w >> 16)};
+  idct::dequant_row(w4, q, v, big);
+}
+__global__ __launch_bounds__(kPlaceChunk) void sample_place_planar_kernel(const HuffSyncArgs a, const int* __restrict__ partial, int self_prefix,
+                                                                          const HuffSampleSink k) {
+  __shared__ int s_sum[3 * (kPlaceChunk / 64)];
+  __shared__ int16_t s_dc[kPlaceChunk];
+  __shared__ uint32_t s_dst[kPlaceChunk];
+  __shared__ uint8_t s_inv[64];
+  __shared__ __attribute__((aligned(16))) uint16_t s_q[3][64];
+  __shared__ int s_ws[kPlaceChunk / 64][8 * 8 * 9];
+  __shared__ __attribute__((aligned(16))) int16_t s_zz[kPlaceChunk / 64][8][kZzPitch];
+  const int tid = (int)threadIdx.x;
+  const uint32_t t0 = blockIdx.x * (uint32_t)kPlaceChunk;
+  if (tid < 64) s_inv[a.zigzag[tid]] = (uint8_t)tid;
+  if (tid < 192) s_q[tid >> 6][tid & 63] = k.q[tid >> 6][tid & 63];
+  place_prologue<true>(a, partial, self_prefix, (uint32_t)kPlaceChunk, s_sum, s_dc, s_dst);
+  const int lane = tid & 63, wv = tid >> 6, rr = lane >> 3, rb = lane & 7;
+  int* ws = s_ws[wv];
+  int16_t* zz = s_zz[wv][rb];
+  uint32_t zp[8];
+#pragma unroll
+  for (int c = 0; c < 8; c++) zp[c] = s_inv[rr * 8 + c];
+  for (int step = 0; step < 8; step++) {
+    const uint32_t loc = (uint32_t)(wv * 64 + step * 8 + rb);
+    const uint32_t ent = s_dst[loc];
+    const bool real = ent != 0xffffffffu;
+    const uint32_t cc = real ? ent >> 30 : 0u;
+    int v[8] = {0, 0, 0, 0, 0, 0, 0, 0};
+    int big = 0;
+    if (real) gather_dequant_row(*(const uint4*)(a.coef_scan + (size_t)(t0 + loc) * 64 + rr * 8), zz, zp, rr, s_dc[loc], &s_q[cc][rr * 8], v, big);
+    uint32_t s[8];
+    idct::idct_wave(ws, v, big, rr, rb, s);
+    if (real) {
+      const uint32_t by = (ent >> 15) & 0x7fffu, bx = ent & 0x7fffu;
+      uint8_t* const plane = cc == 0 ? k.plane[0] : (cc == 1 ? k.plane[1] : k.plane[2]);
+      const uint32_t pitch = cc == 0 ? k.pitch[0] : (cc == 1 ? k.pitch[1] : k.pitch[2]);
+      const uint32_t lo = s[0] | (s[1] << 8) | (s[2] << 16) | (s[3] << 24);
+      const uint32_t hi = s[4] | (s[5] << 8) | (s[6] << 16) | (s[7] << 24);
+      *(uint2*)(plane + (size_t)(by * 8u + (uint32_t)rr) * pitch + (size_t)bx * 8u) = make_uint2(lo, hi);
+    }
+  }
+}
+template <int BPP>
+__global__ __launch_bounds__(kPlaceChunk) void sample_place_rgb_kernel(const HuffSyncArgs a, const int* __restrict__ partial, int self_prefix,
+                                                                       const HuffSampleSink k) {
+  __shared__ int s_sum[3 * (kPlaceChunk / 64)];
+  __shared__ int16_t s_dc[kPlaceChunk];
+  __shared__ uint32_t s_dst[kPlaceChunk];
+  __shared__ uint8_t s_inv[64];
+  __shared__ __attribute__((aligned(16))) uint16_t s_q[3][64];
+  __shared__ int s_ws[kPlaceChunk / 64][8 * 8 * 9];
+  __shared__ __attribute__((aligned(16))) int16_t s_zz[kPlaceChunk / 64][8][kZzPitch];
+  const int tid = (int)threadIdx.x;
+  const uint32_t t0 = blockIdx.x * (uint32_t)kPlaceChunkRgb;
+  if (tid < 64) s_inv[a.zigzag[tid]] = (uint8_t)tid;
+  if (tid < 192) s_q[tid >> 6][tid & 63] = k.q[tid >> 6][tid & 63];
+  place_prologue<true>(a, partial, self_prefix, (uint32_t)kPlaceChunkRgb, s_sum, s_dc, s_dst);
+  const int lane = tid & 63, wv = tid >> 6, rr = lane >> 3, rb = lane & 7;
+  int* ws = s_ws[wv];
+  int16_t* zz = s_zz[wv][rb];
+  uint32_t zp[8];
+#pragma unroll
+  for (int c = 0; c < 8; c++) zp[c] = s_inv[rr * 8 + c];
+  const bool vec_ok = ((k.pitch[0] | (uintptr_t)k.plane[0]) & (BPP == 4 ? 15 : 7)) == 0;
+  for (int step = wv; step < kPlaceChunkRgb / 24; step += kPlaceChunk / 64) {
+    const uint32_t loc = (uint32_t)((step * 8 + rb) * 3);
+    const uint32_t ent = s_dst[loc];
+    const bool real = ent != 0xffffffffu;
+    int vy[8] = {0, 0, 0, 0, 0, 0, 0, 0}, vb[8] = {0, 0, 0, 0, 0, 0, 0, 0}, vr[8] = {0, 0, 0, 0, 0, 0, 0, 0};
+    int big_y = 0, big_b = 0, big_r = 0;
+    if (real) {
+      const int16_t* line = a.coef_scan + (size_t)(t0 + loc) * 64 + rr * 8;
+      const uint4 ry = *(const uint4*)line, rcb = *(const uint4*)(line + 64), rcr = *(const uint4*)(line + 128);
+      gather_dequant_row(ry, zz, zp, rr, s_dc[loc], &s_q[0][rr * 8], vy, big_y);
+      gather_dequant_row(rcb, zz, zp, rr, s_dc[loc + 1u], &s_q[1][rr * 8], vb, big_b);
+      gather_dequant_row(rcr, zz, zp, rr, s_dc[loc + 2u], &s_q[2][rr * 8], vr, big_r);
+    }
+    uint32_t sy[8], sb[8], sr[8];
+    idct::idct_wave(ws, vy, big_y, rr, rb, sy);
+    idct::idct_wave(ws, vb, big_b, rr, rb, sb);
+    idct::idct_wave(ws, vr, big_r, rr, rb, sr);
+    const uint32_t y = ((ent >> 15) & 0x7fffu) * 8u + (uint32_t)rr, x0 = (ent & 0x7fffu) * 8u;
+    if (real && y < k.h && x0 < k.w) {
+      uint32_t px[8];
+#pragma unroll
+      for (int c = 0; c < 8; c++) px[c] = upsample::ycc_px(sy[c], sb[c], sr[c], k.k_cr_g, k.k_cb_g);
+      upsample::store_px8<BPP>(k.plane[0] + (size_t)y * k.pitch[0] + (size_t)x0 * BPP, px, x0, k.w, vec_ok);
+    }
+  }
+}
 __global__ __launch_bounds__(1024) void dc_scan_partials_kernel(int* __restrict__ partial, int nchunks) {
   __shared__ int s_sum[3 * 16];
   const int tid = (int)threadIdx.x;
@@ -1583,14 +1699,32 @@
   }
   hipLaunchKernelGGL(sync_write2_kernel, dim3(grid), dim3(threads), lds, s, a, final_buf);
 }
-static void launch_place(const HuffSyncArgs& a, int* dc_partial, hipStream_t s) {
-  const int nch = (int)((a.total_blocks + kPlaceChunk - 1) / kPlaceChunk);
-  hipLaunchKernelGGL(dc_partial2_kernel, dim3(nch), dim3(kPlaceChunk), 0, s, a, dc_partial);
+static bool sink_fits(const HuffSyncArgs& a, const HuffSampleSink& k) {
+  if (k.kind == 1) {
+    for (int c = 0; c < a.ncomp; c++)
+      if (!k.plane[c] || ((k.pitch[c] | (uintptr_t)k.plane[c]) & 7) != 0 || (size_t)a.bw[c] * 8 > k.pitch[c]) return false;
+    return true;
+  }
+  if (k.kind == 2)
+    return a.ncomp == 3 && a.blocks_per_mcu == 3 && k.plane[0] && (k.bpp == 3 || k.bpp == 4) && (size_t)k.w * (size_t)k.bpp <= k.pitch[0] &&
+           k.w <= (uint32_t)a.bw[0] * 8u && k.h <= (uint32_t)a.bh[0] * 8u;
+  return false;
+}
+static hipError_t launch_place(const HuffSyncArgs& a, int* dc_partial, hipStream_t s, const HuffSampleSink* sink) {
+  if (sink && !sink_fits(a, *sink)) return hipErrorInvalidValue;
+  const uint32_t chunk = sink && sink->kind == 2 ? (uint32_t)kPlaceChunkRgb : (uint32_t)kPlaceChunk;
+  const int nch = (int)((a.total_blocks + chunk - 1) / chunk);
+  hipLaunchKernelGGL(dc_partial2_kernel, dim3(nch), dim3(kPlaceChunk), 0, s, a, dc_partial, chunk);
   const int self_prefix = nch <= kPlaceSelfPrefix ? 1 : 0;
   if (!self_prefix) hipLaunchKernelGGL(dc_scan_partials_kernel, dim3(1), dim3(1024), 0, s, dc_partial, nch);
-  hipLaunchKernelGGL(coef_place_kernel, dim3(nch), dim3(kPlaceChunk), 0, s, a, (const int*)dc_partial, self_prefix);
-}
-int huff_place_chunk() { return kPlaceChunk; }
+  if (!sink) hipLaunchKernelGGL(coef_place_kernel, dim3(nch), dim3(kPlaceChunk), 0, s, a, (const int*)dc_partial, self_prefix);
+  else if (sink->kind == 1) hipLaunchKernelGGL(sample_place_planar_kernel, dim3(nch), dim3(kPlaceChunk), 0, s, a, (const int*)dc_partial, self_prefix, *sink);
+  else if (sink->bpp == 4) hipLaunchKernelGGL((sample_place_rgb_kernel<4>), dim3(nch), dim3(kPlaceChunk), 0, s, a, (const int*)dc_partial, self_prefix, *sink);
+  else hipLaunchKernelGGL((sample_place_rgb_kernel<3>), dim3(nch), dim3(kPlaceChunk), 0, s, a, (const int*)dc_partial, self_prefix, *sink);
+  return hipSuccess;
+}
+int huff_place_chunk() { return kPlaceChunkRgb < kPlaceChunk ? kPlaceChunkRgb : kPlaceChunk; }
+void huff_sink_set_variant(HuffSampleSink* sink, int libjpeg_variant) { upsample::ycc_green_constants(libjpeg_variant, &sink->k_cr_g, &sink->k_cb_g); }
 static void launch_dc(const HuffSyncArgs& a, int* dc_partial, hipStream_t s) {
   const int nch = (int)((a.total_blocks + 1023) / 1024);
   hipLaunchKernelGGL(dc_partial_kernel, dim3(nch), dim3(1024), 0, s, a, dc_partial);
@@ -1601,7 +1735,7 @@
 
 uint32_t huff_sync_max_subsequences(uint64_t nbytes, uint32_t sub_bits) { return (uint32_t)((nbytes * 8 + sub_bits - 1) / sub_bits); }
 
-hipError_t launch_huffman_decode_sync(const HuffSyncArgs& a, int max_rounds, int* dc_partial, int* final_buf, hipStream_t s) {
+hipError_t launch_huffman_decode_sync(const HuffSyncArgs& a, int max_rounds, int* dc_partial, int* final_buf, hipStream_t s, const HuffSampleSink* sink) {
   const uint32_t nsub = huff_sync_max_subsequences(a.nbytes, a.sub_bits);
   const int grid = (int)((nsub + kSyncBlock - 1) / kSyncBlock);
   const size_t lds = (size_t)kSyncBlock * ((a.sub_bits >> 3) + 4) + 64;
@@ -1613,7 +1747,8 @@
   }
   if (a.coef_scan && !a.rst_map) {
     launch_write2(a, nsub, *final_buf, s);
-    launch_place(a, dc_partial, s);
+    const hipError_t ep = launch_place(a, dc_partial, s, sink);
+    if (ep != hipSuccess) return ep;
   } else {
     launch_write(a, nsub, *final_buf, s);
     launch_dc(a, dc_partial, s);
@@ -1628,7 +1763,7 @@
   return pre + ntiles * kHuffHypSlots + ((ntiles + 255) & ~(size_t)255);
 }
 
-hipError_t launch_huffman_decode_hyp(const HuffSyncArgs& a, int* dc_partial, uint8_t* chain_prefix, uint8_t* chain_tiles, hipStream_t s) {
+hipError_t launch_huffman_decode_hyp(const HuffSyncArgs& a, int* dc_partial, uint8_t* chain_prefix, uint8_t* chain_tiles, hipStream_t s, const HuffSampleSink* sink) {
   const uint32_t nsub = huff_sync_max_subsequences(a.nbytes, a.sub_bits);
   const int grid = (int)((nsub + 63) / 64);
   const int threads = 64 * a.hyp_h;
@@ -1700,7 +1835,8 @@
   if (a.coef_scan && !a.rst_map) {
     launch_write2(w, nw, 0, s);
     mark();
-    launch_place(a, dc_partial, s);
+    const hipError_t ep = launch_place(a, dc_partial, s, sink);
+    if (ep != hipSuccess) return ep;
   } else {
     launch_write(a, nsub, 0, s);
     mark();
diff --git a/libultrahdr_amd/csrc/idct_core.h b/libultrahdr_amd/csrc/idct_core.h
--- a/libultrahdr_amd/csrc/idct_core.h
+++ b/libultrahdr_amd/csrc/idct_core.h
@@ -60,19 +60,22 @@
   }
 }
 
+__device__ __forceinline__ void dequant_row(const uint32_t w4[4], const int q[8], int v[8], int& big) {
+#pragma unroll
+  for (int c = 0; c < 4; c++) {
+    v[2 * c] = __mul24((int)(int16_t)(w4[c] & 0xffff), q[2 * c]);
+    v[2 * c + 1] = __mul24((int)(int16_t)(w4[c] >> 16), q[2 * c + 1]);
+  }
+  const int mx = max(max(max(v[0], v[1]), max(v[2], v[3])), max(max(v[4], v[5]), max(v[6], v[7])));
+  const int mn = min(min(min(v[0], v[1]), min(v[2], v[3])), min(min(v[4], v[5]), min(v[6], v[7])));
+  big |= (int)(mx > 8191) | (int)(mn < -8191);
+}
 __device__ __forceinline__ void load_dequant_row(const int16_t* __restrict__ coef, int bw, int by, int bx, int rr,
                                                  const int q[8], int v[8], int& big, bool row_ok = true) {
   if (bx < bw && row_ok) {
     const uint4 raw = *(const uint4*)(coef + ((size_t)by * bw + bx) * 64 + rr * 8);
     const uint32_t w4[4] = {raw.x, raw.y, raw.z, raw.w};
-#pragma unroll
-    for (int c = 0; c < 4; c++) {
-      v[2 * c] = __mul24((int)(int16_t)(w4[c] & 0xffff), q[2 * c]);
-      v[2 * c + 1] = __mul24((int)(int16_t)(w4[c] >> 16), q[2 * c + 1]);
-    }
-    const int mx = max(max(max(v[0], v[1]), max(v[2], v[3])), max(max(v[4], v[5]), max(v[6], v[7])));
-    const int mn = min(min(min(v[0], v[1]), min(v[2], v[3])), min(min(v[4], v[5]), min(v[6], v[7])));
-    big |= (int)(mx > 8191) | (int)(mn < -8191);
+    dequant_row(w4, q, v, big);
   } else {
 #pragma unroll
     for (int c = 0; c < 8; c++) v[c] = 0;
diff --git a/libultrahdr_amd/csrc/uhdr_types.h b/libultrahdr_amd/csrc/uhdr_types.h
--- a/libultrahdr_amd/csrc/uhdr_types.h
+++ b/libultrahdr_amd/csrc/uhdr_types.h
@@ -344,11 +344,21 @@
   uint32_t* rst_partial;
   uint32_t rst_chunks;
 };
+struct HuffSampleSink {
+  int kind;
+  int bpp;
+  uint8_t* plane[3];
+  uint32_t pitch[3];
+  uint32_t w, h;
+  int k_cr_g, k_cb_g;
+  uint16_t q[3][64];
+};
+void huff_sink_set_variant(HuffSampleSink* sink, int libjpeg_variant);
 constexpr int kHuffHypSlots = 48;
 constexpr int kHuffFlagStragglers = 20;
 constexpr int kHuffFlagStray = 21;
 size_t huff_hyp_chain_bytes(uint64_t nbytes, uint32_t sub_bits, size_t* tiles_offset);
-hipError_t launch_huffman_decode_hyp(const HuffSyncArgs& a, int* dc_partial, uint8_t* chain_prefix, uint8_t* chain_tiles, hipStream_t s);
+hipError_t launch_huffman_decode_hyp(const HuffSyncArgs& a, int* dc_partial, uint8_t* chain_prefix, uint8_t* chain_tiles, hipStream_t s, const HuffSampleSink* sink = nullptr);
 int huff_sync_chunks(uint64_t nbytes);
 uint32_t huff_sync_max_subsequences(uint64_t nbytes, uint32_t sub_bits);
 struct HuffInitFill {
@@ -359,7 +369,7 @@
 };
 hipError_t launch_huffman_unstuff(const uint8_t* data, uint32_t nbytes, uint32_t* chunk_counts, uint32_t* nstuffed_dev, uint8_t* clean, hipStream_t s,
                                   uint32_t* rst_map, uint32_t* rst_partial, const HuffInitFill* fill = nullptr);
-hipError_t launch_huffman_decode_sync(const HuffSyncArgs& a, int max_rounds, int* dc_partial, int* final_buf, hipStream_t s);
+hipError_t launch_huffman_decode_sync(const HuffSyncArgs& a, int max_rounds, int* dc_partial, int* final_buf, hipStream_t s, const HuffSampleSink* sink = nullptr);
 void launch_profile_mark(hipStream_t s);
 int huff_marker_chunks(uint64_t nbytes);
 int huff_place_chunk();
```

Measured after the change: 12510 Mpixels/s (median of 6 runs). 4.1% higher.
